# stevengj/nlopt

Hardware: AMD Instinct MI355X
Metric: candidate-evals/sec, CRS2_LM n=4096 pop=100000 (trial phase) (higher is better)
Workload: dtype f64; 1 GPU; NLOPT_GN_CRS2_LM griewank n=4096 pop=100000 seed=42, 2000 candidate evals per step, population resident in HBM

## Files before the change

include/nlopt_amd.h:

```cpp
#ifndef NLOPT_AMD_H
#define NLOPT_AMD_H

#include <stddef.h>
#include <stdint.h>
#include "nlopt.h"

#ifdef __cplusplus
extern "C" {
#endif

#define NLOPT_AMD_OBJ_RASTRIGIN  0
#define NLOPT_AMD_OBJ_ACKLEY     1
#define NLOPT_AMD_OBJ_GRIEWANK   2
#define NLOPT_AMD_OBJ_ROSENBROCK 3
#define NLOPT_AMD_OBJ_LEVY       4
#define NLOPT_AMD_OBJ_SPHERE     5
#define NLOPT_AMD_OBJ_COUNT      6

nlopt_func nlopt_amd_objective(int id);
int nlopt_amd_objective_id(nlopt_func f);
const char *nlopt_amd_objective_name(int id);
void nlopt_amd_objective_box(int id, double *lo, double *hi);

nlopt_func nlopt_amd_constraint_blocksum(void);
int nlopt_amd_constraint_id(nlopt_func f);

int nlopt_amd_device_count(void);

nlopt_result nlopt_amd_set_min_device_objective(nlopt_opt opt, const char *code_object, const char *name, nlopt_func host_twin, void *f_data);
nlopt_result nlopt_amd_set_max_device_objective(nlopt_opt opt, const char *code_object, const char *name, nlopt_func host_twin, void *f_data);
int nlopt_amd_has_device_objective(const nlopt_opt opt);

typedef struct { double f; int64_t row; int32_t kind; int32_t accepted; } nlopt_amd_trace_rec;
nlopt_result nlopt_amd_set_trace(nlopt_opt opt, nlopt_amd_trace_rec *buf, size_t cap);
size_t nlopt_amd_trace_len(const nlopt_opt opt);

typedef struct {
    uint64_t rounds;
    uint64_t slots_launched;
    uint64_t slots_used;
    uint64_t slots_invalid;
    uint64_t slots_newbest;
    uint64_t slots_role;
    uint64_t evals_init, evals_trial, evals_mutation;
    uint64_t accepted;
    uint64_t mt_words;
    double t_init_s, t_trial_s;
    double t_gather_ms;
    uint64_t gather_launches;
    uint64_t gather_bytes;
    uint64_t generations, rank_sweeps;
    double t_eval_s, t_rank_s, t_evolve_s, t_rng_s;
    uint64_t lbfgs_launches, lbfgs_bytes;
    double t_lbfgs_ms;
    double t_stochrank_ms;
    uint64_t stochrank_launches, stochrank_ticks;
    double t_allgather_ms;
    uint64_t allgather_bytes;
    uint64_t evolve_rounds_enqueued, evolve_rounds;
    double t_engine_s, t_walk_s;
    uint64_t list_refreshes, list_refreshes_beside_device;
    double t_list_refresh_s;
    uint64_t isres_gate_timeouts;
    uint64_t mlsl_sampled_ahead;
    uint64_t cobyla_host_searches;
    uint64_t lbfgs_longest_chain_steps;
    uint64_t mlsl_gate_timeouts;
} nlopt_amd_stats;
nlopt_result nlopt_amd_get_stats(const nlopt_opt opt, nlopt_amd_stats *out);
size_t nlopt_amd_get_stats_sized(const nlopt_opt opt, void *out, size_t bytes);

typedef void (*nlopt_amd_progress_fn)(void *data, long generations_done, long numevals);
nlopt_result nlopt_amd_set_progress(nlopt_opt opt, nlopt_amd_progress_fn fn, void *data);

typedef struct nlopt_amd_comm_s nlopt_amd_comm;
typedef int (*nlopt_amd_allgather_fn)(void *ctx, const void *h_send, void *h_recv, size_t bytes);
int nlopt_amd_rccl_unique_id(void *id128);
nlopt_amd_comm *nlopt_amd_comm_create_rccl(int rank, int world, const void *id128);
nlopt_amd_comm *nlopt_amd_comm_create_host(int rank, int world, nlopt_amd_allgather_fn fn, void *ctx);
nlopt_amd_comm *nlopt_amd_comm_create_shm(int rank, int world, const char *name, size_t slot_bytes);
void nlopt_amd_comm_set_timeout(nlopt_amd_comm *c, double seconds);
void nlopt_amd_comm_destroy(nlopt_amd_comm *c);
int nlopt_amd_comm_rank(const nlopt_amd_comm *c);
int nlopt_amd_comm_world(const nlopt_amd_comm *c);
const char *nlopt_amd_comm_error(const nlopt_amd_comm *c);
void nlopt_amd_comm_counters(const nlopt_amd_comm *c, uint64_t *calls, uint64_t *bytes);
nlopt_result nlopt_amd_set_comm(nlopt_opt opt, nlopt_amd_comm *c);

typedef struct nlopt_amd_crs_session nlopt_amd_crs_session;
nlopt_amd_crs_session *nlopt_amd_crs_open(nlopt_opt opt, double *x, double *minf, nlopt_result *ret);
nlopt_result nlopt_amd_crs_step(nlopt_amd_crs_session *s, long eval_budget);
nlopt_result nlopt_amd_crs_close(nlopt_amd_crs_session *s);

#define NLA_MT_N 624
#define NLA_MT_POLYWORDS 312
#define NLA_MT_SEG_REGENS 1024
#define NLA_MT_SEG_WORDS (624ULL * NLA_MT_SEG_REGENS)

int nla_k_mt_jump(const uint64_t *poly, const uint32_t *src_states, uint32_t *dst_states, int count, void *stream);

int nla_k_mt_generate(const uint32_t *seg_states, uint64_t seg_first, int nseg,
                      uint64_t g_first, uint64_t count, uint32_t *out, void *stream);
int nla_k_mt_generate_seg(const uint32_t *seg_states, uint64_t seg_first, int nseg, uint64_t g_first, uint64_t count, uint32_t *out,
                          int seg_regens, void *stream);
int nla_k_mt_rankbits(const uint32_t *seg_states, uint64_t seg_first, int nseg, uint64_t g_rank0, uint64_t g_first,
                      uint64_t count, int64_t popm1, int64_t rowwords, uint64_t *bits, void *stream);
int nla_k_mt_rankbits_gated(const uint32_t *seg_states, uint64_t seg_first, int nseg, uint64_t g_rank0, uint64_t g_first, uint64_t count,
                            int64_t popm1, int64_t rowwords, uint64_t *bits, int *gate, int *ticket, int waves_per_cu, void *stream);
int nla_rankbits_gate_target(uint64_t g_rank0, int64_t popm1, int64_t nrows, int64_t c);

int nla_k_crs_init_rows(int obj, int n, int ld, const double *lb, const double *ub, const uint32_t *words,
                        int64_t row_first, int64_t nrows, double *X, double *F, void *stream);

int nla_k_eval(int obj, int n, int ld, const double *P, int64_t count, double *F, void *stream);

int nla_k_crs_vitter(int n, int64_t N, const uint32_t *words, int nblocks,
                     int32_t *jn, int32_t *pos, int32_t *last, void *stream);

typedef struct { double fT, fM; int32_t t, pad; } nla_crs_slot_status;

int nla_k_crs_advance(int n, int ld, const double *X, int64_t i0, const int32_t *jn_ring,
                      const int32_t *pos_ring, const int32_t *last_ring, uint32_t ring_blocks,
                      uint64_t first_block, int K, const int64_t *W, int nW,
                      const int32_t *t_in, int32_t *t_out, int slot_mask, const double *lb, const double *ub,
                      double *TX, int variant, void *stream);

size_t nla_crs_chain_ctrl_bytes(int K, int nW);
int nla_crs_chain_chunks(int n, int ld);
int nla_k_crs_chain(int obj, int n, int ld, const double *X, int64_t i0, double f_best, const int32_t *jn_ring,
                    const int32_t *pos_ring, const int32_t *last_ring, const uint32_t *words_ring, uint32_t ring_blocks,
                    uint64_t first_block, int K, const int64_t *W, const double *Wf, int nW, int w_on_host, int slot_mask,
                    const double *lb, const double *ub, double *TX, double *TM, void *ctrl, uint32_t ticket_base,
                    nla_crs_slot_status *status, uint32_t *fwcnt, uint32_t *fwrec, int fwcap, void *stream);
int nla_k_crs_chain_lean(int obj, int n, int ld, const double *X, int64_t i0, double f_best, const int32_t *jn_ring,
                         const int32_t *pos_ring, const int32_t *last_ring, const uint32_t *words_ring, uint32_t ring_blocks,
                         uint64_t first_block, int K, const int64_t *W, const double *Wf, int nW, int w_on_host, int slot_mask,
                         const double *lb, const double *ub, double *TX, double *TM, void *ctrl, uint32_t ticket_base,
                         nla_crs_slot_status *status, uint32_t *fwcnt, uint32_t *fwrec, int fwcap, int ctrl_is_zero, void *stream);
int nla_crs_chain_sh_chunks(int n, int ncols);
size_t nla_crs_chain_sh_table_bytes(void);
size_t nla_crs_chain_sh_stop_bytes(void);
int nla_crs_chain_sh_table(void *host_image, int world, int rank, int c0, int ldf, int chunks_total, int chunk0, void *const *peerTX,
                           void *const *peerflags, void *const *peerstop, const double *xbest, const double *lbf, const double *ubf);
int nla_k_crs_chain_sh(int obj, int n, int ncols, int ld, int ldf, const double *X, int64_t i0, double f_best, const int32_t *jn_ring,
                       const int32_t *pos_ring, const int32_t *last_ring, const uint32_t *words_ring, uint32_t ring_blocks,
                       uint64_t first_block, int K, const int64_t *W, const double *Wf, int nW, int w_on_host, int slot_mask,
                       const double *lb, const double *ub, double *TX, double *TM, void *ctrl, uint32_t ticket_base,
                       nla_crs_slot_status *status, uint32_t *fwcnt, uint32_t *fwrec, int fwcap, int ctrl_is_zero,
                       const void *table, uint32_t seq, uint32_t stopbits, int grid_cap, void *stream);
uint32_t nla_crs_chain_sh_tickets(int n, int ncols, int K, int grid_cap);
int nla_k_crs_commit_sh(int nc, int ld, int ldf, int c0, double *X, const double *TX, const double *TM, int ncommit,
                        const int32_t *h_slot, const int32_t *h_kind, const int64_t *h_row, void *zero, size_t zero_bytes,
                        int n, int best_slot, int best_kind, double *xbest, void *stream);
uint32_t nla_crs_chain_tickets(int n, int ld, int K);

int nla_k_crs_finish(int obj, int n, int ld, const double *X, int64_t i0, const double *TX, double *TM,
                     const uint32_t *words_ring, uint32_t ring_blocks, uint64_t first_block, int K,
                     const int32_t *t_in, const int32_t *t_out, int slot_mask,
                     const double *lb, const double *ub, double *fT_ring, double *fM_ring,
                     nla_crs_slot_status *status, void *stream);

int nla_k_crs_advance_args(int n, int ld, const double *X, int64_t i0, const int32_t *jn_ring,
                           const int32_t *pos_ring, const int32_t *last_ring, uint32_t ring_blocks,
                           uint64_t first_block, int K, const int64_t *h_W, int nW,
                           const int32_t *h_t_in, int32_t *t_out, int slot_mask, const double *lb, const double *ub,
                           double *TX, int variant, void *stream);
int nla_k_crs_finish_args(int obj, int n, int ld, const double *X, int64_t i0, const double *TX, double *TM,
                          const uint32_t *words_ring, uint32_t ring_blocks, uint64_t first_block, int K,
                          const int32_t *h_t_in, const int32_t *t_out, int slot_mask,
                          const double *lb, const double *ub, double *fT_ring, double *fM_ring,
                          nla_crs_slot_status *status, void *stream);
int nla_k_crs_finish_args_bell(int obj, int n, int ld, const double *X, int64_t i0, const double *TX, double *TM,
                          const uint32_t *words_ring, uint32_t ring_blocks, uint64_t first_block, int K,
                          const int32_t *h_t_in, const int32_t *t_out, int slot_mask,
                          const double *lb, const double *ub, double *fT_ring, double *fM_ring,
                          nla_crs_slot_status *status, uint32_t *bell_count, uint32_t *bell, uint32_t bell_seq, void *stream);
int nla_k_crs_commit_args(int n, int ld, double *X, const double *TX, const double *TM, int ncommit,
                          const int32_t *h_slot, const int32_t *h_kind, const int64_t *h_row, void *stream);
int nla_k_crs_advance_commit_args(int n, int ld, double *X, int64_t i0, const int32_t *jn_ring,
                                  const int32_t *pos_ring, const int32_t *last_ring, uint32_t ring_blocks,
                                  uint64_t first_block, int K, const int64_t *h_W, int nW,
                                  const int32_t *h_t_in, int32_t *t_out, int slot_mask, const double *lb, const double *ub,
                                  double *TX, const double *TM, int ncommit, const int32_t *h_slot, const int32_t *h_kind,
                                  const int64_t *h_row, int variant, void *stream);

int nla_k_crs_advance_cols(int n, int ncol, int ld, const double *X, int64_t i0, const int32_t *jn_ring,
                           const int32_t *pos_ring, const int32_t *last_ring, uint32_t ring_blocks,
                           uint64_t first_block, int K, const int64_t *W, int nW,
                           const int32_t *t_in, int32_t *t_out, int slot_mask, const double *lb, const double *ub,
                           double *TX, int variant, void *stream);
int nla_k_crs_sh_init_rows(int n, int c0, int nc, int ld, const double *lb, const double *ub, const uint32_t *words,
                           int64_t row_first, int64_t nrows, double *X, void *stream);
int nla_k_crs_sh_mutate_pack(int n, int c0, int nc, int ld, int colper, const double *X, int64_t i0, const double *TX, double *TM,
                             const uint32_t *words_ring, uint32_t ring_blocks, uint64_t first_block, int K, const int32_t *t_in,
                             const int32_t *t_out, int slot_mask, const double *lb, const double *ub, double *SEND,
                             int flag_forced, int flag_timed, void *stream);
int nla_k_crs_sh_eval(int obj, int n, int colper, uint64_t first_block, int K, const int32_t *t_in, const int32_t *t_out, int slot_mask,
                      const double *RECV, int world, double *fT_ring, double *fM_ring, nla_crs_slot_status *status, void *stream);

int nla_k_crs_commit(int n, int ld, double *X, const double *TX, const double *TM, int ncommit,
                     const int32_t *slot, const int32_t *kind, const int64_t *row, void *stream);

int nla_k_crs_commit_zero(int n, int ld, double *X, const double *TX, const double *TM, int ncommit, const int32_t *slot,
                          const int32_t *kind, const int64_t *row, int lists_on_host, void *zero, size_t zero_bytes, void *stream);

int nla_k_crs_mutate(int n, const double *best, double *p, const uint32_t *words,
                     const double *lb, const double *ub, void *stream);


typedef struct { int32_t type; uint32_t q, Q; int32_t pad; double tol; } nla_dev_constraint;

int nla_k_isres_init(int n, int ld, const double *lb, const double *ub, const uint32_t *words, int64_t k_first,
                     int64_t count, const double *x0, double *X, double *S, void *stream);

int nla_k_isres_eval(int obj, int n, int ld, const double *X, int64_t pop, int m, int p, const nla_dev_constraint *con,
                     double *F, double *PEN, double *GPEN, int32_t *FEAS, void *stream);

int nla_k_isres_rank_count(int64_t pop, const double *F, const double *PEN, uint64_t *elems, int32_t *sorted, void *stream);

int nla_k_isres_bits(const uint32_t *words, int64_t row_first, int nrows, int64_t pop, uint64_t *bits, void *stream);

int nla_isres_stochrank_handoff(void);
int nla_k_isres_stochrank(int64_t pop, int64_t nsweeps, uint64_t *streams, int *progress, const uint64_t *bits,
                          int *ticket, uint8_t *swapped, int32_t *irank, void *stream);
int nla_k_isres_stochrank_gated(int64_t pop, int64_t nsweeps, uint64_t *streams, int *progress, const uint64_t *bits, int *ticket,
                                uint8_t *swapped, int32_t *irank, const int *gate, uint64_t gate_g_rank0, int64_t gate_nrows, void *stream);

int nla_k_isres_nrand(const uint32_t *words, int64_t nattempts, int64_t attempt_base, int32_t *counts, int64_t *ztotal,
                      int64_t zbase, double *z, int64_t *zatt, void *stream);

int nla_k_isres_evolve(int n, int ld, int phase, int64_t pop, int64_t survivors, int64_t zcount, double taup, double tau,
                       const double *lb, const double *ub, const double *z, const int32_t *irank, double *X, double *S,
                       double *scratch, int64_t *state, void *stream);

size_t nla_isres_evolve2_ws_bytes(int n);
int nla_isres_evolve2_supported(int n);
int nla_k_isres_inverse(int64_t pop, const int32_t *irank, int32_t *inv, void *stream);
int nla_k_isres_evolve_rounds(int n, int ld, int phase, int64_t pop, int64_t survivors, int64_t zcount, double taup, double tau,
                              const double *lb, const double *ub, const double *z, const int32_t *irank, const int32_t *inv,
                              double *X, double *S, const double *x0c, int64_t *state, double *rho, void *ws, const double *mu_rp,
                              int rounds, void *stream);
int nla_k_isres_evolve_parent_mu(int n, int ld, int64_t survivors, const double *lb, const double *ub, const int32_t *irank,
                                 const double *X, const double *S, double *mu_rp, void *stream);

#define NLA_OBJ_EXTERNAL (-1)
#define NLA_OBJ_NEGATE 0x100
typedef struct { int32_t state, want_grad; } nla_local_req;
typedef struct {
    nla_local_req *req;
    double *EX, *EG, *EF;
    void *save;
    int32_t resume;
    int32_t forced, timeout;
    int32_t pad;
} nla_local_ext;

typedef struct { double minf_max, ftol_rel, ftol_abs, xtol_rel, tolg; int32_t maxeval, exact; double sign;
                 const double *xtol_abs, *x_weights; const int32_t *abort;
                 double *ftrace; int64_t ftrace_cap;
                 int32_t *done;
               } nla_lbfgs_params;
typedef struct { double f; int32_t ret, nevals, iterm, cols; } nla_lbfgs_result;
size_t nla_lbfgs_work_doubles(int ld, int mf, int count);
size_t nla_lbfgs_hist_doubles(int ld, int mf, int count);
size_t nla_lbfgs_save_bytes(void);

int nla_k_lbfgs_batch(int obj, int n, int ld, int mf, int count, const double *lb, const double *ub, double *X,
                      double *work, int *iwork, double *hist, const nla_lbfgs_params *params, nla_lbfgs_result *out,
                      const nla_local_ext *ext, void *stream);

typedef struct { double minf_max, ftol_rel, ftol_abs, xtol_rel, rho_init, sigma_min;
                 int32_t maxeval, inner_maxeval, inner_gradients, always_improve; int32_t exact, pad; double sign;
                 const double *xtol_abs, *x_weights; const int32_t *abort;
                 double *ftrace; int64_t ftrace_cap;
                 int32_t *done;
               } nla_mma_params;
size_t nla_mma_work_doubles(int ld, int count);
size_t nla_mma_save_bytes(void);

typedef struct { double minf_max, ftol_rel, ftol_abs, xtol_rel; int32_t maxeval, exact; double sign;
                 const double *xtol_abs; const int32_t *abort; int32_t *done; } nla_cobyla_params;
size_t nla_cobyla_work_doubles(int n, int ld, int count);
size_t nla_cobyla_work_ints(int n, int count);
size_t nla_cobyla_lds_bytes(int n);
int nla_cobyla_fits(int n);
int nla_k_cobyla_batch(int obj, int n, int ld, int count, const double *lb, const double *ub, const double *dx, double *X,
                       double *work, int *iwork, const nla_cobyla_params *params, nla_lbfgs_result *out, void *stream);

int nla_k_mma_batch(int obj, int n, int ld, int count, const double *lb, const double *ub, const double *sigma_init, double *X,
                    double *work, const nla_mma_params *params, nla_lbfgs_result *out, const nla_local_ext *ext, void *stream);

int nla_k_mlsl_sobol_rows(int n, int ld, const double *lb, const double *ub, const uint32_t *V, uint32_t index_first,
                          int count, double *P, void *stream);
int nla_k_mlsl_dist2(int n, int ld, const double *A, int na, const double *B, int nb, double *D, void *stream);
int nla_k_mlsl_rowmin(const double *D, int ldd, int na, int nb, const double *FA, const double *FB, const double *init, double *out, void *stream);
int nla_k_mlsl_colmin(const double *D, int ldd, int na, int nb, const double *FA, const double *FB, const int32_t *skip, double *inout, void *stream);
int nla_k_mlsl_gather_rows(int n, int ld, const double *src, const int64_t *idx, int count, double *dst, void *stream);
int nla_k_mlsl_gather_pairs(const double *D, int ldd, const int64_t *rows, int nr, const int64_t *cols, int nc, double *out, void *stream);
int nla_k_mlsl_gather_pairs_t(const double *D, int ldd, const int64_t *rows, int nr, const int64_t *cols, int nc, double *out, void *stream);
int nla_k_mlsl_near_bound(int n, int ld, const double *P, const int64_t *idx, int count, const double *lb, const double *ub,
                          double thr, int32_t *flags, void *stream);

int nla_k_mlsl_negate(double *F, int count, void *stream);

int nla_k_esch_cauchy(const uint32_t *words, int64_t nattempts, int64_t attempt_base, int32_t *counts, int64_t *vtotal,
                      int64_t vbase, int64_t vcap, double *v, int64_t *vatt, void *stream);
int nla_k_esch_fill_rows(int n, int ld, const double *lb, const double *ub, const double *v, int64_t e0, int64_t count, double *R, void *stream);
int nla_k_esch_crossover(int n, int ld, int64_t np, int64_t no, const uint32_t *words, const int32_t *slot, double *R, void *stream);
size_t nla_esch_mut_scratch_bytes(int64_t M);
int nla_k_esch_mutate(const uint32_t *W, int64_t M, int64_t total, int n, int ld, int64_t np, int64_t no, const double *lb,
                      const double *ub, const int32_t *slot, double *R, int32_t *last, void *scratch, int64_t *out, void *stream);
int nla_k_esch_gather_rows(int n, int ld, const int32_t *slot, int64_t i0, int64_t count, const double *R, double *G, void *stream);
size_t nla_esch_sort_scratch_bytes(int64_t count);
int nla_k_esch_select(int64_t count, const int32_t *slot_in, const double *fit_in, int32_t *slot_out, double *fit_out,
                      void *scratch, size_t scratch_bytes, void *stream);

int nla_dev_count(void);
int nla_dev_set(int dev);
void *nla_dev_malloc(size_t bytes);
void nla_dev_free(void *p);
void *nla_dev_malloc_uncached(size_t bytes);
void nla_debug_uncached_stats(long out[4]);
void nla_dev_free_uncached(void *p);
size_t nlopt_amd_release_device_memory(void);
void *nla_host_malloc(size_t bytes);
void nla_host_free(void *p);
int nla_host_register(void *p, size_t bytes);
void nla_host_unregister(void *p);
int nla_memcpy_h2d(void *dst, const void *h_src, size_t bytes, void *stream);
int nla_memcpy_d2h(void *h_dst, const void *src, size_t bytes, void *stream);
int nla_memcpy_d2d(void *dst, const void *src, size_t bytes, void *stream);
int nla_memset(void *dst, int value, size_t bytes, void *stream);
void *nla_stream_create(void);
void *nla_stream_create_cu_share(int part, int parts);
#define NLA_IPC_BYTES 96
int nla_ipc_export(const void *p, void *blob96);
void *nla_ipc_open(const void *blob96);
void nla_ipc_close(void *p);
void *nla_stream_create_background(void);
void nla_stream_destroy(void *stream);
int nla_stream_sync(void *stream);
int nla_stream_query(void *stream);
void *nla_event_create(void);
void nla_event_destroy(void *ev);
int nla_event_record(void *ev, void *stream);
int nla_event_sync(void *ev);
float nla_event_elapsed_ms(void *ev0, void *ev1);
int nla_stream_wait_event(void *stream, void *ev);
int nla_k_gate(const int32_t *counter, int32_t from, int32_t need, double timeout_ms, int32_t *gave_up , void *stream);
const char *nla_dev_error_string(int err);
void *nla_module_load_file(const char *path);
void *nla_module_load_data(const void *image);
void nla_module_unload(void *module);
void *nla_module_function(void *module, const char *name);
int nla_module_launch(void *function, unsigned grid_x, unsigned block_x, void **params, void *stream);

#ifdef __cplusplus
}
#endif
#endif
```

nlopt_amd/__init__.py:

```python
import ctypes as C
import os

import numpy as np

_HERE = os.path.dirname(os.path.abspath(__file__))
LIB_PATH = os.environ.get("NLOPT_AMD_LIB") or os.path.join(_HERE, "lib", "libnlopt_amd.so")

GN_CRS2_LM, GN_MLSL, GD_MLSL, GN_MLSL_LDS, GD_MLSL_LDS = 19, 20, 21, 22, 23
LD_LBFGS, LD_MMA, GN_ISRES, G_MLSL, G_MLSL_LDS, GN_ESCH = 11, 24, 35, 38, 39, 42
LN_COBYLA = 25
FAILURE, INVALID_ARGS, OUT_OF_MEMORY, ROUNDOFF_LIMITED, FORCED_STOP = -1, -2, -3, -4, -5
SUCCESS, STOPVAL_REACHED, FTOL_REACHED, XTOL_REACHED, MAXEVAL_REACHED, MAXTIME_REACHED = 1, 2, 3, 4, 5, 6

OBJECTIVES = {"rastrigin": 0, "ackley": 1, "griewank": 2, "rosenbrock": 3, "levy": 4, "sphere": 5}

NLOPT_FUNC = C.CFUNCTYPE(C.c_double, C.c_uint, C.POINTER(C.c_double), C.POINTER(C.c_double), C.c_void_p)

TRACE_DTYPE = np.dtype([("f", "f8"), ("row", "i8"), ("kind", "i4"), ("accepted", "i4")])


class Stats(C.Structure):
    _fields_ = [(k, C.c_uint64) for k in ("rounds", "slots_launched", "slots_used", "slots_invalid", "slots_newbest",
                                           "slots_role", "evals_init", "evals_trial", "evals_mutation", "accepted",
                                           "mt_words")] + \
               [("t_init_s", C.c_double), ("t_trial_s", C.c_double), ("t_gather_ms", C.c_double),
                ("gather_launches", C.c_uint64), ("gather_bytes", C.c_uint64), ("generations", C.c_uint64),
                ("rank_sweeps", C.c_uint64), ("t_eval_s", C.c_double), ("t_rank_s", C.c_double), ("t_evolve_s", C.c_double),
                ("t_rng_s", C.c_double), ("lbfgs_launches", C.c_uint64), ("lbfgs_bytes", C.c_uint64), ("t_lbfgs_ms", C.c_double),
                ("t_stochrank_ms", C.c_double), ("stochrank_launches", C.c_uint64), ("stochrank_ticks", C.c_uint64),
                ("t_allgather_ms", C.c_double), ("allgather_bytes", C.c_uint64),
                ("evolve_rounds_enqueued", C.c_uint64), ("evolve_rounds", C.c_uint64),
                ("t_engine_s", C.c_double), ("t_walk_s", C.c_double),
                ("list_refreshes", C.c_uint64), ("list_refreshes_beside_device", C.c_uint64), ("t_list_refresh_s", C.c_double),
                ("isres_gate_timeouts", C.c_uint64), ("mlsl_sampled_ahead", C.c_uint64), ("cobyla_host_searches", C.c_uint64), ("lbfgs_longest_chain_steps", C.c_uint64), ("mlsl_gate_timeouts", C.c_uint64)]

    def asdict(self):
        return {k: getattr(self, k) for k, _ in self._fields_}


_lib = None


def build(force=False, verbose=False):
    from . import _build as _b
    return _b.build(force=force, verbose=verbose)


def _dp(a):
    return a.ctypes.data_as(C.POINTER(C.c_double))


def lib():
    global _lib
    if _lib is not None:
        return _lib
    if not os.path.exists(LIB_PATH):
        raise RuntimeError("libnlopt_amd.so is not built: run `python -c 'import __graft_entry__ as g; g.build()'`")
    L = C.CDLL(LIB_PATH)
    vp, dbl, dpp = C.c_void_p, C.c_double, C.POINTER(C.c_double)
    L.nlopt_create.restype = vp
    L.nlopt_create.argtypes = [C.c_int, C.c_uint]
    L.nlopt_copy.restype = vp
    L.nlopt_copy.argtypes = [vp]
    L.nlopt_destroy.argtypes = [vp]
    L.nlopt_destroy.restype = None
    L.nlopt_optimize.argtypes = [vp, dpp, dpp]
    for nm in ("nlopt_set_min_objective", "nlopt_set_max_objective"):
        getattr(L, nm).argtypes = [vp, vp, vp]
    for nm in ("nlopt_set_lower_bounds", "nlopt_set_upper_bounds", "nlopt_get_lower_bounds", "nlopt_get_upper_bounds",
               "nlopt_set_xtol_abs", "nlopt_get_xtol_abs", "nlopt_set_x_weights", "nlopt_get_x_weights",
               "nlopt_set_initial_step"):
        getattr(L, nm).argtypes = [vp, dpp]
    for nm in ("nlopt_set_lower_bounds1", "nlopt_set_upper_bounds1", "nlopt_set_stopval", "nlopt_set_ftol_rel",
               "nlopt_set_ftol_abs", "nlopt_set_xtol_rel", "nlopt_set_xtol_abs1", "nlopt_set_x_weights1",
               "nlopt_set_maxtime", "nlopt_set_initial_step1"):
        getattr(L, nm).argtypes = [vp, dbl]
    for nm in ("nlopt_get_stopval", "nlopt_get_ftol_rel", "nlopt_get_ftol_abs", "nlopt_get_xtol_rel", "nlopt_get_maxtime"):
        getattr(L, nm).argtypes = [vp]
        getattr(L, nm).restype = dbl
    L.nlopt_set_lower_bound.argtypes = [vp, C.c_int, dbl]
    L.nlopt_set_upper_bound.argtypes = [vp, C.c_int, dbl]
    L.nlopt_set_maxeval.argtypes = [vp, C.c_int]
    for nm in ("nlopt_get_maxeval", "nlopt_get_numevals", "nlopt_get_force_stop", "nlopt_force_stop", "nlopt_get_algorithm"):
        getattr(L, nm).argtypes = [vp]
    L.nlopt_set_force_stop.argtypes = [vp, C.c_int]
    L.nlopt_get_dimension.argtypes = [vp]
    L.nlopt_get_dimension.restype = C.c_uint
    L.nlopt_set_population.argtypes = [vp, C.c_uint]
    L.nlopt_get_population.argtypes = [vp]
    L.nlopt_get_population.restype = C.c_uint
    L.nlopt_set_vector_storage.argtypes = [vp, C.c_uint]
    L.nlopt_get_vector_storage.argtypes = [vp]
    L.nlopt_get_vector_storage.restype = C.c_uint
    L.nlopt_set_local_optimizer.argtypes = [vp, vp]
    L.nlopt_get_errmsg.argtypes = [vp]
    L.nlopt_get_errmsg.restype = C.c_char_p
    L.nlopt_set_param.argtypes = [vp, C.c_char_p, dbl]
    L.nlopt_get_param.argtypes = [vp, C.c_char_p, dbl]
    L.nlopt_get_param.restype = dbl
    L.nlopt_has_param.argtypes = [vp, C.c_char_p]
    L.nlopt_num_params.argtypes = [vp]
    L.nlopt_num_params.restype = C.c_uint
    L.nlopt_nth_param.argtypes = [vp, C.c_uint]
    L.nlopt_nth_param.restype = C.c_char_p
    for nm in ("nlopt_add_inequality_constraint", "nlopt_add_equality_constraint"):
        getattr(L, nm).argtypes = [vp, vp, vp, dbl]
    for nm in ("nlopt_remove_inequality_constraints", "nlopt_remove_equality_constraints"):
        getattr(L, nm).argtypes = [vp]
    L.nlopt_srand.argtypes = [C.c_ulong]
    L.nlopt_srand.restype = None
    L.nlopt_algorithm_name.argtypes = [C.c_int]
    L.nlopt_algorithm_name.restype = C.c_char_p
    L.nlopt_algorithm_to_string.argtypes = [C.c_int]
    L.nlopt_algorithm_to_string.restype = C.c_char_p
    L.nlopt_algorithm_from_string.argtypes = [C.c_char_p]
    L.nlopt_result_to_string.argtypes = [C.c_int]
    L.nlopt_result_to_string.restype = C.c_char_p
    L.nlopt_result_from_string.argtypes = [C.c_char_p]
    L.nlopt_version.argtypes = [C.POINTER(C.c_int)] * 3
    L.nlopt_urand.argtypes = [dbl, dbl]
    L.nlopt_urand.restype = dbl
    L.nlopt_nrand.argtypes = [dbl, dbl]
    L.nlopt_nrand.restype = dbl
    L.nlopt_iurand.argtypes = [C.c_int]
    L.nla_genrand_int32.restype = C.c_uint32
    L.nlopt_amd_objective.argtypes = [C.c_int]
    L.nlopt_amd_objective.restype = vp
    L.nlopt_amd_objective_id.argtypes = [vp]
    L.nlopt_amd_objective_name.argtypes = [C.c_int]
    L.nlopt_amd_objective_name.restype = C.c_char_p
    L.nlopt_amd_objective_box.argtypes = [C.c_int, dpp, dpp]
    L.nlopt_amd_objective_box.restype = None
    L.nlopt_amd_constraint_blocksum.restype = vp
    L.nlopt_amd_set_trace.argtypes = [vp, vp, C.c_size_t]
    L.nlopt_amd_trace_len.argtypes = [vp]
    L.nlopt_amd_trace_len.restype = C.c_size_t
    L.nlopt_amd_get_stats.argtypes = [vp, C.POINTER(Stats)]
    L.nlopt_amd_crs_open.argtypes = [vp, dpp, dpp, C.POINTER(C.c_int)]
    L.nlopt_amd_crs_open.restype = vp
    L.nlopt_amd_crs_step.argtypes = [vp, C.c_long]
    L.nlopt_amd_crs_close.argtypes = [vp]
    L.nla_dev_malloc.argtypes = [C.c_size_t]
    L.nla_dev_malloc.restype = vp
    L.nla_dev_free.argtypes = [vp]
    L.nla_dev_free.restype = None
    for nm in ("nla_memcpy_h2d", "nla_memcpy_d2h", "nla_memcpy_d2d"):
        getattr(L, nm).argtypes = [vp, vp, C.c_size_t, vp]
    L.nla_memset.argtypes = [vp, C.c_int, C.c_size_t, vp]
    L.nla_stream_create.restype = vp
    L.nla_stream_destroy.argtypes = [vp]
    L.nla_stream_sync.argtypes = [vp]
    L.nla_event_create.restype = vp
    L.nla_event_destroy.argtypes = [vp]
    L.nla_event_record.argtypes = [vp, vp]
    L.nla_event_sync.argtypes = [vp]
    L.nla_event_elapsed_ms.argtypes = [vp, vp]
    L.nla_event_elapsed_ms.restype = C.c_float
    L.nla_dev_error_string.argtypes = [C.c_int]
    L.nla_dev_error_string.restype = C.c_char_p
    L.nla_mtstream_create.argtypes = [vp]
    L.nla_mtstream_create.restype = vp
    L.nla_mtstream_destroy.argtypes = [vp]
    L.nla_mtstream_destroy.restype = None
    L.nla_mtstream_fill.argtypes = [vp, C.c_uint64, C.c_uint64, vp]
    L.nla_mtstream_finish.argtypes = [vp, C.c_uint64]
    L.nla_mtstream_rankbits.argtypes = [vp, C.c_uint64, C.c_uint64, C.c_uint64, C.c_int64, C.c_int64, vp]
    L.nla_k_mt_jump.argtypes = [vp, vp, vp, C.c_int, vp]
    L.nla_k_mt_generate.argtypes = [vp, C.c_uint64, C.c_int, C.c_uint64, C.c_uint64, vp, vp]
    L.nla_k_crs_init_rows.argtypes = [C.c_int, C.c_int, C.c_int, vp, vp, vp, C.c_int64, C.c_int64, vp, vp, vp]
    L.nla_k_eval.argtypes = [C.c_int, C.c_int, C.c_int, vp, C.c_int64, vp, vp]
    L.nla_k_crs_vitter.argtypes = [C.c_int, C.c_int64, vp, C.c_int, vp, vp, vp, vp]
    L.nla_k_crs_advance.argtypes = [C.c_int, C.c_int, vp, C.c_int64, vp, vp, vp, C.c_uint32, C.c_uint64, C.c_int, vp, C.c_int,
                                    vp, vp, C.c_int, vp, vp, vp, C.c_int, vp]
    L.nlopt_amd_has_device_objective.argtypes = [vp]
    L.nla_dev_malloc_uncached.argtypes = [C.c_size_t]
    L.nla_dev_malloc_uncached.restype = vp
    L.nla_dev_free_uncached.argtypes = [vp]
    L.nla_dev_free_uncached.restype = None
    L.nla_k_crs_chain.argtypes = [C.c_int, C.c_int, C.c_int, vp, C.c_int64, C.c_double, vp, vp, vp, vp, C.c_uint32, C.c_uint64, C.c_int, vp, vp,
                                  C.c_int, C.c_int, C.c_int, vp, vp, vp, vp, vp, C.c_uint32, vp, vp, vp, C.c_int, vp]
    L.nla_crs_chain_tickets.argtypes = [C.c_int, C.c_int, C.c_int]
    L.nla_crs_chain_tickets.restype = C.c_uint32
    L.nla_crs_chain_ctrl_bytes.argtypes = [C.c_int, C.c_int]
    L.nla_crs_chain_ctrl_bytes.restype = C.c_size_t
    L.nla_crs_chain_chunks.argtypes = [C.c_int, C.c_int]
    L.nla_k_crs_finish.argtypes = [C.c_int, C.c_int, C.c_int, vp, C.c_int64, vp, vp, vp, C.c_uint32, C.c_uint64, C.c_int,
                                   vp, vp, C.c_int, vp, vp, vp, vp, vp, vp]
    L.nla_k_isres_rank_count.argtypes = [C.c_int64, vp, vp, vp, vp, vp]
    L.nla_k_isres_bits.argtypes = [vp, C.c_int64, C.c_int, C.c_int64, vp, vp]
    L.nla_k_isres_stochrank.argtypes = [C.c_int64, C.c_int64, vp, vp, vp, vp, vp, vp, vp]
    L.nla_k_isres_stochrank_gated.argtypes = [C.c_int64, C.c_int64, vp, vp, vp, vp, vp, vp, vp, C.c_uint64, C.c_int64, vp]
    L.nla_isres_evolve2_ws_bytes.restype = C.c_size_t
    L.nla_isres_evolve2_ws_bytes.argtypes = [C.c_int]
    L.nla_k_isres_inverse.argtypes = [C.c_int64, vp, vp, vp]
    L.nla_k_isres_evolve_rounds.argtypes = ([C.c_int, C.c_int, C.c_int, C.c_int64, C.c_int64, C.c_int64, C.c_double, C.c_double] + [vp] * 12 +
                                            [C.c_int, vp])
    L.nla_k_crs_commit.argtypes = [C.c_int, C.c_int, vp, vp, vp, C.c_int, vp, vp, vp, vp]
    L.nla_k_crs_mutate.argtypes = [C.c_int, vp, vp, vp, vp, vp, vp]
    L.nla_mt_jump_poly_words.argtypes = [C.c_uint64, vp]
    L.nla_mt_jump_poly_words.restype = None
    L.nla_mt_jump_poly_pow2.argtypes = [C.c_int]
    L.nla_mt_jump_poly_pow2.restype = vp
    L.nla_mt_apply_jump_host.argtypes = [vp, vp, vp]
    L.nla_mt_apply_jump_host.restype = None
    L.nla_mt_advance_blocks_host.argtypes = [vp, C.c_uint64, vp]
    L.nla_mt_advance_blocks_host.restype = None
    L.nla_mt_export.argtypes = [vp, C.POINTER(C.c_int)]
    L.nla_mt_export.restype = None
    L.nla_mt_import.argtypes = [vp, C.c_int]
    L.nla_mt_import.restype = None
    L.nla_mt_charpoly_terms.argtypes = [C.POINTER(C.POINTER(C.c_int))]
    L.nlopt_amd_rccl_unique_id.argtypes = [vp]
    L.nlopt_amd_comm_create_rccl.argtypes = [C.c_int, C.c_int, vp]
    L.nlopt_amd_comm_create_rccl.restype = vp
    L.nlopt_amd_comm_create_host.argtypes = [C.c_int, C.c_int, vp, vp]
    L.nlopt_amd_comm_create_host.restype = vp
    L.nlopt_amd_comm_destroy.argtypes = [vp]
    L.nlopt_amd_comm_destroy.restype = None
    L.nlopt_amd_comm_rank.argtypes = [vp]
    L.nlopt_amd_comm_world.argtypes = [vp]
    L.nlopt_amd_comm_error.argtypes = [vp]
    L.nlopt_amd_comm_error.restype = C.c_char_p
    L.nlopt_amd_comm_counters.argtypes = [vp, C.POINTER(C.c_uint64), C.POINTER(C.c_uint64)]
    L.nlopt_amd_comm_counters.restype = None
    L.nlopt_amd_set_comm.argtypes = [vp, vp]
    L.nlopt_amd_set_progress.argtypes = [vp, vp, vp]
    L.nla_comm_allgather_host.argtypes = [vp, vp, vp, C.c_size_t, vp]
    L.nla_comm_allgather_dev.argtypes = [vp, vp, vp, C.c_size_t, vp]
    L.nla_comm_partition.argtypes = [vp, C.c_int64, C.POINTER(C.c_int64), C.POINTER(C.c_int64), C.POINTER(C.c_int64)]
    L.nla_comm_partition.restype = None
    L.nla_dev_set.argtypes = [C.c_int]
    _lib = L
    return L


def device_count():
    return lib().nlopt_amd_device_count()


def srand(seed):
    lib().nlopt_srand(seed)


def objective(name_or_id):
    i = OBJECTIVES[name_or_id] if isinstance(name_or_id, str) else int(name_or_id)
    return lib().nlopt_amd_objective(i)


def objective_box(name_or_id):
    i = OBJECTIVES[name_or_id] if isinstance(name_or_id, str) else int(name_or_id)
    lo, hi = C.c_double(), C.c_double()
    lib().nlopt_amd_objective_box(i, C.byref(lo), C.byref(hi))
    return lo.value, hi.value


class DevBuf:

    def __init__(self, nbytes, uncached=False):
        self.nbytes = int(nbytes)
        self.uncached = bool(uncached)
        self.ptr = (lib().nla_dev_malloc_uncached if uncached else lib().nla_dev_malloc)(self.nbytes)
        if not self.ptr:
            raise MemoryError("nla_dev_malloc(%d) failed" % self.nbytes)

    @classmethod
    def from_array(cls, a, uncached=False):
        a = np.ascontiguousarray(a)
        b = cls(max(a.nbytes, 1), uncached)
        L = lib()
        rc = L.nla_memcpy_h2d(b.ptr, a.ctypes.data, a.nbytes, None) or L.nla_stream_sync(None)
        if rc:
            raise RuntimeError("H2D failed: %s" % L.nla_dev_error_string(rc))
        return b

    def to_array(self, dtype, count):
        out = np.empty(count, dtype=dtype)
        L = lib()
        rc = L.nla_memcpy_d2h(out.ctypes.data, self.ptr, out.nbytes, None) or L.nla_stream_sync(None)
        if rc:
            raise RuntimeError("D2H failed: %s" % L.nla_dev_error_string(rc))
        return out

    def free(self):
        if self.ptr:
            (lib().nla_dev_free_uncached if getattr(self, "uncached", False) else lib().nla_dev_free)(self.ptr)
            self.ptr = None

    def __del__(self):
        try:
            self.free()
        except Exception:
            pass


PROGRESS_FN = C.CFUNCTYPE(None, C.c_void_p, C.c_long, C.c_long)
ALLGATHER_FN = C.CFUNCTYPE(C.c_int, C.c_void_p, C.c_void_p, C.c_void_p, C.c_size_t)


class Comm:

    def __init__(self, handle, keep=None):
        self._L = lib()
        self._h = handle
        self._keep = keep
        if not handle:
            raise RuntimeError("could not create the communicator")

    @classmethod
    def rccl(cls, rank, world, uid):
        buf = C.create_string_buffer(bytes(uid), 128)
        return cls(lib().nlopt_amd_comm_create_rccl(int(rank), int(world), C.cast(buf, C.c_void_p)))

    @classmethod
    def shm(cls, rank, world, name, slot_bytes=0):
        L = lib()
        L.nlopt_amd_comm_create_shm.restype = C.c_void_p
        L.nlopt_amd_comm_create_shm.argtypes = [C.c_int, C.c_int, C.c_char_p, C.c_size_t]
        return cls(L.nlopt_amd_comm_create_shm(int(rank), int(world), name.encode(), int(slot_bytes)))

    @classmethod
    def host(cls, rank, world, allgather):
        def _cb(ctx, send, recv, nbytes):
            try:
                out = allgather(C.string_at(send, nbytes))
                if len(out) != nbytes * world:
                    return 2
                C.memmove(recv, out, len(out))
                return 0
            except Exception:
                import traceback
                traceback.print_exc()
                return 1
        fn = ALLGATHER_FN(_cb)
        return cls(lib().nlopt_amd_comm_create_host(int(rank), int(world), C.cast(fn, C.c_void_p), None), keep=fn)

    @classmethod
    def from_torch_distributed(cls, group=None):
# ... 196 lines not shown
```

nlopt_amd/csrc/api_options.c:

```c
#include "nla_internal.h"
#include <math.h>
#include <stdarg.h>
#include <stdlib.h>
#include <string.h>

static double *dup_doubles(const double *src, unsigned n)
{
    double *d;
    if (!src) return NULL;
    d = (double *) malloc(sizeof(double) * (n ? n : 1));
    if (d && n) memcpy(d, src, sizeof(double) * n);
    return d;
}

const char *nla_set_errmsg(nlopt_opt opt, const char *fmt, ...)
{
    va_list ap;
    va_start(ap, fmt);
    opt->errmsg = nla_vsprintf(opt->errmsg, fmt, ap);
    va_end(ap);
    return opt->errmsg;
}
void nla_unset_errmsg(nlopt_opt opt) { if (opt) { free(opt->errmsg); opt->errmsg = NULL; } }
const char *nlopt_get_errmsg(nlopt_opt opt) { return opt->errmsg; }

static nlopt_result fail_msg(nlopt_opt opt, nlopt_result r, const char *msg) { if (opt) nla_set_errmsg(opt, "%s", msg); return r; }

static void free_constraints(nlopt_opt opt, nla_constraint **c, unsigned *m, unsigned *m_alloc, int munge)
{
    unsigned i;
    if (munge && opt->munge_on_destroy) for (i = 0; i < *m; ++i) opt->munge_on_destroy((*c)[i].f_data);
    for (i = 0; i < *m; ++i) free((*c)[i].tol);
    free(*c);
    *c = NULL; *m = *m_alloc = 0;
}

void nlopt_destroy(nlopt_opt opt)
{
    unsigned i;
    if (!opt) return;
    if (opt->munge_on_destroy) opt->munge_on_destroy(opt->f_data);
    free_constraints(opt, &opt->fc, &opt->m, &opt->m_alloc, 1);
    free_constraints(opt, &opt->h, &opt->p, &opt->p_alloc, 1);
    for (i = 0; i < opt->nparams; ++i) free(opt->params[i].name);
    free(opt->params);
    free(opt->lb); free(opt->ub); free(opt->xtol_abs); free(opt->x_weights); free(opt->dx);
    nlopt_destroy(opt->local_opt);
    nla_userobj_release(opt->userobj);
    free(opt->errmsg);
    free(opt);
}

nlopt_opt nlopt_create(nlopt_algorithm algorithm, unsigned n)
{
    nlopt_opt opt;
    unsigned i;
    if ((int) algorithm < 0 || algorithm >= NLOPT_NUM_ALGORITHMS) return NULL;
    opt = (nlopt_opt) calloc(1, sizeof *opt);
    if (!opt) return NULL;
    opt->algorithm = algorithm;
    opt->n = n;
    opt->stopval = -HUGE_VAL;
    if (n > 0) {
        opt->lb = (double *) malloc(sizeof(double) * n);
        opt->ub = (double *) malloc(sizeof(double) * n);
        if (!opt->lb || !opt->ub) { nlopt_destroy(opt); return NULL; }
        for (i = 0; i < n; ++i) { opt->lb[i] = -HUGE_VAL; opt->ub[i] = +HUGE_VAL; }
    }
    return opt;
}

static int copy_constraints(nlopt_opt dst, nla_constraint **dc, unsigned *dm, unsigned *dalloc,
                            const nla_constraint *sc, unsigned sm)
{
    unsigned i;
    *dc = NULL; *dm = *dalloc = 0;
    if (!sm) return 0;
    *dc = (nla_constraint *) malloc(sizeof(nla_constraint) * sm);
    if (!*dc) return -1;
    memcpy(*dc, sc, sizeof(nla_constraint) * sm);
    for (i = 0; i < sm; ++i) (*dc)[i].tol = NULL;
    *dm = *dalloc = sm;
    for (i = 0; i < sm; ++i) {
        if (dst->munge_on_copy && (*dc)[i].f_data && !((*dc)[i].f_data = dst->munge_on_copy((*dc)[i].f_data))) return -1;
        if (sc[i].tol && !((*dc)[i].tol = dup_doubles(sc[i].tol, sc[i].m))) return -1;
    }
    return 0;
}

nlopt_opt nlopt_copy(const nlopt_opt opt)
{
    nlopt_opt c;
    unsigned i;
    if (!opt) return NULL;
    c = (nlopt_opt) malloc(sizeof *c);
    if (!c) return NULL;
    *c = *opt;
    c->lb = c->ub = c->xtol_abs = c->x_weights = c->dx = NULL;
    c->fc = c->h = NULL; c->m = c->m_alloc = c->p = c->p_alloc = 0;
    c->params = NULL; c->nparams = 0;
    c->local_opt = NULL; c->errmsg = NULL; c->force_stop_child = NULL;
    c->trace = NULL; c->trace_cap = c->trace_len = 0;
    nla_userobj_retain(c->userobj);
    if (c->munge_on_copy && c->f_data && !(c->f_data = c->munge_on_copy(c->f_data))) goto oom;
    if (opt->n > 0) {
        if (!(c->lb = dup_doubles(opt->lb, opt->n)) || !(c->ub = dup_doubles(opt->ub, opt->n))) goto oom;
        if (opt->xtol_abs && !(c->xtol_abs = dup_doubles(opt->xtol_abs, opt->n))) goto oom;
        if (opt->x_weights && !(c->x_weights = dup_doubles(opt->x_weights, opt->n))) goto oom;
        if (opt->dx && !(c->dx = dup_doubles(opt->dx, opt->n))) goto oom;
    }
    if (copy_constraints(c, &c->fc, &c->m, &c->m_alloc, opt->fc, opt->m)) goto oom;
    if (copy_constraints(c, &c->h, &c->p, &c->p_alloc, opt->h, opt->p)) goto oom;
    if (opt->nparams) {
        c->params = (nla_param *) calloc(opt->nparams, sizeof(nla_param));
        if (!c->params) goto oom;
        c->nparams = opt->nparams;
        for (i = 0; i < opt->nparams; ++i) {
            size_t len = strlen(opt->params[i].name) + 1;
            if (!(c->params[i].name = (char *) malloc(len))) goto oom;
            memcpy(c->params[i].name, opt->params[i].name, len);
            c->params[i].val = opt->params[i].val;
        }
    }
    if (opt->local_opt && !(c->local_opt = nlopt_copy(opt->local_opt))) goto oom;
    return c;
oom:
    c->munge_on_destroy = NULL;
    nlopt_destroy(c);
    return NULL;
}

nlopt_result nlopt_set_param(nlopt_opt opt, const char *name, double val)
{
    size_t len;
    unsigned i;
    if (!opt) return NLOPT_INVALID_ARGS;
    if (!name) return fail_msg(opt, NLOPT_INVALID_ARGS, "invalid NULL parameter name");
    len = strnlen(name, 1024) + 1;
    if (len > 1024) return fail_msg(opt, NLOPT_INVALID_ARGS, "parameter name must be < 1024 bytes");
    if (!strncmp(name, "amd_", 4)) {
        static const char *const known[] = { "amd_forward", "amd_shard", "amd_shard_windows", "amd_cu_share", "amd_max_spec", "amd_window_factor", "amd_host_eval",
                                             "amd_exact_dot", "amd_isres_evolve_serial", "amd_isres_overlap", "amd_lbfgs_streaming", "amd_mlsl_seg_regens", "amd_cobyla_host", "amd_cobyla_min_batch", NULL };
        int k;
        for (k = 0; known[k] && strcmp(name, known[k]); ++k) { }
        if (!known[k]) return fail_msg(opt, NLOPT_INVALID_ARGS, "nlopt_amd: no such switch (the amd_* names this build reads: include/nlopt_amd.h, INTEGRATION.md E)");
    }
    for (i = 0; i < opt->nparams; ++i) if (!strcmp(name, opt->params[i].name)) break;
    if (i == opt->nparams) {
        nla_param *np = (nla_param *) realloc(opt->params, sizeof(nla_param) * (opt->nparams + 1));
        if (!np) return NLOPT_OUT_OF_MEMORY;
        opt->params = np;
        if (!(np[i].name = (char *) malloc(len))) return NLOPT_OUT_OF_MEMORY;
        memcpy(np[i].name, name, len);
        opt->nparams++;
    }
    opt->params[i].val = val;
    return NLOPT_SUCCESS;
}

static int find_param(const nlopt_opt opt, const char *name)
{
    unsigned i;
    if (!opt || !name || strnlen(name, 1024) == 1024) return -1;
    for (i = 0; i < opt->nparams; ++i) if (!strcmp(name, opt->params[i].name)) return (int) i;
    return -1;
}
double nlopt_get_param(const nlopt_opt opt, const char *name, double defaultval)
{
    int i = find_param(opt, name);
    return i < 0 ? defaultval : opt->params[i].val;
}
int nlopt_has_param(const nlopt_opt opt, const char *name) { return find_param(opt, name) >= 0; }
unsigned nlopt_num_params(const nlopt_opt opt) { return opt ? opt->nparams : 0; }
const char *nlopt_nth_param(const nlopt_opt opt, unsigned n) { return opt && n < opt->nparams ? opt->params[n].name : NULL; }

static nlopt_result set_objective(nlopt_opt opt, nlopt_func f, nlopt_precond pre, void *f_data, int maximize)
{
    if (!opt) return NLOPT_INVALID_ARGS;
    nla_unset_errmsg(opt);
    if (opt->munge_on_destroy) opt->munge_on_destroy(opt->f_data);
    nla_userobj_release(opt->userobj);
    opt->userobj = NULL;
    opt->f = f; opt->f_data = f_data; opt->pre = pre; opt->maximize = maximize;
    if (nla_isinf(opt->stopval) && (maximize ? opt->stopval < 0 : opt->stopval > 0))
        opt->stopval = maximize ? +HUGE_VAL : -HUGE_VAL;
    return NLOPT_SUCCESS;
}
nlopt_result nlopt_set_precond_min_objective(nlopt_opt o, nlopt_func f, nlopt_precond pre, void *d) { return set_objective(o, f, pre, d, 0); }
nlopt_result nlopt_set_precond_max_objective(nlopt_opt o, nlopt_func f, nlopt_precond pre, void *d) { return set_objective(o, f, pre, d, 1); }
nlopt_result nlopt_set_min_objective(nlopt_opt o, nlopt_func f, void *d) { return set_objective(o, f, NULL, d, 0); }
nlopt_result nlopt_set_max_objective(nlopt_opt o, nlopt_func f, void *d) { return set_objective(o, f, NULL, d, 1); }

static void snap_lower(nlopt_opt opt, unsigned i) { if (opt->lb[i] < opt->ub[i] && nla_istiny(opt->ub[i] - opt->lb[i])) opt->lb[i] = opt->ub[i]; }
static void snap_upper(nlopt_opt opt, unsigned i) { if (opt->lb[i] < opt->ub[i] && nla_istiny(opt->ub[i] - opt->lb[i])) opt->ub[i] = opt->lb[i]; }

nlopt_result nlopt_set_lower_bounds(nlopt_opt opt, const double *lb)
{
    unsigned i;
    nla_unset_errmsg(opt);
    if (!opt || (opt->n && !lb)) return NLOPT_INVALID_ARGS;
    for (i = 0; i < opt->n; ++i) opt->lb[i] = lb[i];
    for (i = 0; i < opt->n; ++i) snap_lower(opt, i);
    return NLOPT_SUCCESS;
}
nlopt_result nlopt_set_lower_bounds1(nlopt_opt opt, double lb)
{
    unsigned i;
    nla_unset_errmsg(opt);
    if (!opt) return NLOPT_INVALID_ARGS;
    for (i = 0; i < opt->n; ++i) { opt->lb[i] = lb; snap_lower(opt, i); }
    return NLOPT_SUCCESS;
}
nlopt_result nlopt_set_lower_bound(nlopt_opt opt, int i, double lb)
{
    nla_unset_errmsg(opt);
    if (!opt) return NLOPT_INVALID_ARGS;
    if (i < 0 || i >= (int) opt->n) return fail_msg(opt, NLOPT_INVALID_ARGS, "invalid bound index");
    opt->lb[i] = lb; snap_lower(opt, (unsigned) i);
    return NLOPT_SUCCESS;
}
nlopt_result nlopt_get_lower_bounds(const nlopt_opt opt, double *lb)
{
    nla_unset_errmsg(opt);
    if (!opt || (opt->n && !lb)) return NLOPT_INVALID_ARGS;
    if (opt->n) memcpy(lb, opt->lb, sizeof(double) * opt->n);
    return NLOPT_SUCCESS;
}
nlopt_result nlopt_set_upper_bounds(nlopt_opt opt, const double *ub)
{
    unsigned i;
    nla_unset_errmsg(opt);
    if (!opt || (opt->n && !ub)) return NLOPT_INVALID_ARGS;
    for (i = 0; i < opt->n; ++i) opt->ub[i] = ub[i];
    for (i = 0; i < opt->n; ++i) snap_upper(opt, i);
    return NLOPT_SUCCESS;
}
nlopt_result nlopt_set_upper_bounds1(nlopt_opt opt, double ub)
{
    unsigned i;
    nla_unset_errmsg(opt);
    if (!opt) return NLOPT_INVALID_ARGS;
    for (i = 0; i < opt->n; ++i) { opt->ub[i] = ub; snap_upper(opt, i); }
    return NLOPT_SUCCESS;
}
nlopt_result nlopt_set_upper_bound(nlopt_opt opt, int i, double ub)
{
    nla_unset_errmsg(opt);
    if (!opt) return NLOPT_INVALID_ARGS;
    if (i < 0 || i >= (int) opt->n) return fail_msg(opt, NLOPT_INVALID_ARGS, "invalid bound index");
    opt->ub[i] = ub; snap_upper(opt, (unsigned) i);
    return NLOPT_SUCCESS;
}
nlopt_result nlopt_get_upper_bounds(const nlopt_opt opt, double *ub)
{
    nla_unset_errmsg(opt);
    if (!opt || (opt->n && !ub)) return NLOPT_INVALID_ARGS;
    if (opt->n) memcpy(ub, opt->ub, sizeof(double) * opt->n);
    return NLOPT_SUCCESS;
}

static int is_auglag(nlopt_algorithm a)
{
    return a == NLOPT_AUGLAG || a == NLOPT_AUGLAG_EQ || a == NLOPT_LN_AUGLAG || a == NLOPT_LN_AUGLAG_EQ ||
           a == NLOPT_LD_AUGLAG || a == NLOPT_LD_AUGLAG_EQ;
}
static int accepts_inequality(nlopt_algorithm a)
{
    return a == NLOPT_LD_MMA || a == NLOPT_LD_CCSAQ || a == NLOPT_LD_SLSQP || a == NLOPT_LN_COBYLA || is_auglag(a) ||
           a == NLOPT_GN_ISRES || a == NLOPT_GN_ORIG_DIRECT || a == NLOPT_GN_ORIG_DIRECT_L || a == NLOPT_GN_AGS;
}
static int accepts_equality(nlopt_algorithm a)
{
    return is_auglag(a) || a == NLOPT_LD_SLSQP || a == NLOPT_GN_ISRES || a == NLOPT_LN_COBYLA;
}

static nlopt_result push_constraint(nlopt_opt opt, unsigned *m, unsigned *m_alloc, nla_constraint **c, unsigned fm,
                                    nlopt_func fc, nlopt_mfunc mfc, nlopt_precond pre, void *data, const double *tol)
{
    double *tolcopy;
    unsigned i;
    if ((fc && mfc) || (fc && fm != 1) || (!fc && !mfc)) return NLOPT_INVALID_ARGS;
    if (tol) for (i = 0; i < fm; ++i) if (tol[i] < 0) return fail_msg(opt, NLOPT_INVALID_ARGS, "negative constraint tolerance");
    tolcopy = (double *) calloc(fm ? fm : 1, sizeof(double));
    if (!tolcopy) return NLOPT_OUT_OF_MEMORY;
    if (tol) memcpy(tolcopy, tol, sizeof(double) * fm);
    if (*m + 1 > *m_alloc) {
        unsigned na = 2 * (*m + 1);
        nla_constraint *nc = (nla_constraint *) realloc(*c, sizeof(nla_constraint) * na);
        if (!nc) { free(tolcopy); return NLOPT_OUT_OF_MEMORY; }
        *c = nc; *m_alloc = na;
    }
    (*c)[*m].m = fm; (*c)[*m].f = fc; (*c)[*m].mf = mfc; (*c)[*m].pre = pre; (*c)[*m].f_data = data; (*c)[*m].tol = tolcopy;
    ++*m;
    return NLOPT_SUCCESS;
}

static nlopt_result add_any(nlopt_opt opt, int equality, unsigned fm, nlopt_func fc, nlopt_mfunc mfc, nlopt_precond pre,
                            void *data, const double *tol)
{
    nlopt_result ret;
    nla_unset_errmsg(opt);
    if (mfc && !fm) {
        if (opt && opt->munge_on_destroy) opt->munge_on_destroy(data);
        return NLOPT_SUCCESS;
    }
    if (!opt) ret = NLOPT_INVALID_ARGS;
    else if (!(equality ? accepts_equality(opt->algorithm) : accepts_inequality(opt->algorithm)))
        ret = fail_msg(opt, NLOPT_INVALID_ARGS, "invalid algorithm for constraints");
    else if (equality) ret = push_constraint(opt, &opt->p, &opt->p_alloc, &opt->h, fm, fc, mfc, pre, data, tol);
    else ret = push_constraint(opt, &opt->m, &opt->m_alloc, &opt->fc, fm, fc, mfc, pre, data, tol);
    if (ret < 0 && opt && opt->munge_on_destroy) opt->munge_on_destroy(data);
    return ret;
}

nlopt_result nlopt_remove_inequality_constraints(nlopt_opt opt)
{
    nla_unset_errmsg(opt);
    if (!opt) return NLOPT_INVALID_ARGS;
    free_constraints(opt, &opt->fc, &opt->m, &opt->m_alloc, 1);
    return NLOPT_SUCCESS;
}
nlopt_result nlopt_remove_equality_constraints(nlopt_opt opt)
{
    nla_unset_errmsg(opt);
    if (!opt) return NLOPT_INVALID_ARGS;
    free_constraints(opt, &opt->h, &opt->p, &opt->p_alloc, 1);
    return NLOPT_SUCCESS;
}
nlopt_result nlopt_add_inequality_mconstraint(nlopt_opt o, unsigned m, nlopt_mfunc fc, void *d, const double *tol) { return add_any(o, 0, m, NULL, fc, NULL, d, tol); }
nlopt_result nlopt_add_precond_inequality_constraint(nlopt_opt o, nlopt_func fc, nlopt_precond pre, void *d, double tol) { return add_any(o, 0, 1, fc, NULL, pre, d, &tol); }
nlopt_result nlopt_add_inequality_constraint(nlopt_opt o, nlopt_func fc, void *d, double tol) { return add_any(o, 0, 1, fc, NULL, NULL, d, &tol); }
nlopt_result nlopt_add_equality_mconstraint(nlopt_opt o, unsigned m, nlopt_mfunc fc, void *d, const double *tol) { return add_any(o, 1, m, NULL, fc, NULL, d, tol); }
nlopt_result nlopt_add_precond_equality_constraint(nlopt_opt o, nlopt_func fc, nlopt_precond pre, void *d, double tol) { return add_any(o, 1, 1, fc, NULL, pre, d, &tol); }
nlopt_result nlopt_add_equality_constraint(nlopt_opt o, nlopt_func fc, void *d, double tol) { return add_any(o, 1, 1, fc, NULL, NULL, d, &tol); }

#define NLA_SCALAR(name, T, field)                                                             \
    nlopt_result nlopt_set_##name(nlopt_opt opt, T v)                                          \
    { if (!opt) return NLOPT_INVALID_ARGS; nla_unset_errmsg(opt); opt->field = v; return NLOPT_SUCCESS; } \
    T nlopt_get_##name(const nlopt_opt opt) { return opt->field; }
NLA_SCALAR(stopval, double, stopval)
NLA_SCALAR(ftol_rel, double, ftol_rel)
NLA_SCALAR(ftol_abs, double, ftol_abs)
NLA_SCALAR(xtol_rel, double, xtol_rel)
NLA_SCALAR(maxeval, int, maxeval)
NLA_SCALAR(maxtime, double, maxtime)
NLA_SCALAR(population, unsigned, stochastic_population)
NLA_SCALAR(vector_storage, unsigned, vector_storage)
int nlopt_get_numevals(const nlopt_opt opt) { return opt->numevals; }
nlopt_algorithm nlopt_get_algorithm(const nlopt_opt opt) { return opt->algorithm; }
unsigned nlopt_get_dimension(const nlopt_opt opt) { return opt->n; }

static nlopt_result ensure_vec(nlopt_opt opt, double **v)
{
    if (!*v && opt->n > 0) { *v = (double *) calloc(opt->n, sizeof(double)); if (!*v) return NLOPT_OUT_OF_MEMORY; }
    return NLOPT_SUCCESS;
}

nlopt_result nlopt_set_xtol_abs(nlopt_opt opt, const double *tol)
{
    if (!opt) return NLOPT_INVALID_ARGS;
    nla_unset_errmsg(opt);
    if (!tol) { free(opt->xtol_abs); opt->xtol_abs = NULL; return NLOPT_SUCCESS; }
    if (ensure_vec(opt, &opt->xtol_abs) != NLOPT_SUCCESS) return NLOPT_OUT_OF_MEMORY;
    if (opt->n) memcpy(opt->xtol_abs, tol, sizeof(double) * opt->n);
    return NLOPT_SUCCESS;
}
nlopt_result nlopt_set_xtol_abs1(nlopt_opt opt, double tol)
{
    unsigned i;
    if (!opt) return NLOPT_INVALID_ARGS;
    nla_unset_errmsg(opt);
    if (ensure_vec(opt, &opt->xtol_abs) != NLOPT_SUCCESS) return NLOPT_OUT_OF_MEMORY;
    for (i = 0; i < opt->n; ++i) opt->xtol_abs[i] = tol;
    return NLOPT_SUCCESS;
}
nlopt_result nlopt_get_xtol_abs(const nlopt_opt opt, double *tol)
{
    unsigned i;
    nla_unset_errmsg(opt);
    if (!opt || (opt->n && !tol)) return NLOPT_INVALID_ARGS;
    for (i = 0; i < opt->n; ++i) tol[i] = opt->xtol_abs ? opt->xtol_abs[i] : 0;
    return NLOPT_SUCCESS;
}
nlopt_result nlopt_set_x_weights(nlopt_opt opt, const double *w)
{
    unsigned i;
    if (!opt) return NLOPT_INVALID_ARGS;
    nla_unset_errmsg(opt);
    if (!w) { free(opt->x_weights); opt->x_weights = NULL; return NLOPT_SUCCESS; }
    for (i = 0; i < opt->n; ++i) if (w[i] < 0) return fail_msg(opt, NLOPT_INVALID_ARGS, "invalid negative weight");
    if (ensure_vec(opt, &opt->x_weights) != NLOPT_SUCCESS) return NLOPT_OUT_OF_MEMORY;
    if (opt->n) memcpy(opt->x_weights, w, sizeof(double) * opt->n);
    return NLOPT_SUCCESS;
}
nlopt_result nlopt_set_x_weights1(nlopt_opt opt, double w)
{
    unsigned i;
    if (!opt) return NLOPT_INVALID_ARGS;
    if (w < 0) return fail_msg(opt, NLOPT_INVALID_ARGS, "invalid negative weight");
    nla_unset_errmsg(opt);
    if (ensure_vec(opt, &opt->x_weights) != NLOPT_SUCCESS) return NLOPT_OUT_OF_MEMORY;
    for (i = 0; i < opt->n; ++i) opt->x_weights[i] = w;
    return NLOPT_SUCCESS;
}
nlopt_result nlopt_get_x_weights(const nlopt_opt opt, double *w)
{
    unsigned i;
    if (!opt) return NLOPT_INVALID_ARGS;
    if (opt->n && !w) return fail_msg(opt, NLOPT_INVALID_ARGS, "invalid NULL weights");
    nla_unset_errmsg(opt);
    for (i = 0; i < opt->n; ++i) w[i] = opt->x_weights ? opt->x_weights[i] : 1;
    return NLOPT_SUCCESS;
}

nlopt_result nlopt_set_force_stop(nlopt_opt opt, int val)
{
    if (!opt) return NLOPT_INVALID_ARGS;
    nla_unset_errmsg(opt);
    opt->force_stop = val;
    if (opt->force_stop_child) return nlopt_set_force_stop(opt->force_stop_child, val);
    return NLOPT_SUCCESS;
}
int nlopt_get_force_stop(const nlopt_opt opt) { return opt->force_stop; }
nlopt_result nlopt_force_stop(nlopt_opt opt) { return nlopt_set_force_stop(opt, 1); }

nlopt_result nlopt_set_local_optimizer(nlopt_opt opt, const nlopt_opt local_opt)
{
    if (!opt) return NLOPT_INVALID_ARGS;
    nla_unset_errmsg(opt);
    if (local_opt && local_opt->n != opt->n) return fail_msg(opt, NLOPT_INVALID_ARGS, "dimension mismatch in local optimizer");
    nlopt_destroy(opt->local_opt);
    opt->local_opt = nlopt_copy(local_opt);
    if (local_opt) {
        if (!opt->local_opt) return NLOPT_OUT_OF_MEMORY;
        nlopt_set_lower_bounds(opt->local_opt, opt->lb);
        nlopt_set_upper_bounds(opt->local_opt, opt->ub);
        nlopt_remove_inequality_constraints(opt->local_opt);
        nlopt_remove_equality_constraints(opt->local_opt);
        nlopt_set_min_objective(opt->local_opt, NULL, NULL);
        nlopt_set_munge(opt->local_opt, NULL, NULL);
        opt->local_opt->force_stop = 0;
    }
    return NLOPT_SUCCESS;
}
// ... 92 lines not shown
```

nlopt_amd/csrc/crs_driver.c:

```c
#include "nla_internal.h"
#include <limits.h>
#include <math.h>
#include <stdlib.h>
#include <string.h>

typedef struct { double f; int64_t row; } osnode;
typedef struct {
    const double *F;
    osnode *node;
    void *mem;
    int64_t nheap, best;
    void *cand;
    int64_t *gpos;
} ordset;
#define OSN(s, i) ((s)->node[(i) + 3])

static inline int key_less(const double *F, int64_t a, int64_t b)
{
    if (F[a] < F[b]) return 1;
    if (F[a] > F[b]) return 0;
    return a < b;
}
static inline int node_less(const osnode a, const osnode b)
{
// ... 172 lines not shown
    tl_refresh(t, s, ahead > need ? ahead : need);
}

static inline int64_t tl_worst(const toplist *t) { return t->T[t->head].row; }

static void tl_idle(toplist *t, ordset *s)
{
    const int k = t->inflight;
    if (k <= 0 || t->whole || t->tail - t->head - k >= k) return;
    { const uint64_t r0 = t->refreshes; tl_refresh(t, s, 3 * k + 16); t->refreshes_idle += t->refreshes - r0; }
}

static void tl_accepted(toplist *t, ordset *s)
{
    topent e = t->T[t->head++];
    const double f = s->F[e.row];
    if (!e.recorded) {
        t->chg[t->nchg++] = e.pos;
        e.recorded = 1;
    }
    if (t->whole || t->thr_f < f || (!(t->thr_f > f) && t->thr_row < e.row)) {
        int lo = t->head, hi = t->tail;
        osnode k; k.f = f; k.row = e.row;
        while (lo < hi) {
            const int mid = (lo + hi) >> 1;
            osnode m; m.f = t->T[mid].f; m.row = t->T[mid].row;
            if (node_less(m, k)) hi = mid; else lo = mid + 1;
        }
        if (t->tail == 2 * t->cap) {
            memmove(t->T, t->T + t->head, sizeof(topent) * (size_t) (t->tail - t->head));
            lo -= t->head; t->tail -= t->head; t->head = 0;
        }
        memmove(t->T + lo + 1, t->T + lo, sizeof(topent) * (size_t) (t->tail - lo));
        e.f = f;
        t->T[lo] = e;
        ++t->tail;
    }
}

typedef struct {
    const nla_crs_engine_ops *ops; void *e;
    const nla_crs_problem *pb;
    ordset os;
    double *F;
    double *x;
    double *minf;
    double *xtmp;
    int need_x;
    const nla_stopping *sp;
    int64_t xrow;
    nlopt_result ret;
} run_state;

static void trace_add(const nla_crs_problem *pb, double f, int64_t row, int kind, int accepted)
{
    if (!pb->trace || !pb->trace_len) return;
    if (*pb->trace_len < pb->trace_cap) {
        nlopt_amd_trace_rec *r = pb->trace + *pb->trace_len;
        r->f = f; r->row = row; r->kind = kind; r->accepted = accepted;
    }
    ++*pb->trace_len;
}

static int after_accept(run_state *rs, uint64_t block, int kind)
{
    const nla_crs_problem *pb = rs->pb;
    nla_stopping *stop = pb->stop;
    const int64_t b = rs->os.best;
    nlopt_result ret = NLOPT_SUCCESS;
    int have_x = 0;
    if (rs->F[b] < *rs->minf) {
        if (rs->F[b] < stop->minf_max) ret = NLOPT_MINF_MAX_REACHED;
        else if (nla_stop_f(stop, rs->F[b], *rs->minf)) ret = NLOPT_FTOL_REACHED;
        else if (rs->need_x) {
            if (rs->ops->read_slot(rs->e, block, kind, rs->xtmp)) return -1;
            if (nla_stop_x(stop, rs->xtmp, rs->x)) ret = NLOPT_XTOL_REACHED;
            memcpy(rs->x, rs->xtmp, sizeof(double) * (size_t) pb->n);
            have_x = 1;
        }
        rs->xrow = have_x ? -1 : b;
        *rs->minf = rs->F[b];
    }
    if (ret != NLOPT_SUCCESS) {
        if (nla_stop_evals(stop)) ret = NLOPT_MAXEVAL_REACHED;
        else if (nla_stop_time(rs->sp)) ret = NLOPT_MAXTIME_REACHED;
    }
    rs->ret = ret;
    return 0;
}

#define TRING 2048
#define FWCAP 48

struct nla_crs_session {
    run_state rs;
    nla_crs_problem pb;
    nlopt_result ret;
    uint64_t block;
    uint64_t fresh_from;
    uint64_t init_words;
    int Kmax, host_eval;
    double kmult;
    double runlen;
    nla_crs_slot_status *status;
    int32_t *tprev;
    uint64_t *cblock;
    int32_t *ckind;
    int64_t *W, *crow;
    toplist tl;
    int forward;
    double *Wf;
    uint32_t *fwcnt, *fwrec;
    uint64_t *lastw;
    nla_stopping view; int agreed_force;
};

static void session_free(nla_crs_session *S)
{
    if (!S) return;
    free(S->rs.F); os_free(&S->rs.os); free(S->rs.xtmp);
    free(S->status); free(S->tprev); free(S->W); tl_free(&S->tl); free(S->cblock); free(S->ckind); free(S->crow);
    free(S->Wf); free(S->fwcnt); free(S->fwrec); free(S->lastw);
    free(S);
}

static void crs_idle(void *arg)
{
    nla_crs_session *S = (nla_crs_session *) arg;
    tl_idle(&S->tl, &S->rs.os);
}

static void engine_failed(nla_crs_session *S)
{
    nla_stopping *stop = S->pb.stop;
    if (stop->stop_msg && S->rs.ops->last_error) nla_stop_msg(stop, "device engine: %s", S->rs.ops->last_error(S->rs.e));
    S->ret = NLOPT_FAILURE;
}

nla_crs_session *nla_crs_begin(const nla_crs_engine_ops *ops, void *e, const nla_crs_problem *pb,
                               double *x, double *minf, nlopt_result *ret_out)
{
    const int n = pb->n;
    const int64_t N = pb->N;
    nla_stopping *stop = pb->stop;
    nlopt_amd_stats *st = pb->stats;
    nla_crs_session *S = (nla_crs_session *) calloc(1, sizeof *S);
    run_state *rs;
    nlopt_result ret = NLOPT_SUCCESS;
    int64_t rows_done = 0, i;
    double t0 = nla_seconds();
    if (!S) { *ret_out = NLOPT_OUT_OF_MEMORY; return NULL; }
    rs = &S->rs;
    S->pb = *pb;
    S->host_eval = pb->obj == -1;
    S->Kmax = pb->max_spec > 0 ? pb->max_spec : 256;
    S->kmult = pb->window_factor > 0 ? pb->window_factor : 1.5;
    if (S->Kmax > 1024) S->Kmax = 1024;
    if (S->host_eval) S->Kmax = 1;
    S->forward = pb->forward && ops->chain && pb->obj >= 0 && S->Kmax > 1;
    if (S->forward && S->Kmax > 256) S->Kmax = 256;
    if (S->forward && pb->max_spec <= 0 && S->Kmax > (n >= 2048 ? 128 : 256)) S->Kmax = n >= 2048 ? 128 : 256;
    if (S->forward && pb->max_spec <= 0 && (int64_t) S->Kmax > N / 16) S->Kmax = N / 16 > 8 ? (int) (N / 16) : 8;
    S->runlen = 4.0;
    rs->ops = ops; rs->e = e; rs->pb = &S->pb; rs->x = x; rs->minf = minf;
    rs->need_x = (stop->xtol_rel > 0 || stop->xtol_abs != NULL);

    rs->F = (double *) malloc(sizeof(double) * (size_t) N);
    const int os_bad = os_alloc(&rs->os, N, 3 * S->Kmax + 64);
    rs->xtmp = (double *) malloc(sizeof(double) * (size_t) (n > 0 ? n : 1));
    S->status = (nla_crs_slot_status *) malloc(sizeof(nla_crs_slot_status) * (size_t) S->Kmax);
    S->tprev = (int32_t *) calloc(TRING, sizeof(int32_t));
    S->W = (int64_t *) malloc(sizeof(int64_t) * (size_t) S->Kmax);
    const int tl_bad = tl_alloc(&S->tl, S->Kmax);
    S->cblock = (uint64_t *) malloc(sizeof(uint64_t) * (size_t) S->Kmax);
    S->ckind = (int32_t *) malloc(sizeof(int32_t) * (size_t) S->Kmax);
    S->crow = (int64_t *) malloc(sizeof(int64_t) * (size_t) S->Kmax);
    S->Wf = (double *) malloc(sizeof(double) * (size_t) S->Kmax);
    if (S->forward) {
        S->fwcnt = (uint32_t *) calloc((size_t) S->Kmax, sizeof(uint32_t));
        S->fwrec = (uint32_t *) calloc((size_t) S->Kmax * FWCAP, sizeof(uint32_t));
        S->lastw = (uint64_t *) calloc((size_t) N, sizeof(uint64_t));
    }
    if (!rs->F || os_bad || !rs->xtmp || !S->status || !S->tprev || !S->W || tl_bad || !S->Wf || !S->cblock ||
        !S->ckind || !S->crow || (S->forward && (!S->fwcnt || !S->fwrec || !S->lastw))) {
        session_free(S);
        *ret_out = NLOPT_OUT_OF_MEMORY;
        return NULL;
    }
    rs->os.F = rs->F;
    S->tl.st = st;
    if (ops->set_idle) ops->set_idle(e, crs_idle, S);

    rs->sp = stop;
    if (ops->init_population(e, x, rs->F)) { engine_failed(S); *ret_out = S->ret; return S; }
    if (pb->comm) {
        rs->sp = nla_comm_agree_stop(pb->comm, stop, &S->view, &S->agreed_force);
        if (!rs->sp) { nla_stop_msg(stop, "stop agreement failed: %s", nlopt_amd_comm_error(pb->comm)); S->ret = NLOPT_FAILURE; *ret_out = S->ret; return S; }
    }
    for (i = 0; i < N && ret == NLOPT_SUCCESS; ++i) {
        if (S->host_eval) {
            if (i == 0) rs->F[0] = pb->f((unsigned) n, x, NULL, pb->f_data);
            else {
                if (ops->read_row(e, i, rs->xtmp)) { engine_failed(S); *ret_out = S->ret; return S; }
                rs->F[i] = pb->f((unsigned) n, rs->xtmp, NULL, pb->f_data);
            }
        }
        ++*stop->nevals_p;
        if (st) ++st->evals_init;
        os_push(&rs->os, i);
        trace_add(pb, rs->F[i], i, 0, 1);
        rows_done = i + 1;
        if (rs->F[i] < stop->minf_max) ret = NLOPT_MINF_MAX_REACHED;
        else if (nla_stop_evals(stop)) ret = NLOPT_MAXEVAL_REACHED;
        else if (nla_stop_time(rs->sp)) ret = NLOPT_MAXTIME_REACHED;
    }
    S->init_words = 2ULL * (uint64_t) n * (uint64_t) (rows_done - 1);
    *minf = rs->F[rs->os.best];
    if (ops->read_row(e, rs->os.best, x)) { engine_failed(S); *ret_out = S->ret; return S; }
    rs->xrow = -1;
    if (st) st->t_init_s = nla_seconds() - t0;
    S->ret = ret;
    *ret_out = ret;
    return S;
}

nlopt_result nla_crs_advance(nla_crs_session *S, int64_t eval_budget)
{
    run_state *rs = &S->rs;
    const nla_crs_engine_ops *ops = rs->ops;
    void *e = rs->e;
    const nla_crs_problem *pb = &S->pb;
    nla_stopping *stop = pb->stop;
    nlopt_amd_stats *st = pb->stats;
    const int n = pb->n, host_eval = S->host_eval;
    const int64_t N = pb->N;
    nla_crs_slot_status *status = S->status;
    uint64_t *cblock = S->cblock;
    int32_t *ckind = S->ckind;
    int64_t *W = S->W, *crow = S->crow;
    nlopt_result ret = S->ret;
    const int evals_at_entry = *stop->nevals_p;
    double t0 = nla_seconds();

    while (ret == NLOPT_SUCCESS) {
        int K, nW, j = 0, ncommit = 0, best_changed = 0, cap, a, timed_pass = 1;
        uint64_t wend;
        if (eval_budget > 0 && (int64_t) (*stop->nevals_p - evals_at_entry) >= eval_budget) break;
        if (pb->comm) {
            if (ops->stop_flags_in && ops->stop_flags_out) ops->stop_flags_in(e, nla_stop_forced(stop), nla_stop_time(stop));
            else {
                rs->sp = nla_comm_agree_stop(pb->comm, stop, &S->view, &S->agreed_force);
                if (!rs->sp) { nla_stop_msg(stop, "stop agreement failed: %s", nlopt_amd_comm_error(pb->comm)); S->ret = NLOPT_FAILURE; return S->ret; }
            }
        }
        cap = ops->max_slots(e, S->block);
        if (cap <= 0) { engine_failed(S); return S->ret; }
        K = (int) ceil(S->kmult * S->runlen) + 4;
        if (K > S->Kmax) K = S->Kmax;
        if (K > cap) K = cap;
        if (K < 1) K = 1;
        if (!S->forward && S->fresh_from > S->block && (uint64_t) K < S->fresh_from - S->block && S->fresh_from - S->block <= (uint64_t) cap &&
            S->fresh_from - S->block <= (uint64_t) S->Kmax)
            K = (int) (S->fresh_from - S->block);
        nW = K < N ? K : (int) N;
        tl_need(&S->tl, &rs->os, nW, 3 * K + 16);
        for (a = 0; a < nW; ++a) { W[a] = S->tl.T[S->tl.head + a].row; S->Wf[a] = S->tl.T[S->tl.head + a].f; }
        if (S->forward) for (a = 0; a < nW; ++a) __builtin_prefetch(&S->lastw[W[a]], 1);
        const double t_eng0 = st ? nla_seconds() : 0.;
        const uint64_t gl0 = st ? st->gather_launches : 0;
        S->tl.inflight = nW;
        if (S->forward) {
            if (st && S->fresh_from > S->block) st->slots_invalid += S->fresh_from - S->block;
            S->fresh_from = S->block;
            if (ops->chain(e, S->block, K, rs->os.best, rs->F[rs->os.best], W, S->Wf, nW, status, S->fwcnt, S->fwrec, FWCAP)) { engine_failed(S); return S->ret; }
            if (pb->comm && ops->stop_flags_in && ops->stop_flags_out) {
                int forced = 0, timed = 0;
                ops->stop_flags_out(e, &forced, &timed);
                nla_stop_view(stop, forced, timed, &S->view, &S->agreed_force);
                rs->sp = &S->view;
            }
        } else
        {
            if (!S->forward && ops->advance(e, S->block, K, S->fresh_from, rs->os.best, W, nW, status)) { engine_failed(S); return S->ret; }
            if (pb->comm && ops->stop_flags_in && ops->stop_flags_out) {
                int forced = 0, timed = 0;
                ops->stop_flags_out(e, &forced, &timed);
                nla_stop_view(stop, forced, timed, &S->view, &S->agreed_force);
                rs->sp = &S->view;
            }
        }
        S->tl.inflight = 0;
        timed_pass = !st || st->gather_launches != gl0;
        wend = S->block + (uint64_t) K;
        const double t_walk0 = st ? nla_seconds() : 0.;
        if (st) {
            st->t_engine_s += t_walk0 - t_eng0;
            ++st->rounds;
            for (a = 0; a < K; ++a) {
                const uint64_t b = S->block + (uint64_t) a;
                const int32_t told = b >= S->fresh_from ? 0 : S->tprev[b % TRING];
                const int32_t tnew = status[a].t;
                if (b >= S->fresh_from) ++st->slots_launched;
                if (tnew > told && timed_pass) st->gather_bytes += 8ULL * (uint64_t) n * (uint64_t) (tnew - told + (told == 0 ? 1 : 0));
                S->tprev[b % TRING] = tnew;
            }
        }
        if (wend > S->fresh_from) S->fresh_from = wend;

        while (j < K && ret == NLOPT_SUCCESS) {
            int64_t worst;
            int kind = 1, accepted = 0;
            double fcand;
            const uint64_t blk = S->block + (uint64_t) j;
            if (best_changed) break;
            if (status[j].t < n) break;
            if (S->forward) {
                const uint32_t cnt = S->fwcnt[j];
                int ok = cnt <= FWCAP;
                uint32_t c;
                for (c = 0; ok && c < cnt; ++c) {
                    const uint32_t rec = S->fwrec[(size_t) j * FWCAP + c];
                    const int64_t r = W[rec & 0xffu];
                    const uint64_t pbk = S->block + (uint64_t) ((rec >> 8) & 0xffu);
                    const unsigned kind = (rec >> 16) & 3u;
                    if (kind == 0) ok = (S->lastw[r] >> 1) <= S->block;
                    else ok = S->lastw[r] == (((pbk + 1) << 1) | (kind == 1 ? 1u : 0u));
                }
                if (!ok) {
                    if (st) ++st->slots_invalid;
                    break;
                }
            }
            if (st) ++st->slots_used;
            if (S->tl.head == S->tl.tail) tl_need(&S->tl, &rs->os, 1, 3 * K + 16);
            worst = tl_worst(&S->tl);
            if (host_eval) {
                if (ops->read_slot(e, blk, 1, rs->xtmp)) { engine_failed(S); return S->ret; }
                status[j].fT = pb->f((unsigned) n, rs->xtmp, NULL, pb->f_data);
            }
            fcand = status[j].fT;
            ++*stop->nevals_p;
            if (st) ++st->evals_trial;
            if (nla_stop_forced(rs->sp)) { trace_add(pb, fcand, -1, 1, 0); ret = NLOPT_FORCED_STOP; ++j; break; }
            if (fcand < rs->F[worst]) accepted = 1;
            else {
                trace_add(pb, fcand, -1, 1, 0);
                if (nla_stop_evals(stop)) { ret = NLOPT_MAXEVAL_REACHED; ++j; break; }
                if (nla_stop_time(rs->sp)) { ret = NLOPT_MAXTIME_REACHED; ++j; break; }
                kind = 2;
                if (host_eval) {
                    if (ops->mutate_slot(e, blk, rs->os.best) || ops->read_slot(e, blk, 1, rs->xtmp)) { engine_failed(S); return S->ret; }
                    status[j].fM = pb->f((unsigned) n, rs->xtmp, NULL, pb->f_data);
                }
                fcand = status[j].fM;
                ++*stop->nevals_p;
                if (st) { ++st->evals_mutation; if (blk + 1 < S->fresh_from) ++st->slots_role; }
                if (nla_stop_forced(rs->sp)) { trace_add(pb, fcand, -1, 2, 0); ret = NLOPT_FORCED_STOP; j += 2; break; }
                if (fcand < rs->F[worst]) accepted = 1;
                else {
                    trace_add(pb, fcand, -1, 2, 0);
                    if (nla_stop_evals(stop)) { ret = NLOPT_MAXEVAL_REACHED; j += 2; break; }
                    if (nla_stop_time(rs->sp)) { ret = NLOPT_MAXTIME_REACHED; j += 2; break; }
                }
            }
            if (accepted) {
                if (worst == rs->xrow) {
                    if (ops->read_row(e, rs->xrow, rs->x)) { engine_failed(S); return S->ret; }
                    rs->xrow = -1;
                }
                rs->F[worst] = fcand;
                tl_accepted(&S->tl, &rs->os);
                trace_add(pb, fcand, worst, kind, 1);
                if (st) ++st->accepted;
                cblock[ncommit] = blk; ckind[ncommit] = host_eval ? 1 : kind; crow[ncommit] = worst; ++ncommit;
                if (S->forward) S->lastw[worst] = ((blk + 1) << 1) | (kind == 1 ? 1u : 0u);
                if (key_less(rs->F, worst, rs->os.best)) { rs->os.best = worst; best_changed = 1; }
                if (after_accept(rs, blk, host_eval ? 1 : kind)) { engine_failed(S); return S->ret; }
                ret = rs->ret;
            }
            j += (kind == 2) ? 2 : 1;
        }
        S->block += (uint64_t) j;
        if (best_changed) {
            if (st && S->fresh_from > S->block) st->slots_newbest += S->fresh_from - S->block;
            S->fresh_from = S->block;
        }
        if (S->fresh_from < S->block) S->fresh_from = S->block;
        {
            double obs = (j >= K) ? 2.0 * K : (double) j;
            S->runlen = 0.7 * S->runlen + 0.3 * obs;
            if (S->runlen < 1.0) S->runlen = 1.0;
        }
        if (ncommit > 0) {
            int k, m = 0;
            for (k = 0; k < ncommit; ++k) {
                int later = 0, q;
                for (q = k + 1; q < ncommit; ++q) if (crow[q] == crow[k]) { later = 1; break; }
                if (!later) { cblock[m] = cblock[k]; ckind[m] = ckind[k]; crow[m] = crow[k]; ++m; }
            }
            if (ops->commit(e, m, cblock, ckind, crow)) { engine_failed(S); return S->ret; }
        }
        if (st) st->t_walk_s += nla_seconds() - t_walk0;
    }
    if (st) st->t_trial_s += nla_seconds() - t0;
    S->ret = ret;
    return ret;
}

nlopt_result nla_crs_end(nla_crs_session *S, uint64_t *words_used)
{
    nlopt_result ret;
    if (!S) return NLOPT_INVALID_ARGS;
    ret = S->ret;
    if (words_used) *words_used = S->init_words + 2ULL * (uint64_t) S->pb.n * S->block;
    if (ret != NLOPT_FAILURE && S->rs.os.nheap > 0 && S->rs.xrow >= 0 && S->rs.ops->read_row(S->rs.e, S->rs.xrow, S->rs.x)) {
        engine_failed(S);
        ret = S->ret;
    }
    if (S->rs.ops->set_idle) S->rs.ops->set_idle(S->rs.e, NULL, NULL);
    session_free(S);
    return ret;
}

nlopt_result nla_crs_run(const nla_crs_engine_ops *ops, void *e, const nla_crs_problem *pb,
                         double *x, double *minf, uint64_t *words_used)
{
    nlopt_result ret;
    nla_crs_session *S = nla_crs_begin(ops, e, pb, x, minf, &ret);
    if (!S) return ret;
    if (ret == NLOPT_SUCCESS) nla_crs_advance(S, 0);
    return nla_crs_end(S, words_used);
}
```

nlopt_amd/csrc/crs_engine.c:

```c
#include "nla_internal.h"
#include "nla_switches.h"
#include <stdio.h>
#include <stdlib.h>
#include <string.h>

#define INIT_CHUNK_WORDS (1ULL << 28)
#define NLA_KC_MAX 16
#define KCAP 1024
#define OBJK(e) (((e)->obj >= 0 && (e)->sign < 0) ? ((e)->obj | NLA_OBJ_NEGATE) : (e)->obj)
#define NLA_KARG_MAX 128
#define TIME_EVERY 8
#define TIME_EVERY_WINDOW 4
#define ROWPAD 64

typedef struct {
    int64_t index;
    void *ev_ready;
    int waited;
} crs_batch;

#define UPLOAD_BYTES (KCAP * (8 + 8 + 4 + 4 + 4 + 4))
#define CHAIN_KMAX 256
#define CHAIN_FWCAP 48

struct nla_crs_hip_engine {
    int n, ld, obj;
    nla_userobj *user; double sign;
    int32_t *d_list, *h_list;
    double *h_fTM;
    int64_t N;
    int B;
    int variant;
    void *main, *rng;
    nla_mtstream *mts;
    double *d_lb, *d_ub, *d_X, *d_F;
    uint32_t *d_initwords; size_t initwords_cap;
    crs_batch bat[2];
    uint32_t *d_words;
    int32_t *d_jn, *d_pos, *d_last;
    double *d_TX, *d_TM, *d_fT, *d_fM;
    char *d_up, *h_up;
    int32_t *d_tout;
    nla_crs_slot_status *d_status, *h_status;
    int32_t h_t[KCAP];
    int npending;
    int fuse_commit;
    int32_t pend_slot[KCAP], pend_kind[KCAP];
    int64_t pend_row[KCAP];
    void *ev0, *ev1;
    unsigned pass_no; int timed;
    int uncached;
    int direct_status;
    int doorbell;
    uint32_t *h_bell, *d_bellcount, bell_seq;
    void (*idle_fn)(void *); void *idle_arg;
    void *d_ctrl;
    uint32_t ticket_base;
    uint32_t *h_fwcnt, *h_fwrec;
    double *d_Wf;
    int force_upload;
    FILE *pass_log;
    nlopt_amd_stats *stats;
    nlopt_amd_comm *comm;
    int sharded, world, rank, c0, nc, colper;
    int ncopy;
    double *d_csend, *d_crecv;
    int stop_in[2], stop_out[2];
    double *d_gsend, *d_grecv, *h_g;
    const double *h_lb_full, *h_ub_full;
    int shchain, ldf, ncolp;
    int sh_chunks, sh_chunk0, sh_chunks_total;
    uint32_t sh_seq;
    int sh_grid_cap;
    void *d_shared;
    uint32_t *d_flags, *d_stopw;
    void *peer_block[8];
    void *d_table;
    double *d_xbest, *d_lbf, *d_ubf;
    int64_t xbest_row;
    char err[256];
};

#define NLA_CRS_FORWARD_MIN_N 1

#define FAIL(e, ...) do { snprintf((e)->err, sizeof (e)->err, __VA_ARGS__); return -1; } while (0)
#define CK(e, call) do { int rc_ = (call); if (rc_) FAIL(e, "%.160s failed: %s", #call, nla_dev_error_string(rc_)); } while (0)

int nla_crs_can_shard(int n, int world)
{
    if (world < 2) return 0;
    return (int64_t) (world - 1) * ((n + world - 1) / world) < n;
}

static int shchain_colper(int n, int world) { return (((n + world - 1) / world) + 15) & ~15; }
int nla_crs_can_shard_windows(int n, int world)
{
    if (world < 2 || world > 8) return 0;
    return (int64_t) (world - 1) * shchain_colper(n, world) < n;
}

static uint64_t trial_word0(const nla_crs_hip_engine *e) { return 2ULL * (uint64_t) e->n * (uint64_t) (e->N - 1); }

static int prepare_batch(nla_crs_hip_engine *e, crs_batch *b, int64_t index)
{
    const size_t half = (size_t) (index & 1) * (size_t) e->B;
    const uint64_t w0 = trial_word0(e) + 2ULL * (uint64_t) e->n * (uint64_t) index * (uint64_t) e->B;
    uint32_t *words = e->d_words + half * 2 * (size_t) e->n;
    b->index = index;
    b->waited = 0;
    if (nla_mtstream_fill(e->mts, w0, 2ULL * (uint64_t) e->n * (uint64_t) e->B, words))
        FAIL(e, "MT stream fill failed for batch %lld", (long long) index);
    CK(e, nla_k_crs_vitter(e->n, e->N, words, e->B, e->d_jn + half, e->d_pos + half * (size_t) e->n, e->d_last + half, e->rng));
    CK(e, nla_event_record(b->ev_ready, e->rng));
    return 0;
}

static int ensure_blocks(nla_crs_hip_engine *e, uint64_t first, uint64_t last)
{
    const int64_t i0 = (int64_t) (first / (uint64_t) e->B), i1 = (int64_t) (last / (uint64_t) e->B);
    crs_batch *cur = &e->bat[i0 & 1], *nxt = &e->bat[(i0 + 1) & 1];
    if (i1 > i0 + 1) FAIL(e, "window reaches past the prepared batches");
    if (cur->index != i0 && prepare_batch(e, cur, i0)) return -1;
    if (nxt->index != i0 + 1 && prepare_batch(e, nxt, i0 + 1)) return -1;
    if (!cur->waited) { CK(e, nla_stream_wait_event(e->main, cur->ev_ready)); cur->waited = 1; }
    if (i1 > i0 && !nxt->waited) { CK(e, nla_stream_wait_event(e->main, nxt->ev_ready)); nxt->waited = 1; }
    return 0;
}

void nla_crs_hip_engine_destroy(nla_crs_hip_engine *e, uint64_t words_used)
{
    if (!e) return;
    if (e->main) nla_stream_sync(e->main);
    if (e->rng) nla_stream_sync(e->rng);
    if (e->mts) { nla_mtstream_finish(e->mts, words_used); nla_mtstream_destroy(e->mts); }
    if (e->pass_log) fclose(e->pass_log);
    for (int i = 0; i < 2; ++i) nla_event_destroy(e->bat[i].ev_ready);
    nla_dev_free(e->d_words); nla_dev_free(e->d_jn); nla_dev_free(e->d_pos); nla_dev_free(e->d_last);
    nla_dev_free(e->d_lb); nla_dev_free(e->d_ub); nla_dev_free(e->d_X); nla_dev_free(e->d_F);
    nla_dev_free(e->d_initwords);
    if (e->shchain) {
        for (int r = 0; r < 8; ++r) nla_ipc_close(e->peer_block[r]);
        nla_dev_free_uncached(e->d_shared); nla_dev_free_uncached(e->d_TM); nla_dev_free_uncached(e->d_ctrl);
        nla_dev_free(e->d_table); nla_dev_free(e->d_xbest); nla_dev_free(e->d_lbf); nla_dev_free(e->d_ubf);
    } else
    if (e->uncached) { nla_dev_free_uncached(e->d_TX); nla_dev_free_uncached(e->d_TM); nla_dev_free_uncached(e->d_ctrl); }
    else { nla_dev_free(e->d_TX); nla_dev_free(e->d_TM); nla_dev_free(e->d_ctrl); }
    nla_dev_free(e->d_fT);
    nla_dev_free(e->d_up); nla_dev_free(e->d_tout); nla_dev_free(e->d_status);
    nla_dev_free(e->d_list); nla_host_free(e->h_list); nla_host_free(e->h_fTM);
    nla_dev_free(e->d_Wf); nla_host_free(e->h_fwcnt); nla_host_free(e->h_fwrec);
    nla_host_free(e->h_up); nla_host_free(e->h_status); nla_host_free(e->h_bell); nla_dev_free(e->d_bellcount);
    nla_dev_free(e->d_csend); nla_dev_free(e->d_crecv); nla_dev_free(e->d_gsend); nla_dev_free(e->d_grecv); nla_host_free(e->h_g);
    nla_event_destroy(e->ev0); nla_event_destroy(e->ev1);
    if (e->rng != e->main) nla_stream_destroy(e->rng);
    nla_stream_destroy(e->main);
    free(e);
}

static int shchain_setup(nla_crs_hip_engine *e);

nla_crs_hip_engine *nla_crs_hip_engine_create(int n, int64_t N, const double *lb, const double *ub, int obj, int forward,
                                              nlopt_amd_comm *comm, int shard, int cu_parts, nlopt_amd_stats *stats, char **errmsg)
{
    nla_crs_hip_engine *e;
    size_t B;
    (void) errmsg;
    if (nla_dev_count() <= 0) return NULL;
    e = (nla_crs_hip_engine *) calloc(1, sizeof *e);
    if (!e) return NULL;
    e->n = n; e->N = N; e->obj = obj; e->stats = stats; e->comm = comm; e->h_lb_full = lb; e->h_ub_full = ub;
    e->world = nlopt_amd_comm_world(comm); e->rank = nlopt_amd_comm_rank(comm);
    e->sharded = shard && nla_crs_can_shard(n, e->world) && obj >= 0;
    e->shchain = e->sharded && shard == 2 && nla_crs_can_shard_windows(n, e->world);
    e->c0 = 0; e->nc = e->ncopy = n; e->colper = n;
    e->xbest_row = -1;
    e->sh_grid_cap = cu_parts >= 2 ? (224 / cu_parts >= 4 ? 224 / cu_parts : 4) : 0;
    if (e->sharded) {
        e->colper = e->shchain ? shchain_colper(n, e->world) : (n + e->world - 1) / e->world;
        e->c0 = e->rank * e->colper;
        e->nc = n - e->c0 < e->colper ? n - e->c0 : e->colper;
        e->ncopy = e->nc;
        forward = e->shchain;
    }
    e->ld = (e->nc + 15) & ~15;
    e->ldf = e->shchain ? ((n + 15) & ~15) : e->ld;
    e->ncolp = (n >= 128 && (e->nc & 1)) ? e->nc + 1 : e->nc;
    e->bat[0].index = e->bat[1].index = -1;
    {
        const char *lg = NLA_DBG_ENV("NLA_CRS_BATCH_LOG2");
        const int lg2 = lg ? atoi(lg) : 28;
        B = (size_t) ((1ULL << (lg2 >= 20 && lg2 <= 31 ? lg2 : 28)) / (2ULL * (uint64_t) n));
    }
    if (B > 65536) B = 65536;
    if (B < 2 * KCAP) B = 2 * KCAP;
    e->B = (int) B;
    if (NLA_DBG_ENV("NLA_CRS_PASS_LOG")) e->pass_log = fopen(NLA_DBG_ENV("NLA_CRS_PASS_LOG"), "a");
    e->main = cu_parts >= 2 ? nla_stream_create_cu_share(e->rank % cu_parts, cu_parts) : nla_stream_create();
    if (!e->main && cu_parts >= 2) e->main = nla_stream_create();
    e->rng = NLA_DBG_ENV("NLA_ONE_STREAM") ? e->main : nla_stream_create();
    if (!e->main || !e->rng) goto fail;
    e->mts = nla_mtstream_create(e->rng);
    if (!e->mts) goto fail;
    e->d_lb = (double *) nla_dev_malloc(sizeof(double) * (size_t) e->ld);
    e->d_ub = (double *) nla_dev_malloc(sizeof(double) * (size_t) e->ld);
    e->d_X = (double *) nla_dev_malloc(sizeof(double) * (size_t) e->ld * (size_t) (N + ROWPAD));
    e->d_F = (double *) nla_dev_malloc(sizeof(double) * (size_t) (N + ROWPAD));
    e->d_words = (uint32_t *) nla_dev_malloc(sizeof(uint32_t) * 2 * (size_t) n * 2 * B);
    e->d_jn = (int32_t *) nla_dev_malloc(sizeof(int32_t) * 2 * B);
    e->d_last = (int32_t *) nla_dev_malloc(sizeof(int32_t) * 2 * B);
    e->d_pos = (int32_t *) nla_dev_malloc(sizeof(int32_t) * 2 * B * (size_t) n);
    for (int i = 0; i < 2; ++i) {
        e->bat[i].ev_ready = nla_event_create();
        if (!e->bat[i].ev_ready) goto fail;
    }
    e->uncached = (forward && obj >= 0) || NLA_DBG_ENV("NLA_UC_ALWAYS") != NULL;
    if (e->shchain) {
        const size_t txb = sizeof(double) * (size_t) e->ldf * KCAP;
        e->sh_chunks = nla_crs_chain_sh_chunks(n, e->ncolp);
        e->sh_chunks_total = 0;
        for (int r = 0; r < e->world; ++r) {
            const int c0r = r * e->colper, ncr = n - c0r < e->colper ? n - c0r : e->colper;
            if (r == e->rank) e->sh_chunk0 = e->sh_chunks_total;
            e->sh_chunks_total += nla_crs_chain_sh_chunks(n, (n >= 128 && (ncr & 1)) ? ncr + 1 : ncr);
        }
        {
            const size_t flb = (sizeof(uint32_t) * (size_t) CHAIN_KMAX * (size_t) e->sh_chunks_total + 127) & ~(size_t) 127;
            e->d_shared = nla_dev_malloc_uncached(txb + flb + nla_crs_chain_sh_stop_bytes());
            e->d_TX = (double *) e->d_shared;
            e->d_flags = e->d_shared ? (uint32_t *) ((char *) e->d_shared + txb) : NULL;
            e->d_stopw = e->d_shared ? (uint32_t *) ((char *) e->d_shared + txb + flb) : NULL;
            if (e->d_shared && nla_memset(e->d_flags, 0, flb + nla_crs_chain_sh_stop_bytes(), e->main)) goto fail;
        }
        e->d_TM = (double *) nla_dev_malloc_uncached(txb);
        e->d_table = nla_dev_malloc(nla_crs_chain_sh_table_bytes());
        e->d_xbest = (double *) nla_dev_malloc(sizeof(double) * (size_t) e->ldf);
        e->d_lbf = (double *) nla_dev_malloc(sizeof(double) * (size_t) e->ldf);
        e->d_ubf = (double *) nla_dev_malloc(sizeof(double) * (size_t) e->ldf);
    } else {
    e->d_TX = (double *) (e->uncached ? nla_dev_malloc_uncached : nla_dev_malloc)(sizeof(double) * (size_t) e->ld * KCAP);
    e->d_TM = (double *) (e->uncached ? nla_dev_malloc_uncached : nla_dev_malloc)(sizeof(double) * (size_t) e->ld * KCAP);
    }
    e->d_fT = (double *) nla_dev_malloc(sizeof(double) * 2 * KCAP);
    e->d_fM = e->d_fT ? e->d_fT + KCAP : NULL;
    e->d_up = (char *) nla_dev_malloc(UPLOAD_BYTES);
    e->d_tout = (int32_t *) nla_dev_malloc(sizeof(int32_t) * KCAP);
    e->d_status = (nla_crs_slot_status *) nla_dev_malloc(sizeof(nla_crs_slot_status) * (KCAP + 1));
    e->h_up = (char *) nla_host_malloc(UPLOAD_BYTES);
    e->h_status = (nla_crs_slot_status *) nla_host_malloc(sizeof(nla_crs_slot_status) * (KCAP + 1));
    e->ev0 = nla_event_create();
    e->ev1 = nla_event_create();
    if (obj == -2) {
        e->d_list = (int32_t *) nla_dev_malloc(sizeof(int32_t) * KCAP);
        e->h_list = (int32_t *) nla_host_malloc(sizeof(int32_t) * KCAP);
        e->h_fTM = (double *) nla_host_malloc(sizeof(double) * 2 * KCAP);
        if (!e->d_list || !e->h_list || !e->h_fTM) goto fail;
    }
    if (e->uncached && obj >= 0) {
        e->d_ctrl = nla_dev_malloc_uncached(nla_crs_chain_ctrl_bytes(CHAIN_KMAX, CHAIN_KMAX));
        e->d_Wf = (double *) nla_dev_malloc(sizeof(double) * CHAIN_KMAX);
        e->h_fwcnt = (uint32_t *) nla_host_malloc(sizeof(uint32_t) * CHAIN_KMAX);
        e->h_fwrec = (uint32_t *) nla_host_malloc(sizeof(uint32_t) * CHAIN_KMAX * CHAIN_FWCAP);
    }
    e->direct_status = !NLA_DBG_ENV("NLA_CRS_COPY_STATUS");
    e->h_bell = (uint32_t *) nla_host_malloc(64);
    e->d_bellcount = (uint32_t *) nla_dev_malloc(64);
    e->doorbell = 1;
    e->force_upload = NLA_DBG_ENV("NLA_CRS_UPLOAD") != NULL;
    if (!e->d_lb || !e->d_ub || !e->d_X || !e->d_F || !e->d_words || !e->d_jn || !e->d_last || !e->d_pos || !e->d_TX ||
        !e->d_TM || !e->d_fT || !e->d_up || !e->d_tout || !e->d_status || !e->h_up || !e->h_status || !e->h_bell || !e->d_bellcount || !e->ev0 || !e->ev1 ||
        (e->uncached && obj >= 0 && (!e->d_ctrl || !e->d_Wf || !e->h_fwcnt || !e->h_fwrec))) {
        if (e->shchain) shchain_setup(e);
        goto fail;
    }
    if (e->sharded) {
        const size_t cslots = e->shchain ? 1 : 2 * KCAP;
        e->d_csend = (double *) nla_dev_malloc(sizeof(double) * (cslots * (size_t) e->colper + 2));
        e->d_crecv = (double *) nla_dev_malloc(sizeof(double) * (cslots * (size_t) e->colper + 2) * (size_t) e->world);
        e->d_gsend = (double *) nla_dev_malloc(sizeof(double) * (size_t) e->colper);
        e->d_grecv = (double *) nla_dev_malloc(sizeof(double) * (size_t) e->colper * (size_t) e->world);
        e->h_g = (double *) nla_host_malloc(sizeof(double) * (size_t) e->colper * (size_t) e->world);
        if (!e->d_csend || !e->d_crecv || !e->d_gsend || !e->d_grecv || !e->h_g) goto fail;
        {
            size_t big = sizeof(double) * (cslots * (size_t) e->colper + 2), ini = sizeof(double) * (size_t) ((e->N - 1 + e->world - 1) / e->world);
            if (nla_comm_reserve(comm, big > ini ? big : ini)) goto fail;
        }
        if (nla_memset(e->d_gsend, 0, sizeof(double) * (size_t) e->colper, e->main) ||
            nla_memset(e->d_csend, 0, sizeof(double) * (cslots * (size_t) e->colper + 2), e->main)) goto fail;
    }
    *e->h_bell = 0;
    if (nla_memset(e->d_bellcount, 0, 64, e->main)) goto fail;
    if ((e->d_ctrl && nla_memset(e->d_ctrl, 0, nla_crs_chain_ctrl_bytes(CHAIN_KMAX, CHAIN_KMAX), e->main)) ||
        nla_memset(e->d_lb, 0, sizeof(double) * (size_t) e->ld, e->main) || nla_memset(e->d_ub, 0, sizeof(double) * (size_t) e->ld, e->main) ||
        nla_memcpy_h2d(e->d_lb, lb + e->c0, sizeof(double) * (size_t) e->nc, e->main) ||
        nla_memcpy_h2d(e->d_ub, ub + e->c0, sizeof(double) * (size_t) e->nc, e->main) || nla_stream_sync(e->main)) goto fail;
    if (e->shchain && shchain_setup(e)) goto fail;
    return e;
fail:
    nla_crs_hip_engine_destroy(e, 0);
    return NULL;
}

static int shchain_setup(nla_crs_hip_engine *e)
{
    unsigned char mine[NLA_IPC_BYTES], all[8 * NLA_IPC_BYTES];
    void *ptx[8], *pfl[8], *pst[8];
    char *img;
    const size_t txb = sizeof(double) * (size_t) e->ldf * KCAP;
    const size_t flb = (sizeof(uint32_t) * (size_t) CHAIN_KMAX * (size_t) e->sh_chunks_total + 127) & ~(size_t) 127;
    int ok = e->d_shared && e->d_TM && e->d_table && e->d_xbest && e->d_lbf && e->d_ubf && e->d_ctrl && e->main, bad = 0;
    memset(mine, 0, sizeof mine);
    if (ok && (nla_stream_sync(e->main) || nla_ipc_export(e->d_shared, mine))) { ok = 0; memset(mine, 0, sizeof mine); }
    if (nla_comm_allgather_host(e->comm, mine, all, NLA_IPC_BYTES, e->main)) FAIL(e, "exchange of the window buffers' handles failed: %s", nlopt_amd_comm_error(e->comm));
    for (int r = 0; r < e->world; ++r) {
        int zero = 1;
        for (int i = 0; i < NLA_IPC_BYTES; ++i) if (all[r * NLA_IPC_BYTES + i]) { zero = 0; break; }
        if (zero) bad = 1;
    }
    if (!ok || bad) FAIL(e, "%s", ok ? "another rank could not set up its window buffers" : "window buffers: allocation or export failed");
    for (int r = 0; r < e->world; ++r) {
        char *base;
        if (r == e->rank) base = (char *) e->d_shared;
        else {
            e->peer_block[r] = nla_ipc_open(all + r * NLA_IPC_BYTES);
            if (!e->peer_block[r]) { bad = 1; base = (char *) e->d_shared; }
            else base = (char *) e->peer_block[r];
        }
        ptx[r] = base; pfl[r] = base + txb; pst[r] = base + txb + flb;
    }
    if (!nla_comm_agree_ready(e->comm, !bad) || bad) FAIL(e, "%s", bad ? "mapping a peer's window buffers failed (hipIpcOpenMemHandle)" : "another rank could not map the window buffers");
    img = (char *) malloc(nla_crs_chain_sh_table_bytes());
    if (!img) FAIL(e, "out of memory");
    if (nla_crs_chain_sh_table(img, e->world, e->rank, e->c0, e->ldf, e->sh_chunks_total, e->sh_chunk0, ptx, pfl, pst, e->d_xbest, e->d_lbf, e->d_ubf) ||
        nla_memcpy_h2d(e->d_table, img, nla_crs_chain_sh_table_bytes(), e->main) ||
        nla_memset(e->d_lbf, 0, sizeof(double) * (size_t) e->ldf, e->main) || nla_memset(e->d_ubf, 0, sizeof(double) * (size_t) e->ldf, e->main) ||
        nla_memset(e->d_xbest, 0, sizeof(double) * (size_t) e->ldf, e->main) ||
        nla_memcpy_h2d(e->d_lbf, e->h_lb_full, sizeof(double) * (size_t) e->n, e->main) ||
        nla_memcpy_h2d(e->d_ubf, e->h_ub_full, sizeof(double) * (size_t) e->n, e->main) || nla_stream_sync(e->main)) { free(img); FAIL(e, "window table upload failed"); }
    free(img);
    return 0;
}

static void dump_init(nla_crs_hip_engine *e, size_t nwords)
{
    char path[512];
    FILE *fp;
    const size_t nx = (size_t) e->N * (size_t) e->ld;
    int64_t hdr[5] = { e->n, e->ld, e->N, (int64_t) nwords, (int64_t) nla_mtstream_origin(e->mts) };
    uint32_t *w = (uint32_t *) malloc(sizeof(uint32_t) * (nwords ? nwords : 1));
    double *x = (double *) malloc(sizeof(double) * (nx + (size_t) e->N));
    if (w && x && !nla_memcpy_d2h(w, e->d_initwords, sizeof(uint32_t) * nwords, e->main) &&
        !nla_memcpy_d2h(x, e->d_X, sizeof(double) * nx, e->main) && !nla_memcpy_d2h(x + nx, e->d_F, sizeof(double) * (size_t) e->N, e->main) &&
        !nla_stream_sync(e->main)) {
        snprintf(path, sizeof path, "%s/init_last.bin", NLA_DBG_ENV("NLA_CRS_DEBUG_DIR"));
        if ((fp = fopen(path, "wb"))) {
            fwrite(hdr, sizeof hdr, 1, fp); fwrite(w, sizeof(uint32_t), nwords, fp); fwrite(x, sizeof(double), nx + (size_t) e->N, fp);
            fclose(fp);
        }
    }
    free(w); free(x);
}

static int gather_point(nla_crs_hip_engine *e, const double *src, double *x)
{
#define GP(call, what) do { int rc_ = (call); if (rc_) { snprintf(e->err, sizeof e->err, "%s failed: %s", what, nla_dev_error_string(rc_)); nla_comm_abort(e->comm); return -1; } } while (0)
    GP(nla_memcpy_d2d(e->d_gsend, src, sizeof(double) * (size_t) e->nc, e->main), "gather_point: D2D");
    if (nla_comm_allgather_dev(e->comm, e->d_gsend, e->d_grecv, sizeof(double) * (size_t) e->colper, e->main)) {
        nla_comm_abort(e->comm);
        FAIL(e, "all-gather of a point's slices failed: %s", nlopt_amd_comm_error(e->comm));
    }
    GP(nla_memcpy_d2h(e->h_g, e->d_grecv, sizeof(double) * (size_t) e->colper * (size_t) e->world, e->main), "gather_point: D2H");
    GP(nla_stream_sync(e->main), "gather_point: synchronisation");
#undef GP
    for (int r = 0; r < e->world; ++r) {
        const int c0 = r * e->colper, cnt = e->n - c0 < e->colper ? e->n - c0 : e->colper;
        memcpy(x + c0, e->h_g + (size_t) r * (size_t) e->colper, sizeof(double) * (size_t) cnt);
// ... 228 lines not shown
    const int n = e->n;
    const uint32_t ring = 2u * (uint32_t) e->B;
    int32_t t_in[KCAP];
    const int64_t *d_W = NULL;
    const int32_t *d_tin = NULL;
    if (K < 1 || K > KCAP || nW > KCAP || nW < 0) FAIL(e, "bad window K=%d nW=%d", K, nW);
    if (e->shchain) FAIL(e, "this engine was set up for device-resolved windows on a column-sharded population: no conservative passes");
    if (K > op_max_slots(ve, first_block)) FAIL(e, "window reaches past the prepared batches");
    if (ensure_blocks(e, first_block, first_block + (uint64_t) K)) { if (!e->err[0]) snprintf(e->err, sizeof e->err, "batch preparation failed"); return -1; }
    e->timed = (e->n >= 2048 || e->pass_log || (e->pass_no++ % TIME_EVERY) == 0) && e->stats;
#define EVREC(ev) do { if (e->timed) CK(e, nla_event_record((ev), e->main)); } while (0)
    for (int a = 0; a < K; ++a) {
        const uint64_t b = first_block + (uint64_t) a;
        t_in[a] = b >= fresh_from ? 0 : e->h_t[b & (KCAP - 1)];
    }
    if (e->sharded) {
        const int ncol = (e->ld % 2 == 0 && e->nc % 2 != 0) ? e->nc + 1 : e->nc;
        int lerr = 0;
#define SOFT(call) do { if (!lerr) { int rc_ = (call); if (rc_) { lerr = 1; snprintf(e->err, sizeof e->err, "%.160s failed: %s", #call, nla_dev_error_string(rc_)); } } } while (0)
#define HARD(call) do { int rc_ = (call); if (rc_) { if (!lerr) snprintf(e->err, sizeof e->err, "%.160s failed: %s", #call, nla_dev_error_string(rc_)); nla_comm_abort(e->comm); return -1; } } while (0)
        if (upload_and_commit(e, W, nW, t_in, K, &d_W, &d_tin, NULL, NULL)) { lerr = 1; d_tin = e->d_tout; }
        if (nla_dbg_int("NLA_CRS_FAIL_RANK", -1) == e->rank && (int64_t) e->pass_no == (int64_t) nla_dbg_int("NLA_CRS_FAIL_PASS", -1)) {
            lerr = 1; snprintf(e->err, sizeof e->err, "injected failure (NLA_CRS_FAIL_RANK / NLA_CRS_FAIL_PASS)");
        }
        EVREC(e->ev0);
        SOFT(nla_k_crs_advance_cols(n, ncol, e->ld, e->d_X, i0, e->d_jn, e->d_pos, e->d_last, ring, first_block, K, d_W, nW,
                                    d_tin, e->d_tout, KCAP - 1, e->d_lb, e->d_ub, e->d_TX, e->variant, e->main));
        EVREC(e->ev1);
        HARD(nla_k_crs_sh_mutate_pack(n, e->c0, e->nc, e->ld, e->colper, e->d_X, i0, e->d_TX, e->d_TM, e->d_words, ring, first_block, K,
                                      d_tin, e->d_tout, KCAP - 1, e->d_lb, e->d_ub, e->d_csend, lerr ? 2 : e->stop_in[0], e->stop_in[1], e->main));
        if (nla_comm_allgather_dev(e->comm, e->d_csend, e->d_crecv, sizeof(double) * (2 * (size_t) K * (size_t) e->colper + 2), e->main)) {
            nla_comm_abort(e->comm);
            if (!lerr) snprintf(e->err, sizeof e->err, "all-gather of the candidates failed: %s", nlopt_amd_comm_error(e->comm));
            return -1;
        }
        HARD(nla_k_crs_sh_eval(OBJK(e), n, e->colper, first_block, K, d_tin, e->d_tout, KCAP - 1, e->d_crecv, e->world, e->d_fT, e->d_fM, e->d_status, e->main));
        if (e->stats) e->stats->allgather_bytes += (uint64_t) e->world * (2 * (uint64_t) K * (uint64_t) e->colper + 2) * sizeof(double);
        HARD(nla_memcpy_d2h(e->h_status, e->d_status, sizeof(nla_crs_slot_status) * ((size_t) K + 1), e->main));
        if (e->idle_fn) e->idle_fn(e->idle_arg);
        HARD(nla_stream_sync(e->main));
#undef SOFT
#undef HARD
        if (e->h_status[K].t != 0) {
            if (!lerr) snprintf(e->err, sizeof e->err, "another rank failed in the middle of a sharded pass");
            return -1;
        }
        e->stop_out[0] = e->h_status[K].fT != 0.; e->stop_out[1] = e->h_status[K].fM != 0.;
        goto have_status;
    }
    if (K <= NLA_KARG_MAX && nW <= NLA_KARG_MAX && e->npending <= NLA_KARG_MAX && !e->force_upload && e->obj != -2) {
        int fuse = e->fuse_commit && e->npending > 0 && e->npending <= NLA_KC_MAX;
        for (int c = 0; fuse && c < e->npending; ++c)
            for (int a = 0; a < K; ++a)
                if ((int32_t) ((first_block + (uint64_t) a) & (KCAP - 1)) == e->pend_slot[c]) { fuse = 0; break; }
        if (e->npending && !fuse) {
            CK(e, nla_k_crs_commit_args(n, e->ld, e->d_X, e->d_TX, e->d_TM, e->npending, e->pend_slot, e->pend_kind, e->pend_row, e->main));
            e->npending = 0;
        }
        EVREC(e->ev0);
        if (fuse) {
            CK(e, nla_k_crs_advance_commit_args(n, e->ld, e->d_X, i0, e->d_jn, e->d_pos, e->d_last, ring, first_block, K, W, nW,
                                                t_in, e->d_tout, KCAP - 1, e->d_lb, e->d_ub, e->d_TX, e->d_TM, e->npending, e->pend_slot,
                                                e->pend_kind, e->pend_row, e->variant, e->main));
            e->npending = 0;
        } else
        CK(e, nla_k_crs_advance_args(n, e->ld, e->d_X, i0, e->d_jn, e->d_pos, e->d_last, ring, first_block, K, W, nW,
                                     t_in, e->d_tout, KCAP - 1, e->d_lb, e->d_ub, e->d_TX, e->variant, e->main));
        EVREC(e->ev1);
        if (e->direct_status && e->doorbell) {
            const uint32_t seq = ++e->bell_seq ? e->bell_seq : ++e->bell_seq;
            CK(e, nla_k_crs_finish_args_bell(OBJK(e), n, e->ld, e->d_X, i0, e->d_TX, e->d_TM, e->d_words, ring, first_block, K,
                                             t_in, e->d_tout, KCAP - 1, e->d_lb, e->d_ub, e->d_fT, e->d_fM, e->h_status, e->d_bellcount,
                                             e->h_bell, seq, e->main));
            if (e->idle_fn) e->idle_fn(e->idle_arg);
            if (bell_wait(e, seq)) CK(e, nla_stream_sync(e->main));
            goto have_status;
        }
        CK(e, nla_k_crs_finish_args(OBJK(e), n, e->ld, e->d_X, i0, e->d_TX, e->d_TM, e->d_words, ring, first_block, K,
                                    t_in, e->d_tout, KCAP - 1, e->d_lb, e->d_ub, e->d_fT, e->d_fM,
                                    e->direct_status ? e->h_status : e->d_status, e->main));
        if (e->direct_status) {
            if (e->idle_fn) e->idle_fn(e->idle_arg);
            CK(e, nla_stream_sync(e->main));
            goto have_status;
        }
        goto launched;
    }
    if (upload_and_commit(e, W, nW, t_in, K, &d_W, &d_tin, NULL, NULL)) return -1;
    EVREC(e->ev0);
    CK(e, nla_k_crs_advance(n, e->ld, e->d_X, i0, e->d_jn, e->d_pos, e->d_last, ring, first_block, K, d_W, nW,
                            d_tin, e->d_tout, KCAP - 1, e->d_lb, e->d_ub, e->d_TX, e->variant, e->main));
    EVREC(e->ev1);
    CK(e, nla_k_crs_finish(OBJK(e), n, e->ld, e->d_X, i0, e->d_TX, e->d_TM, e->d_words, ring, first_block, K,
                           d_tin, e->d_tout, KCAP - 1, e->d_lb, e->d_ub, e->d_fT, e->d_fM, e->d_status, e->main));
launched:
    if (e->obj == -2) {
        for (int a = 0; a < K; ++a) e->h_list[a] = -(int32_t) (((first_block + (uint64_t) a) & (KCAP - 1)) + 1);
        CK(e, nla_memcpy_h2d(e->d_list, e->h_list, sizeof(int32_t) * (size_t) K, e->main));
        CK(e, nla_userobj_evalgrad_list(e->user, n, e->ld, K, e->d_list, e->d_TX, e->d_fT, NULL, e->sign, e->main));
        CK(e, nla_userobj_evalgrad_list(e->user, n, e->ld, K, e->d_list, e->d_TM, e->d_fM, NULL, e->sign, e->main));
        CK(e, nla_memcpy_d2h(e->h_fTM, e->d_fT, sizeof(double) * 2 * KCAP, e->main));
    }
    CK(e, nla_memcpy_d2h(e->h_status, e->d_status, sizeof(nla_crs_slot_status) * (size_t) K, e->main));
    if (e->idle_fn) e->idle_fn(e->idle_arg);
    CK(e, nla_stream_sync(e->main));
    if (e->obj == -2)
        for (int a = 0; a < K; ++a) {
            const size_t q = (size_t) ((first_block + (uint64_t) a) & (KCAP - 1));
            e->h_status[a].fT = e->h_fTM[q]; e->h_status[a].fM = e->h_fTM[KCAP + q];
        }
have_status:
    memcpy(status, e->h_status, sizeof(nla_crs_slot_status) * (size_t) K);

    for (int a = 0; a < K; ++a) e->h_t[(first_block + (uint64_t) a) & (KCAP - 1)] = status[a].t;
    if (e->timed) {
        float ms = nla_event_elapsed_ms(e->ev0, e->ev1);
        if (ms >= 0) e->stats->t_gather_ms += ms;
        e->stats->gather_launches += 1;
    }
#undef EVREC
    if (e->pass_log) {
        long rows = 0;
        int done_in = 0, fresh = 0, stopped = 0;
        for (int a = 0; a < K; ++a) {
            rows += status[a].t - t_in[a];
            done_in += t_in[a] == n;
            fresh += t_in[a] == 0;
            stopped += status[a].t < n;
        }
        fprintf(e->pass_log, "%d,%d,%d,%d,%d,%d,%ld,%.4f\n", n, K, nW, done_in, fresh, stopped, rows, (double) nla_event_elapsed_ms(e->ev0, e->ev1));
    }
    return 0;
}

static int op_commit(void *ve, int ncommit, const uint64_t *block, const int32_t *kind, const int64_t *row)
{
    nla_crs_hip_engine *e = (nla_crs_hip_engine *) ve;
    if (ncommit <= 0) return 0;
    if (e->npending && flush_commits(e)) return -1;
    if (ncommit > KCAP) FAIL(e, "too many commits");
    for (int c = 0; c < ncommit; ++c) {
        e->pend_slot[c] = (int32_t) (block[c] & (KCAP - 1));
        e->pend_kind[c] = kind[c];
        e->pend_row[c] = row[c];
    }
    e->npending = ncommit;
    return 0;
}

static int op_read_slot(void *ve, uint64_t block, int kind, double *x)
{
    nla_crs_hip_engine *e = (nla_crs_hip_engine *) ve;
    const double *src = (kind == 1 ? e->d_TX : e->d_TM) + (size_t) (block & (KCAP - 1)) * (size_t) e->ld;
    if (e->shchain) {
        const double *whole = (kind == 1 ? e->d_TX : e->d_TM) + (size_t) (block & (KCAP - 1)) * (size_t) e->ldf;
        CK(e, nla_memcpy_d2h(x, whole, sizeof(double) * (size_t) e->n, e->main));
        CK(e, nla_stream_sync(e->main));
        return 0;
    }
    if (flush_commits(e)) return -1;
    if (e->sharded) return gather_point(e, src, x);
    CK(e, nla_memcpy_d2h(x, src, sizeof(double) * (size_t) e->n, e->main));
    CK(e, nla_stream_sync(e->main));
    return 0;
}

static int op_read_row(void *ve, int64_t row, double *x)
{
    nla_crs_hip_engine *e = (nla_crs_hip_engine *) ve;
    if (flush_commits(e)) return -1;
    if (e->sharded) return gather_point(e, e->d_X + (size_t) row * (size_t) e->ld, x);
    CK(e, nla_memcpy_d2h(x, e->d_X + (size_t) row * (size_t) e->ld, sizeof(double) * (size_t) e->n, e->main));
    CK(e, nla_stream_sync(e->main));
    return 0;
}

static int op_mutate_slot(void *ve, uint64_t block, int64_t i0)
{
    nla_crs_hip_engine *e = (nla_crs_hip_engine *) ve;
    const uint32_t ring = 2u * (uint32_t) e->B;
    if (ensure_blocks(e, block, block + 1) || flush_commits(e)) return -1;
    CK(e, nla_k_crs_mutate(e->n, e->d_X + (size_t) i0 * (size_t) e->ld, e->d_TX + (size_t) (block & (KCAP - 1)) * (size_t) e->ld,
                           e->d_words + (size_t) ((block + 1) % ring) * 2 * (size_t) e->n, e->d_lb, e->d_ub, e->main));
    return 0;
}

static int commit_sh(nla_crs_hip_engine *e, void *zero, size_t zero_bytes, int best_slot, int best_kind)
{
    int done = 0, first = 1;
    while (first || done < e->npending) {
        const int cnt = e->npending - done < NLA_KARG_MAX ? e->npending - done : NLA_KARG_MAX;
        CK(e, nla_k_crs_commit_sh(e->nc, e->ld, e->ldf, e->c0, e->d_X, e->d_TX, e->d_TM, cnt, e->pend_slot + done, e->pend_kind + done, e->pend_row + done,
                                  first ? zero : NULL, first ? zero_bytes : 0, e->n, first ? best_slot : -1, best_kind, e->d_xbest, e->main));
        done += cnt; first = 0;
    }
    e->npending = 0;
    return 0;
}

static int op_chain_sh(nla_crs_hip_engine *e, uint64_t first_block, int K, int64_t i0, double f_best, const int64_t *W, const double *Wf, int nW,
                       nla_crs_slot_status *status, uint32_t *fwcnt, uint32_t *fwrec, int fwcap)
{
    const int n = e->n;
    const uint32_t ring = 2u * (uint32_t) e->B;
    const int on_host = nW <= NLA_KARG_MAX;
    const int64_t *d_W = W;
    const double *d_Wf = Wf;
    const size_t zero_bytes = nla_crs_chain_ctrl_bytes(K, nW) - sizeof(uint32_t);
    void *zero = (char *) e->d_ctrl + sizeof(uint32_t);
    int best_slot = -1, best_kind = 0;
    if (i0 != e->xbest_row) {
        for (int c = e->npending - 1; c >= 0; --c)
            if (e->pend_row[c] == i0) { best_slot = e->pend_slot[c]; best_kind = e->pend_kind[c]; break; }
        if (best_slot < 0) {
            if (flush_commits(e)) return -1;
            CK(e, nla_memcpy_d2d(e->d_gsend, e->d_X + (size_t) i0 * (size_t) e->ld, sizeof(double) * (size_t) e->nc, e->main));
            if (nla_comm_allgather_dev(e->comm, e->d_gsend, e->d_grecv, sizeof(double) * (size_t) e->colper, e->main)) {
                nla_comm_abort(e->comm);
                FAIL(e, "all-gather of the best row's slices failed: %s", nlopt_amd_comm_error(e->comm));
            }
            CK(e, nla_memcpy_d2d(e->d_xbest, e->d_grecv, sizeof(double) * (size_t) n, e->main));
        }
        e->xbest_row = i0;
    }
    if (!on_host) {
        memcpy(e->h_up, W, 8 * (size_t) nW); memcpy(e->h_up + 8 * (size_t) nW, Wf, 8 * (size_t) nW);
        CK(e, nla_memcpy_h2d(e->d_up, e->h_up, 16 * (size_t) nW, e->main));
        d_W = (const int64_t *) e->d_up; d_Wf = (const double *) (e->d_up + 8 * (size_t) nW);
    }
    if (commit_sh(e, zero, zero_bytes, best_slot, best_kind)) return -1;
    e->timed = e->stats != NULL;
    if (e->timed) CK(e, nla_event_record(e->ev0, e->main));
    ++e->sh_seq;
    {
        const int rc = nla_k_crs_chain_sh(OBJK(e), n, e->ncolp, e->ld, e->ldf, e->d_X, i0, f_best, e->d_jn, e->d_pos, e->d_last, e->d_words, ring, first_block, K,
                                          d_W, d_Wf, nW, on_host, KCAP - 1, e->d_lb, e->d_ub, e->d_TX, e->d_TM, e->d_ctrl, e->ticket_base, e->h_status,
                                          e->h_fwcnt, e->h_fwrec, fwcap, 1, e->d_table, e->sh_seq, (uint32_t) ((e->stop_in[0] ? 1 : 0) | (e->stop_in[1] ? 2 : 0)), e->sh_grid_cap, e->main);
        if (rc) FAIL(e, "nla_k_crs_chain_sh failed: %s", nla_dev_error_string(rc));
    }
    e->ticket_base += nla_crs_chain_sh_tickets(n, e->ncolp, K, e->sh_grid_cap);
    if (e->timed) CK(e, nla_event_record(e->ev1, e->main));
    if (e->idle_fn) e->idle_fn(e->idle_arg);
    CK(e, nla_stream_sync(e->main));
    if (e->h_status[K].t != 0) FAIL(e, "a rank's share of a trial point did not arrive within 1.5 s (column-sharded window %u)", e->sh_seq);
    e->stop_out[0] = e->h_status[K].fT != 0.; e->stop_out[1] = e->h_status[K].fM != 0.;
    memcpy(status, e->h_status, sizeof(nla_crs_slot_status) * (size_t) K);
    memcpy(fwcnt, e->h_fwcnt, sizeof(uint32_t) * (size_t) K);
    for (int a = 0; a < K; ++a) {
        const uint32_t c = e->h_fwcnt[a] < (uint32_t) fwcap ? e->h_fwcnt[a] : (uint32_t) fwcap;
        if (c) memcpy(fwrec + (size_t) a * (size_t) fwcap, e->h_fwrec + (size_t) a * (size_t) fwcap, sizeof(uint32_t) * (size_t) c);
    }
    for (int a = 0; a < K; ++a) e->h_t[(first_block + (uint64_t) a) & (KCAP - 1)] = n;
    if (e->timed) {
        float ms = nla_event_elapsed_ms(e->ev0, e->ev1);
        if (ms >= 0) e->stats->t_gather_ms += ms;
        e->stats->gather_launches += 1;
        e->stats->allgather_bytes += (uint64_t) K * (uint64_t) (e->world - 1) * (uint64_t) e->ncolp * sizeof(double);
    }
    return 0;
}

static int op_chain(void *ve, uint64_t first_block, int K, int64_t i0, double f_best, const int64_t *W, const double *Wf, int nW,
                    nla_crs_slot_status *status, uint32_t *fwcnt, uint32_t *fwrec, int fwcap)
{
    nla_crs_hip_engine *e = (nla_crs_hip_engine *) ve;
    const int n = e->n;
    const uint32_t ring = 2u * (uint32_t) e->B;
    const int on_host = nW <= NLA_KARG_MAX && !e->force_upload;
    const int64_t *d_W = W;
    const double *d_Wf = Wf;
    if (e->obj < 0 || !e->d_ctrl) FAIL(e, "no device-resolved windows for a host objective");
    if (K < 1 || K > CHAIN_KMAX || nW < 0 || nW > CHAIN_KMAX || fwcap != CHAIN_FWCAP) FAIL(e, "bad window K=%d nW=%d", K, nW);
    if (K > op_max_slots(ve, first_block)) FAIL(e, "window reaches past the prepared batches");
    if (ensure_blocks(e, first_block, first_block + (uint64_t) K)) { if (!e->err[0]) snprintf(e->err, sizeof e->err, "batch preparation failed"); return -1; }
    if (e->shchain) return op_chain_sh(e, first_block, K, i0, f_best, W, Wf, nW, status, fwcnt, fwrec, fwcap);
    {
        const size_t zero_bytes = nla_crs_chain_ctrl_bytes(K, nW) - sizeof(uint32_t);
        void *zero = (char *) e->d_ctrl + sizeof(uint32_t);
        int zeroed = 0;
        if (e->npending && e->npending <= NLA_KARG_MAX && !e->force_upload) {
            CK(e, nla_k_crs_commit_zero(n, e->ld, e->d_X, e->d_TX, e->d_TM, e->npending, e->pend_slot, e->pend_kind, e->pend_row, 1, zero, zero_bytes, e->main));
            e->npending = 0; zeroed = 1;
        }
        if (e->npending || !on_host) {
            const int nc = e->npending, nWu = on_host ? 0 : nW;
            const size_t oW = 0, oF = oW + 8 * (size_t) nWu, oR = oF + 8 * (size_t) nWu, oS = oR + 8 * (size_t) nc, oK = oS + 4 * (size_t) nc;
            const size_t total = oK + 4 * (size_t) nc;
            if (nWu) { memcpy(e->h_up + oW, W, 8 * (size_t) nWu); memcpy(e->h_up + oF, Wf, 8 * (size_t) nWu); }
            if (nc) {
                memcpy(e->h_up + oR, e->pend_row, 8 * (size_t) nc);
                memcpy(e->h_up + oS, e->pend_slot, 4 * (size_t) nc);
                memcpy(e->h_up + oK, e->pend_kind, 4 * (size_t) nc);
            }
            CK(e, nla_memcpy_h2d(e->d_up, e->h_up, total, e->main));
            if (nc) {
                CK(e, nla_k_crs_commit_zero(e->ncopy, e->ld, e->d_X, e->d_TX, e->d_TM, nc, (const int32_t *) (e->d_up + oS), (const int32_t *) (e->d_up + oK),
                                            (const int64_t *) (e->d_up + oR), 0, zero, zero_bytes, e->main));
                e->npending = 0; zeroed = 1;
            }
            if (nWu) { d_W = (const int64_t *) (e->d_up + oW); d_Wf = (const double *) (e->d_up + oF); }
        }
        e->timed = (n >= 2048 || e->pass_log || (e->pass_no++ % TIME_EVERY_WINDOW) == 0) && e->stats;
        if (e->timed) CK(e, nla_event_record(e->ev0, e->main));
        {
            const int rc = nla_k_crs_chain_lean(OBJK(e), n, e->ld, e->d_X, i0, f_best, e->d_jn, e->d_pos, e->d_last, e->d_words, ring, first_block, K, d_W,
                                                d_Wf, nW, on_host, KCAP - 1, e->d_lb, e->d_ub, e->d_TX, e->d_TM, e->d_ctrl, e->ticket_base, e->h_status,
                                                e->h_fwcnt, e->h_fwrec, fwcap, zeroed, e->main);
            if (rc) FAIL(e, "nla_k_crs_chain failed: %s", nla_dev_error_string(rc));
        }
    }
    e->ticket_base += nla_crs_chain_tickets(n, e->ld, K);
    if (e->timed) CK(e, nla_event_record(e->ev1, e->main));
    if (e->idle_fn) e->idle_fn(e->idle_arg);
    CK(e, nla_stream_sync(e->main));
    memcpy(status, e->h_status, sizeof(nla_crs_slot_status) * (size_t) K);
    memcpy(fwcnt, e->h_fwcnt, sizeof(uint32_t) * (size_t) K);
    for (int a = 0; a < K; ++a) {
        const uint32_t c = e->h_fwcnt[a] < (uint32_t) fwcap ? e->h_fwcnt[a] : (uint32_t) fwcap;
        if (c) memcpy(fwrec + (size_t) a * (size_t) fwcap, e->h_fwrec + (size_t) a * (size_t) fwcap, sizeof(uint32_t) * (size_t) c);
    }
    for (int a = 0; a < K; ++a) e->h_t[(first_block + (uint64_t) a) & (KCAP - 1)] = n;
    if (e->timed) {
        float ms = nla_event_elapsed_ms(e->ev0, e->ev1);
        if (ms >= 0) e->stats->t_gather_ms += ms;
        e->stats->gather_launches += 1;
        if (e->pass_log) fprintf(e->pass_log, "%d,%d,%d,%d,%d,%d,%ld,%.4f\n", n, K, nW, 0, K, 0, (long) K * n, (double) ms);
    }
    return 0;
}

static const char *op_last_error(void *ve) { return ((nla_crs_hip_engine *) ve)->err; }
static void op_stop_flags_in(void *ve, int forced, int timed) { nla_crs_hip_engine *e = (nla_crs_hip_engine *) ve; e->stop_in[0] = forced != 0; e->stop_in[1] = timed != 0; }
static void op_stop_flags_out(void *ve, int *forced, int *timed) { nla_crs_hip_engine *e = (nla_crs_hip_engine *) ve; *forced = e->stop_out[0]; *timed = e->stop_out[1]; }

static void op_set_idle(void *ve, void (*fn)(void *), void *arg) { nla_crs_hip_engine *e = (nla_crs_hip_engine *) ve; e->idle_fn = fn; e->idle_arg = arg; }

static int op_reset_slot(void *ve, uint64_t block)
{
    ((nla_crs_hip_engine *) ve)->h_t[block & (KCAP - 1)] = 0;
    return 0;
}

const nla_crs_engine_ops nla_crs_hip_ops = {
    op_init_population, op_max_slots, op_advance, op_chain, op_reset_slot, op_commit, op_read_slot, op_read_row, op_mutate_slot, op_last_error,
    op_stop_flags_in, op_stop_flags_out, op_set_idle
};

static nlopt_result crs_open_common(nlopt_opt opt, int n, nlopt_func f, void *f_data, const double *lb, const double *ub, const double *x,
                                    nla_stopping *stop, int population, nla_crs_problem *pb, nla_crs_hip_engine **eout)
{
    int64_t N = population ? (int64_t) population : 10 * ((int64_t) n + 1);
    nla_userobj *user = NULL;
    double sign = 1.;
    *eout = NULL;
    if (N < n + 1) {
        nla_stop_msg(stop, "population %d should be >= dimension + 1 = %d", (int) N, n + 1);
        return NLOPT_INVALID_ARGS;
    }
    memset(pb, 0, sizeof *pb);
    pb->forward = n >= NLA_CRS_FORWARD_MIN_N;
    pb->n = n; pb->N = N; pb->lb = lb; pb->ub = ub; pb->f = f; pb->f_data = f_data; pb->stop = stop;
    {
        nla_evaluator ev;
        nla_evaluator_resolve(&ev, opt, f, f_data);
        pb->obj = ev.kind == NLA_EVAL_DEVICE ? ev.obj : (ev.kind == NLA_EVAL_USER ? -2 : -1);
        user = ev.user; sign = ev.sign;
    }
    if (opt) {
        pb->trace = opt->trace; pb->trace_cap = opt->trace_cap; pb->trace_len = &opt->trace_len;
        pb->stats = &opt->stats;
        pb->max_spec = (int) nlopt_get_param(opt, "amd_max_spec", 0);
        pb->window_factor = nlopt_get_param(opt, "amd_window_factor", 0);
        pb->forward = nlopt_get_param(opt, "amd_forward", n >= NLA_CRS_FORWARD_MIN_N ? 1 : 0) != 0;
        pb->forward = nla_dbg_int("NLA_CRS_FORWARD", pb->forward);
        if (nlopt_get_param(opt, "amd_host_eval", 0) != 0) pb->obj = -1;
    }
    if (nla_dev_count() <= 0) {
        nla_stop_msg(stop, "nlopt_amd: no HIP device visible (this library has no CPU fallback)");
        nla_comm_agree_ready(opt ? opt->comm : NULL, 0);
        return NLOPT_FAILURE;
    }
    {
        nlopt_amd_comm *comm = opt ? opt->comm : NULL;
        const int shard = comm && nla_crs_can_shard(n, nlopt_amd_comm_world(comm)) && pb->obj >= 0 &&
                          (!opt || nlopt_get_param(opt, "amd_shard", 1) != 0);
        const int windows = shard && pb->forward && pb->max_spec != 1  &&
                            nla_crs_can_shard_windows(n, nlopt_amd_comm_world(comm)) &&
                            (!opt || nlopt_get_param(opt, "amd_shard_windows", 1) != 0);
        const int cu_parts = opt ? (int) nlopt_get_param(opt, "amd_cu_share", 0) : 0;
        if (shard) { pb->comm = comm; if (!windows) pb->forward = 0; }
        *eout = nla_crs_hip_engine_create(n, N, lb, ub, pb->obj, pb->forward, comm, windows ? 2 : shard, windows || !comm ? cu_parts : 0, pb->stats, NULL);
        if (windows) {
            const int all = nla_comm_agree_ready(comm, *eout != NULL);
            if (!all) {
                if (*eout) nla_crs_hip_engine_destroy(*eout, 0);
                pb->forward = 0;
                *eout = nla_crs_hip_engine_create(n, N, lb, ub, pb->obj, 0, comm, 1, 0, pb->stats, NULL);
            }
        }
        if (*eout) { (*eout)->fuse_commit = 1; (*eout)->doorbell = 1; }
    }
    if (opt && nlopt_amd_comm_world(opt->comm) > 1) {
        const int all = nla_comm_agree_same(opt->comm, *eout != NULL, nla_problem_fingerprint(NLOPT_GN_CRS2_LM, n, (int) N, pb->obj, lb, ub, x, stop) + nla_params_fingerprint(opt));
        if (all <= 0 && *eout) {
            nla_crs_hip_engine_destroy(*eout, 0); *eout = NULL;
            if (all < 0) { nla_stop_msg(stop, NLA_MSG_RANKS_DIFFER); return NLOPT_INVALID_ARGS; }
            nla_stop_msg(stop, "nlopt_amd: another rank could not set up its device engine");
            return NLOPT_FAILURE;
        }
    }
    if (!*eout) {
        nla_stop_msg(stop, "nlopt_amd: could not create the device engine (out of device memory?)");
        return NLOPT_OUT_OF_MEMORY;
    }
    (*eout)->user = user; (*eout)->sign = sign;
    (*eout)->variant = 0;
    return NLOPT_SUCCESS;
}

nlopt_result nla_crs_minimize(nlopt_opt opt, int n, nlopt_func f, void *f_data, const double *lb, const double *ub,
                              double *x, double *minf, nla_stopping *stop, int population)
{
    nla_crs_problem pb;
    nla_crs_hip_engine *e;
    nlopt_result ret;
    uint64_t words = 0;
    ret = crs_open_common(opt, n, f, f_data, lb, ub, x, stop, population, &pb, &e);
    if (ret != NLOPT_SUCCESS) return ret;
    ret = nla_crs_run(&nla_crs_hip_ops, e, &pb, x, minf, &words);
    if (pb.stats) pb.stats->mt_words = words;
    nla_crs_hip_engine_destroy(e, words);
    return ret;
}

struct nlopt_amd_crs_session {
    nlopt_opt opt;
    nla_stopping stop;
    nla_crs_problem pb;
    nla_crs_hip_engine *e;
    nla_crs_session *S;
    nlopt_result ret;
};

nlopt_result nla_setup_run(nlopt_opt opt, double *x, double *minf, nla_stopping *stop);

nlopt_amd_crs_session *nlopt_amd_crs_open(nlopt_opt opt, double *x, double *minf, nlopt_result *ret_out)
{
    nlopt_amd_crs_session *h;
    nlopt_result ret;
    int pop;
    nla_unset_errmsg(opt);
    if (!opt || opt->algorithm != NLOPT_GN_CRS2_LM || opt->maximize) { if (ret_out) *ret_out = NLOPT_INVALID_ARGS; return NULL; }
    h = (nlopt_amd_crs_session *) calloc(1, sizeof *h);
    if (!h) { if (ret_out) *ret_out = NLOPT_OUT_OF_MEMORY; return NULL; }
    h->opt = opt;
    nlopt_set_force_stop(opt, 0);
    ret = nla_setup_run(opt, x, minf, &h->stop);
    if (ret == NLOPT_SUCCESS) {
        pop = opt->stochastic_population > 0 ? (int) opt->stochastic_population
                                             : (nla_stochastic_population > 0 ? nla_stochastic_population : 0);
        ret = crs_open_common(opt, (int) opt->n, opt->f, opt->f_data, opt->lb, opt->ub, x, &h->stop, pop, &h->pb, &h->e);
    }
    if (ret != NLOPT_SUCCESS) { if (ret_out) *ret_out = ret; free(h); return NULL; }
    h->S = nla_crs_begin(&nla_crs_hip_ops, h->e, &h->pb, x, minf, &ret);
    h->ret = ret;
    if (ret_out) *ret_out = ret;
    if (!h->S) { nla_crs_hip_engine_destroy(h->e, 0); free(h); return NULL; }
    return h;
}

nlopt_result nlopt_amd_crs_step(nlopt_amd_crs_session *h, long eval_budget)
{
    if (!h || !h->S) return NLOPT_INVALID_ARGS;
    if (h->ret == NLOPT_SUCCESS) h->ret = nla_crs_advance(h->S, (int64_t) eval_budget);
    return h->ret;
}

nlopt_result nlopt_amd_crs_close(nlopt_amd_crs_session *h)
{
    nlopt_result ret;
    uint64_t words = 0;
    if (!h) return NLOPT_INVALID_ARGS;
    ret = nla_crs_end(h->S, &words);
    if (h->pb.stats) h->pb.stats->mt_words = words;
    nla_crs_hip_engine_destroy(h->e, words);
    free(h);
    return ret;
}
```

nlopt_amd/csrc/hip/crs_chain.hip:

```cpp
#include "crs_common.h"
#include "../nla_switches.h"
#include <stdlib.h>
#include "../../../include/nlopt_amd.h"

#define NLA_CHAIN_LIGHT_BELOW 2048
#define CH_EXTRA 32
#define CH_FWAVES 8
#include <stddef.h>
#include <string.h>

struct chain_ctrl {
    uint32_t ticket, lock, next, halt, naccept, wp, nextra, pk;
    double xf[CH_EXTRA]; int64_t xrow[CH_EXTRA];
};

#include "crs_chain_resolver.h"
static_assert(offsetof(chain_ctrl, next) == 4 * CH_CTRL_NEXT && offsetof(chain_ctrl, halt) == 4 * CH_CTRL_HALT && offsetof(chain_ctrl, naccept) == 4 * CH_CTRL_NACCEPT &&
              offsetof(chain_ctrl, wp) == 4 * CH_CTRL_WP && offsetof(chain_ctrl, nextra) == 4 * CH_CTRL_NEXTRA && offsetof(chain_ctrl, pk) == 4 * CH_CTRL_PK &&
              sizeof(chain_ctrl) % 16 == 0, "crs_chain_resolver.h addresses the control block by word");

#define NLA_KA_MAX 128
struct chain_lists { int inl; int64_t W[NLA_KA_MAX]; double Wf[NLA_KA_MAX]; };

__device__ __forceinline__ uint32_t ld_agent(const uint32_t *p) { return __hip_atomic_load(p, __ATOMIC_RELAXED, __HIP_MEMORY_SCOPE_AGENT); }
__device__ __forceinline__ void st_agent(uint32_t *p, uint32_t v) { __hip_atomic_store(p, v, __ATOMIC_RELAXED, __HIP_MEMORY_SCOPE_AGENT); }
__device__ __forceinline__ uint32_t ld_sys(const uint32_t *p) { return __hip_atomic_load(p, __ATOMIC_RELAXED, __HIP_MEMORY_SCOPE_SYSTEM); }
__device__ __forceinline__ void st_sys(uint32_t *p, uint32_t v) { __hip_atomic_store(p, v, __ATOMIC_RELAXED, __HIP_MEMORY_SCOPE_SYSTEM); }
__device__ __forceinline__ void st_sys_f64(double *p, double v)
{
    __hip_atomic_store(reinterpret_cast<uint64_t *>(p), (uint64_t) __double_as_longlong(v), __ATOMIC_RELAXED, __HIP_MEMORY_SCOPE_SYSTEM);
}

#define NLA_SH_MAXW 8
struct chain_shard {
    int world, rank, c0, ldf, chunks_total, chunk0, pad0, pad1;
    double *peerTX[NLA_SH_MAXW];
    uint32_t *peerflags[NLA_SH_MAXW];
    uint32_t *peerstop[NLA_SH_MAXW];
    const double *xbest, *lbf, *ubf;
};
#define NLA_SH_WAIT_TICKS 150000000ull

template <int VEC, int U, int WAVES, int OBJ, bool SH = false>
__global__ __launch_bounds__(WAVES * 64) void crs_chain_kernel(
    const chain_lists L_first_kernel_argument,
    int n, int ld, const double *__restrict__ X, int64_t i0, double f_best, const int32_t *__restrict__ jn_ring,
    const int32_t *__restrict__ pos_ring, const int32_t *__restrict__ last_ring, const uint32_t *__restrict__ words_ring,
    uint32_t ring_blocks, uint64_t first_block, int K, const int64_t *__restrict__ Wd, const double *__restrict__ Wfd, int nW,
    int slot_mask, int chunks, const double *__restrict__ lb, const double *__restrict__ ub, double *__restrict__ TX,
    double *__restrict__ TM, chain_ctrl *__restrict__ ctrl, uint32_t ticket_base, nla_crs_slot_status *__restrict__ status,
    uint32_t *__restrict__ fwcnt, uint32_t *__restrict__ fwrec, int fwcap, double sign, uint64_t resolver_timeout,
    int ncols, const chain_shard *__restrict__ S, uint32_t seq, uint32_t stopbits)
{
    typedef const __attribute__((address_space(4))) chain_lists *kernarg_lists;
    const kernarg_lists Lk = (kernarg_lists) __builtin_amdgcn_kernarg_segment_ptr();
    (void) L_first_kernel_argument;
    typedef typename VecT<VEC>::T V;
    static_assert(U <= 64, "one lane per row of a batch");
    __shared__ V sacc[64];
    __shared__ int32_t srow[NLA_ADV_RCAP];
    __shared__ int s_turn, s_ticket, s_last, s_state;
    __shared__ uint32_t s_nrec, s_halt;
    __shared__ double scratch[2 * CH_FWAVES];
    volatile __attribute__((address_space(3))) int *turn = (volatile __attribute__((address_space(3))) int *) &s_turn;
    const int lane = threadIdx.x & 63;
    const int wave = __builtin_amdgcn_readfirstlane((int) (threadIdx.x >> 6));
    double *fv = reinterpret_cast<double *>(ctrl + 1);
    uint32_t *done = reinterpret_cast<uint32_t *>(fv + 2 * (size_t) K), *rowstate = done + 2 * (size_t) K;
    const int64_t *W = Lk->inl ? (const int64_t *) Lk->W : Wd;
    const double *Wf = Lk->inl ? (const double *) Lk->Wf : Wfd;
#define CH_NEXT do { if constexpr (SH) continue; else return; } while (0)
    for (;;) {
    if constexpr (SH) __syncthreads();
    if (threadIdx.x == 0) { s_ticket = (int) (atomicAdd(&ctrl->ticket, 1u) - ticket_base); s_nrec = 0; s_halt = ld_agent(&ctrl->halt); }
    __syncthreads();
    if constexpr (SH) { if (s_ticket > K * chunks) return; }
    if (s_ticket == 0) {
        if (wave == 0) {
            if constexpr (SH) {
                if (lane < S->world) st_sys(S->peerstop[lane] + (seq & 1u) * NLA_SH_MAXW + (uint32_t) S->rank, (seq << 2) | (stopbits & 3u));
            }
            chain_resolver_wave(reinterpret_cast<uint32_t *>(ctrl), reinterpret_cast<const uint64_t *>(fv), rowstate, K, nW, W, Wf, f_best, i0,
                                resolver_timeout, !SH && n < NLA_CHAIN_LIGHT_BELOW);
            if constexpr (SH) {
                uint32_t bits = 0, bad = 0;
                if (lane < S->world) {
                    const uint32_t *wp_ = S->peerstop[S->rank] + (seq & 1u) * NLA_SH_MAXW + (uint32_t) lane;
                    const uint64_t t0 = wall_clock64();
                    uint32_t v;
                    while (((v = ld_sys(wp_)) >> 2) != seq) {
                        if (wall_clock64() - t0 > NLA_SH_WAIT_TICKS) { bad = 1; break; }
                        __builtin_amdgcn_s_sleep(8);
                    }
                    bits = v & 3u;
                }
                const uint32_t forced = __ballot((bits & 1u) != 0) != 0, timed = __ballot((bits & 2u) != 0) != 0;
                const uint32_t failed = (__ballot(bad != 0) != 0 || ld_agent(&ctrl->lock) != 0) ? 1u : 0u;
                if (lane == 0) { status[K].fT = forced ? 1. : 0.; status[K].fM = timed ? 1. : 0.; status[K].t = (int32_t) failed; status[K].pad = 0; }
            }
        }
        return;
    }
    const int wg = s_ticket - 1;
    const int a = wg / chunks, chunk = wg % chunks;
    {
        const uint32_t h = s_halt;
        if ((h & 2u) && (uint32_t) a >= (h >> 8)) {
            if (threadIdx.x == 0) { status[a].t = 0; if (chunk == 0) fwcnt[a] = 0; }
            CH_NEXT;
        }
    }
    const uint64_t block = first_block + (uint64_t) a;
    const uint32_t rb = (uint32_t) (block % ring_blocks);
    const int q = (int) (block & (uint64_t) slot_mask);
    const int32_t *p = pos_ring + (size_t) rb * (size_t) n;
    const int jn = jn_ring[rb];
    const int64_t rbase = p[n - 1];
    int64_t al = rbase + (rbase >= i0 ? 1 : 0) + (int64_t) last_ring[rb];
    al += (al == i0) ? 1 : 0;
    auto pick_row = [&](int t) -> int32_t {
        int64_t r;
        if (t < n - 1) { r = p[t]; r += (r >= i0 ? 1 : 0); } else r = al;
        return (int32_t) r;
    };
    const int nun = a < nW ? a : nW;
    auto mark_hazards = [&](int cnt) {
        int hit[(256 + 63) / 64];
#pragma unroll
        for (int it = 0; it < (256 + 63) / 64; ++it) {
            const int j = it * 64 + lane;
            hit[it] = -1;
            if (j < nun) {
                const int64_t r = W[j];
                int lo = 0, hi = cnt - 1;
                while (r != i0 && lo <= hi) {
                    const int mid = (lo + hi) >> 1;
                    const int32_t pv = srow[mid];
                    if (pv == (int32_t) r) { hit[it] = mid; break; }
                    if (pv < (int32_t) r) lo = mid + 1; else hi = mid - 1;
                }
            }
        }
        asm volatile("s_waitcnt lgkmcnt(0)" ::: "memory");
#pragma unroll
        for (int it = 0; it < (256 + 63) / 64; ++it)
            if (hit[it] >= 0) srow[hit[it]] = -(it * 64 + lane + 1);
    };
    const int col = (chunk * 64 + lane) * VEC;
    const bool active = col < (SH ? ncols : n);
    const size_t colc = active ? (size_t) col : 0;
    const double *Xc = X + colc;
    const size_t tld = SH ? (size_t) S->ldf : (size_t) ld;
    const size_t tc0 = SH ? (size_t) S->c0 : 0;
    double *accrow = TX + (size_t) q * tld + tc0 + colc;
    if (wave == 0) sacc[lane] = ldv<VEC>(Xc + (size_t) i0 * (size_t) ld);
    const double hneg = -(0.5 * n);
    const uint32_t lane_off = (uint32_t) (colc * sizeof(double));
    V v[U];
    for (int seg0 = 0; seg0 < n; seg0 += NLA_ADV_RCAP) {
        const int cnt = (n - seg0 < NLA_ADV_RCAP) ? n - seg0 : NLA_ADV_RCAP;
        nla_lds_barrier();
        for (int i = threadIdx.x; i < cnt; i += WAVES * 64) srow[i] = pick_row(seg0 + i);
        nla_lds_barrier();
        if (wave == 0 && nun > 0) mark_hazards(cnt);
        if (threadIdx.x == 0) *turn = 0;
        nla_lds_barrier();
        const int nb = (cnt + U - 1) / U;
        auto issue = [&](int b) {
            const int base = b * U;
            const int mine = base + lane < cnt ? base + lane : cnt - 1;
            const int32_t myrow = srow[mine];
#pragma unroll
            for (int u = 0; u < U; ++u) {
                const int64_t r = (int64_t) __builtin_amdgcn_readlane(myrow, u);
                const char *rowp = reinterpret_cast<const char *>(X + (size_t) r * (size_t) ld);
                if (r < 0) {
                    const int j = (int) (-r - 1);
                    uint32_t rs;
                    for (;;) {
                        rs = ld_agent(&rowstate[j]);
                        if (rs) break;
                        const uint32_t pk = ld_agent(&ctrl->pk);
                        if ((int32_t) (((pk & 0xffffu) - (uint32_t) a) & ((pk >> 16) - (uint32_t) (a - j))) >= 0) { rs = ld_agent(&rowstate[j]); break; }
                        __builtin_amdgcn_s_sleep(4);
                    }
                    __builtin_amdgcn_fence(__ATOMIC_ACQUIRE, "wavefront");
                    int pj = 0, kind = 0;
                    if (rs && (int) (rs >> 3) < a) {
                        pj = (int) (rs >> 3); kind = (int) ((rs >> 1) & 3u);
                        const int qk = (int) ((first_block + (uint64_t) pj) & (uint64_t) slot_mask);
                        rowp = reinterpret_cast<const char *>((kind == 1 ? TX : TM) + (size_t) qk * tld + tc0);
                    } else rowp = reinterpret_cast<const char *>(X + (size_t) W[j] * (size_t) ld);
                    if (chunk == 0 && lane == 0 && base + u < cnt) {
                        const uint32_t k = atomicAdd(&s_nrec, 1u);
                        if ((int) k < fwcap) fwrec[(size_t) a * (size_t) fwcap + k] = (uint32_t) j | ((uint32_t) pj << 8) | ((uint32_t) kind << 16);
                    }
                }
                v[u] = *reinterpret_cast<const V *>(rowp + lane_off);
            }
        };
        if (wave < nb) issue(wave);
        for (int ph = wave; ph < nb; ph += WAVES) {
            while (*turn != ph) __builtin_amdgcn_s_sleep(1);
            asm volatile("" ::: "memory");
            V acc = sacc[lane];
            const int base = ph * U, tb = seg0 + base;
            if (base + U <= cnt && !(jn >= tb && jn < tb + U)) {
#pragma unroll
                for (int u = 0; u < U; ++u) add_row(acc, v[u]);
            } else {
#pragma unroll
                for (int u = 0; u < U; ++u)
                    if (base + u < cnt) acc_row(acc, v[u], (tb + u == jn) ? hneg : 1.0);
            }
            sacc[lane] = acc;
            asm volatile("s_waitcnt lgkmcnt(0)" ::: "memory");
            if (lane == 0) *turn = ph + 1;
            if (ph + WAVES < nb) issue(ph + WAVES);
        }
        if (wave == 0) {
            while (*turn != nb) __builtin_amdgcn_s_sleep(1);
            asm volatile("" ::: "memory");
        }
    }
    if (wave == 0 && active) {
        V acc = sacc[lane];
        const double s = 2.0 / n;
        double rx, ry = 0.;
        if constexpr (VEC == 1) {
            double a0 = *reinterpret_cast<double *>(&acc);
            rx = nla_clamp_box(a0 * s, lb[col], ub[col]);
            *accrow = rx;
        } else {
            double2 a2 = *reinterpret_cast<double2 *>(&acc), r2;
            r2.x = rx = nla_clamp_box(a2.x * s, lb[col], ub[col]);
            r2.y = ry = nla_clamp_box(a2.y * s, lb[col + 1], ub[col + 1]);
            *reinterpret_cast<double2 *>(accrow) = r2;
        }
        if constexpr (SH) {
            const int me = S->rank, Wn = S->world;
            for (int r = 0; r < Wn; ++r) {
                if (r == me) continue;
                double *dst = S->peerTX[r] + (size_t) q * tld + tc0 + colc;
                st_sys_f64(dst, rx);
                if constexpr (VEC == 2) st_sys_f64(dst + 1, ry);
            }
        }
        (void) ry;
        asm volatile("s_waitcnt vmcnt(0)" ::: "memory");
    }
    __syncthreads();
    if constexpr (SH) {
        if (threadIdx.x < (unsigned) S->world)
            st_sys(S->peerflags[threadIdx.x] + (size_t) a * (size_t) S->chunks_total + (size_t) (S->chunk0 + chunk), seq << 2);
    }
    if (threadIdx.x == 0) {
        if (chunk == 0) fwcnt[a] = s_nrec;
        s_last = (atomicAdd(&done[a], 1u) == (uint32_t) (chunks - 1));
    }
    __syncthreads();
    if (!s_last) CH_NEXT;
    if constexpr (SH) {
        if (wave == 0) {
            const uint32_t *fl = S->peerflags[S->rank] + (size_t) a * (size_t) S->chunks_total;
            const int nch = S->chunks_total;
            const uint64_t t0 = wall_clock64();
            int state = 0;
            while (!state) {
                bool all = true;
                for (int c = lane; c < nch; c += 64) all = all && ((int32_t) (ld_sys(fl + c) - (seq << 2)) >= 0);
                if (__ballot(!all) == 0) state = 1;
                else {
                    const uint32_t h = ld_agent(&ctrl->halt);
                    if ((h & 2u) && (uint32_t) a >= (h >> 8)) state = 2;
                    else if (wall_clock64() - t0 > NLA_SH_WAIT_TICKS) state = 3;
                    else __builtin_amdgcn_s_sleep(4);
                }
            }
            if (lane == 0) s_state = state;
        }
        __syncthreads();
        if (s_state != 1) {
            if (threadIdx.x == 0) {
                status[a].t = 0;
                if (s_state == 3) st_agent(&ctrl->lock, 1u);
            }
            CH_NEXT;
        }
        __builtin_amdgcn_fence(__ATOMIC_ACQUIRE, "");
    } else
    {
        if (n < NLA_CHAIN_LIGHT_BELOW) __builtin_amdgcn_fence(__ATOMIC_ACQUIRE, "workgroup");
        else __builtin_amdgcn_fence(__ATOMIC_ACQUIRE, "agent");
    }
    {
        const int tid = threadIdx.x;
        const double *x = TX + (size_t) q * tld;
        const double *xb = SH ? S->xbest : X + (size_t) i0 * (size_t) ld;
        const double *lbm = SH ? S->lbf : lb, *ubm = SH ? S->ubf : ub;
        const uint32_t *w = words_ring + (size_t) ((block + 1) % ring_blocks) * 2 * (size_t) n;
        double *m = TM + (size_t) q * tld;
        auto getx = [&](int i) { return __builtin_nontemporal_load(x + i); };
        const double fT = sign * nla_block_objective_as<OBJ, WAVES, CH_FWAVES>(n, getx, scratch);
        uint64_t *rec = reinterpret_cast<uint64_t *>(fv) + 2 * (size_t) a;
#ifndef NLA_CHAIN_LATE_FT
        if (tid == 0) __hip_atomic_store(rec, ch_bits_of_f(fT), __ATOMIC_RELAXED, __HIP_MEMORY_SCOPE_AGENT);
#endif
        auto mut = [&](int i) {
            const uint2 ww = *reinterpret_cast<const uint2 *>(w + 2 * i);
            const double wv = nla_urand_from(0., 1., ww.x, ww.y);
            return nla_clamp_box(xb[i] * (1 + wv) - wv * getx(i), lbm[i], ubm[i]);
        };
        for (int i = tid; i < n; i += WAVES * 64) m[i] = mut(i);
        const double fM = sign * nla_block_objective_as<OBJ, WAVES, CH_FWAVES>(n, mut, scratch);
        asm volatile("s_waitcnt vmcnt(0)" ::: "memory");
        __syncthreads();
        if (tid == 0) {
            status[a].fT = fT; status[a].fM = fM; status[a].t = n; status[a].pad = 0;
#ifdef NLA_CHAIN_LATE_FT
            __hip_atomic_store(rec, ch_bits_of_f(fT), __ATOMIC_RELAXED, __HIP_MEMORY_SCOPE_AGENT);
#endif
            __hip_atomic_store(rec + 1, ch_bits_of_f(fM), __ATOMIC_RELAXED, __HIP_MEMORY_SCOPE_AGENT);
        }
    }
    if constexpr (!SH) return;
    }
#undef CH_NEXT
}

extern "C" size_t nla_crs_chain_ctrl_bytes(int K, int nW)
{
    return sizeof(chain_ctrl) + sizeof(double) * 2 * (size_t) K + sizeof(uint32_t) * (2 * (size_t) K + (size_t) nW + 8);
}

static bool chain_vec2(int n, int ld)
{
    static int force1 = -1;
    if (force1 < 0) { const char *s = NLA_DBG_ENV("NLA_CHAIN_VEC1"); force1 = (s && atoi(s) > 0) ? 1 : 0; }
    return !force1 && (n % 2 == 0) && (ld % 2 == 0) && n >= 128;
}

extern "C" int nla_crs_chain_chunks(int n, int ld)
{
    const bool vec2 = chain_vec2(n, ld);
    const int cpw = vec2 ? 128 : 64;
    return (n + cpw - 1) / cpw;
}

extern "C" uint32_t nla_crs_chain_tickets(int n, int ld, int K)
{
    return (uint32_t) nla_crs_chain_chunks(n, ld) * (uint32_t) K + 1u;
}

extern "C" int nla_k_crs_chain_lean(int obj, int n, int ld, const double *X, int64_t i0, double f_best, const int32_t *jn_ring,
                                    const int32_t *pos_ring, const int32_t *last_ring, const uint32_t *words_ring, uint32_t ring_blocks,
                                    uint64_t first_block, int K, const int64_t *W, const double *Wf, int nW, int w_on_host, int slot_mask,
                                    const double *lb, const double *ub, double *TX, double *TM, void *ctrl, uint32_t ticket_base,
                                    nla_crs_slot_status *status, uint32_t *fwcnt, uint32_t *fwrec, int fwcap, int ctrl_is_zero, void *stream);
extern "C" int nla_k_crs_chain(int obj, int n, int ld, const double *X, int64_t i0, double f_best, const int32_t *jn_ring,
                               const int32_t *pos_ring, const int32_t *last_ring, const uint32_t *words_ring, uint32_t ring_blocks,
                               uint64_t first_block, int K, const int64_t *W, const double *Wf, int nW, int w_on_host, int slot_mask,
                               const double *lb, const double *ub, double *TX, double *TM, void *ctrl, uint32_t ticket_base,
                               nla_crs_slot_status *status, uint32_t *fwcnt, uint32_t *fwrec, int fwcap, void *stream)
{
    return nla_k_crs_chain_lean(obj, n, ld, X, i0, f_best, jn_ring, pos_ring, last_ring, words_ring, ring_blocks, first_block, K, W, Wf, nW, w_on_host,
                                slot_mask, lb, ub, TX, TM, ctrl, ticket_base, status, fwcnt, fwrec, fwcap, 0, stream);
}

static int chain_launch(int obj, int n, int ld, const double *X, int64_t i0, double f_best, const int32_t *jn_ring,
                        const int32_t *pos_ring, const int32_t *last_ring, const uint32_t *words_ring, uint32_t ring_blocks,
                        uint64_t first_block, int K, const int64_t *W, const double *Wf, int nW, int w_on_host, int slot_mask,
                        const double *lb, const double *ub, double *TX, double *TM, void *ctrl, uint32_t ticket_base,
                        nla_crs_slot_status *status, uint32_t *fwcnt, uint32_t *fwrec, int fwcap, int ctrl_is_zero, void *stream,
                        int ncols, const chain_shard *S, int ldf, uint32_t seq, uint32_t stopbits, int grid_cap);
extern "C" int nla_k_crs_chain_lean(int obj, int n, int ld, const double *X, int64_t i0, double f_best, const int32_t *jn_ring,
                                    const int32_t *pos_ring, const int32_t *last_ring, const uint32_t *words_ring, uint32_t ring_blocks,
                                    uint64_t first_block, int K, const int64_t *W, const double *Wf, int nW, int w_on_host, int slot_mask,
                                    const double *lb, const double *ub, double *TX, double *TM, void *ctrl, uint32_t ticket_base,
                                    nla_crs_slot_status *status, uint32_t *fwcnt, uint32_t *fwrec, int fwcap, int ctrl_is_zero, void *stream)
{
    return chain_launch(obj, n, ld, X, i0, f_best, jn_ring, pos_ring, last_ring, words_ring, ring_blocks, first_block, K, W, Wf, nW, w_on_host, slot_mask,
                        lb, ub, TX, TM, ctrl, ticket_base, status, fwcnt, fwrec, fwcap, ctrl_is_zero, stream, n, nullptr, ld, 0u, 0u, 0);
}

extern "C" int nla_crs_chain_sh_chunks(int n, int ncols)
{
    const int cpw = (n >= 128 && ncols % 2 == 0) ? 128 : 64;
    return (ncols + cpw - 1) / cpw;
}
extern "C" size_t nla_crs_chain_sh_table_bytes(void) { return sizeof(chain_shard); }
extern "C" int nla_crs_chain_sh_table(void *host_image, int world, int rank, int c0, int ldf, int chunks_total, int chunk0, void *const *peerTX,
                                      void *const *peerflags, void *const *peerstop, const double *xbest, const double *lbf, const double *ubf)
{
    if (world < 2 || world > NLA_SH_MAXW || rank < 0 || rank >= world) return (int) hipErrorInvalidValue;
    chain_shard t;
    memset(&t, 0, sizeof t);
    t.world = world; t.rank = rank; t.c0 = c0; t.ldf = ldf; t.chunks_total = chunks_total; t.chunk0 = chunk0;
    for (int r = 0; r < world; ++r) { t.peerTX[r] = (double *) peerTX[r]; t.peerflags[r] = (uint32_t *) peerflags[r]; t.peerstop[r] = (uint32_t *) peerstop[r]; }
    t.xbest = xbest; t.lbf = lbf; t.ubf = ubf;
    memcpy(host_image, &t, sizeof t);
    return 0;
}
extern "C" size_t nla_crs_chain_sh_stop_bytes(void) { return sizeof(uint32_t) * 2 * NLA_SH_MAXW; }
extern "C" int nla_k_crs_chain_sh(int obj, int n, int ncols, int ld, int ldf, const double *X, int64_t i0, double f_best, const int32_t *jn_ring,
                                  const int32_t *pos_ring, const int32_t *last_ring, const uint32_t *words_ring, uint32_t ring_blocks,
                                  uint64_t first_block, int K, const int64_t *W, const double *Wf, int nW, int w_on_host, int slot_mask,
                                  const double *lb, const double *ub, double *TX, double *TM, void *ctrl, uint32_t ticket_base,
                                  nla_crs_slot_status *status, uint32_t *fwcnt, uint32_t *fwrec, int fwcap, int ctrl_is_zero,
                                  const void *table, uint32_t seq, uint32_t stopbits, int grid_cap, void *stream)
{
    if (!table || ncols < 1 || ncols > ld || ldf < n || ldf % 16 != 0) return (int) hipErrorInvalidValue;
    return chain_launch(obj, n, ld, X, i0, f_best, jn_ring, pos_ring, last_ring, words_ring, ring_blocks, first_block, K, W, Wf, nW, w_on_host, slot_mask,
                        lb, ub, TX, TM, ctrl, ticket_base, status, fwcnt, fwrec, fwcap, ctrl_is_zero, stream, ncols, (const chain_shard *) table, ldf, seq, stopbits, grid_cap);
}
static unsigned chain_sh_grid(int n, int ncols, int K, int grid_cap)
{
    const long total = (long) nla_crs_chain_sh_chunks(n, ncols) * K + 1;
    return (unsigned) ((grid_cap >= 2 && grid_cap < total) ? grid_cap : total);
}
extern "C" uint32_t nla_crs_chain_sh_tickets(int n, int ncols, int K, int grid_cap)
{
    return (uint32_t) nla_crs_chain_sh_chunks(n, ncols) * (uint32_t) K + chain_sh_grid(n, ncols, K, grid_cap);
}

static int chain_launch(int obj, int n, int ld, const double *X, int64_t i0, double f_best, const int32_t *jn_ring,
                        const int32_t *pos_ring, const int32_t *last_ring, const uint32_t *words_ring, uint32_t ring_blocks,
                        uint64_t first_block, int K, const int64_t *W, const double *Wf, int nW, int w_on_host, int slot_mask,
                        const double *lb, const double *ub, double *TX, double *TM, void *ctrl, uint32_t ticket_base,
                        nla_crs_slot_status *status, uint32_t *fwcnt, uint32_t *fwrec, int fwcap, int ctrl_is_zero, void *stream,
                        int ncols, const chain_shard *S, int ldf, uint32_t seq, uint32_t stopbits, int grid_cap)
{
    if (K <= 0) return 0;
    if (K > 256 || nW > 256 || nW < 0 || obj < 0) return (int) hipErrorInvalidValue;
    const double sign = nla_obj_sign(&obj);
    if (ld % 16 != 0 || ((uintptr_t) TX | (uintptr_t) TM) % 128 != 0) return (int) hipErrorInvalidValue;
    (void) ldf;
    hipStream_t st = (hipStream_t) stream;
    chain_lists L;
    L.inl = 0;
    if (w_on_host) {
        if (nW > NLA_KA_MAX) return (int) hipErrorInvalidValue;
        L.inl = 1;
        for (int j = 0; j < nW; ++j) { L.W[j] = W[j]; L.Wf[j] = Wf[j]; }
        W = nullptr; Wf = nullptr;
    }
    const bool sh = S != nullptr;
    const bool vec2 = sh ? (n >= 128 && ncols % 2 == 0 && ld % 2 == 0) : chain_vec2(n, ld);
    const int chunks = sh ? nla_crs_chain_sh_chunks(n, ncols) : nla_crs_chain_chunks(n, ld);
    if (sh && (ldf % 16 != 0)) return (int) hipErrorInvalidValue;
    const dim3 grid(sh ? chain_sh_grid(n, ncols, K, grid_cap) : (unsigned) ((long) chunks * K) + 1u);
    const uint64_t res_timeout = 200000000ull;
    chain_ctrl *c = (chain_ctrl *) ctrl;
    if (!ctrl_is_zero) {
        hipError_t e = hipMemsetAsync((char *) ctrl + sizeof(uint32_t), 0, nla_crs_chain_ctrl_bytes(K, nW) - sizeof(uint32_t), st);
        if (e != hipSuccess) return (int) e;
    }
#define CHAIN(VEC, UU, WV, O) hipLaunchKernelGGL((crs_chain_kernel<VEC, UU, WV, O>), grid, dim3(WV * 64), 0, st, L, n, ld, X, i0, f_best, jn_ring, \
        pos_ring, last_ring, words_ring, ring_blocks, first_block, K, W, Wf, nW, slot_mask, chunks, lb, ub, TX, TM, c, ticket_base, status,         \
        fwcnt, fwrec, fwcap, sign, res_timeout, ncols, S, seq, stopbits)
#define CHAIN_SH(VEC, UU, WV, O) hipLaunchKernelGGL((crs_chain_kernel<VEC, UU, WV, O, true>), grid, dim3(WV * 64), 0, st, L, n, ld, X, i0, f_best, jn_ring, \
        pos_ring, last_ring, words_ring, ring_blocks, first_block, K, W, Wf, nW, slot_mask, chunks, lb, ub, TX, TM, c, ticket_base, status,         \
        fwcnt, fwrec, fwcap, sign, res_timeout, ncols, S, seq, stopbits)
#ifndef NLA_CHAIN_MID_W
#define NLA_CHAIN_MID_W 8
#endif
#ifndef NLA_CHAIN_MID_U
#define NLA_CHAIN_MID_U 32
#endif
#ifndef NLA_CHAIN_LOW_W
#define NLA_CHAIN_LOW_W 4
#endif
#ifndef NLA_CHAIN_LOW_U
#define NLA_CHAIN_LOW_U 16
#endif
#ifndef NLA_CHAIN_TINY_W
#define NLA_CHAIN_TINY_W 4
#endif
#define CHAIN_SHAPE(O)                                                                   \
    if (vec2) {                                                                          \
        if (n >= 2048) CHAIN(2, 32, 8, O); else if (n >= 512) CHAIN(2, NLA_CHAIN_MID_U, NLA_CHAIN_MID_W, O); else CHAIN(2, NLA_CHAIN_LOW_U, NLA_CHAIN_LOW_W, O); \
    } else {                                                                             \
        if (n >= 2048) CHAIN(1, 32, 8, O); else if (n >= 512) CHAIN(1, NLA_CHAIN_MID_U, NLA_CHAIN_MID_W, O); else if (n >= 128) CHAIN(1, NLA_CHAIN_LOW_U, NLA_CHAIN_LOW_W, O); else CHAIN(1, 16, NLA_CHAIN_TINY_W, O); \
    }
#define CHAIN_SHAPE_SH(O)                                                                \
    if (vec2) { if (n >= 512) CHAIN_SH(2, 32, 8, O); else CHAIN_SH(2, 16, 4, O); } else CHAIN_SH(1, 16, 4, O);
    if (sh) { NLA_OBJ_DISPATCH(obj, CHAIN_SHAPE_SH) }
    else { NLA_OBJ_DISPATCH(obj, CHAIN_SHAPE) }
#undef CHAIN_SHAPE_SH
#undef CHAIN_SH
#undef CHAIN_SHAPE
#undef CHAIN
    NLA_LAUNCH_CHECK();
    return 0;
}
```

nlopt_amd/csrc/hip/crs_chain_resolver.h:

```cpp
#ifndef NLA_CRS_CHAIN_RESOLVER_H
#define NLA_CRS_CHAIN_RESOLVER_H

#ifndef CH_EXTRA
#define CH_EXTRA 32
#endif

#ifndef CH_PRIMITIVES_DEFINED
#define CH_DEV __device__ __forceinline__
CH_DEV int ch_lane() { return (int) (threadIdx.x & 63u); }
CH_DEV uint64_t ch_ballot(bool p) { return __ballot(p); }
CH_DEV uint64_t ch_readlane_u64(uint64_t v, uint32_t l)
{
    const int ls = __builtin_amdgcn_readfirstlane((int) l);
    const uint32_t lo = (uint32_t) __builtin_amdgcn_readlane((int) (uint32_t) v, ls), hi = (uint32_t) __builtin_amdgcn_readlane((int) (uint32_t) (v >> 32), ls);
    return (uint64_t) lo | ((uint64_t) hi << 32);
}
CH_DEV uint64_t ch_shuffle_u64(uint64_t v, uint32_t src)
{
    const uint32_t lo = (uint32_t) __builtin_amdgcn_ds_bpermute((int) (src << 2), (int) (uint32_t) v);
    const uint32_t hi = (uint32_t) __builtin_amdgcn_ds_bpermute((int) (src << 2), (int) (uint32_t) (v >> 32));
    return (uint64_t) lo | ((uint64_t) hi << 32);
}
CH_DEV uint64_t ch_ld64(const uint64_t *p) { return __hip_atomic_load(p, __ATOMIC_RELAXED, __HIP_MEMORY_SCOPE_AGENT); }
CH_DEV void ch_st32(uint32_t *p, uint32_t v) { __hip_atomic_store(p, v, __ATOMIC_RELAXED, __HIP_MEMORY_SCOPE_AGENT); }
CH_DEV void ch_release() { __builtin_amdgcn_fence(__ATOMIC_RELEASE, "agent"); }
CH_DEV void ch_landed() { asm volatile("s_waitcnt vmcnt(0)" ::: "memory"); }
CH_DEV void ch_sleep() { __builtin_amdgcn_s_sleep(2); }
CH_DEV uint64_t ch_clock() { return (uint64_t) wall_clock64(); }
CH_DEV double ch_f_of_bits(uint64_t b) { return __longlong_as_double((long long) ~b); }
#endif

#ifdef CH_PRIMITIVES_DEFINED
CH_DEV void ch_landed() { ch_release(); }
#endif

CH_DEV uint64_t ch_bits_of_f(double f)
{
    uint64_t b;
    __builtin_memcpy(&b, &f, sizeof b);
    b = ~b;
    return b ? b : 1ull;
}

CH_DEV uint32_t ch_rowstate_word(int kind, uint32_t slot) { return 1u | ((uint32_t) kind << 1) | (slot << 3); }

#define CH_CTRL_NEXT 2
#define CH_CTRL_HALT 3
#define CH_CTRL_NACCEPT 4
#define CH_CTRL_WP 5
#define CH_CTRL_NEXTRA 6
#define CH_CTRL_PK 7

CH_DEV void chain_resolver_wave(uint32_t *ctrl_words, const uint64_t *recs, uint32_t *rowstate, int K, int nW,
                                const int64_t *W, const double *Wf, double f_best, int64_t i0, uint64_t timeout, bool light = false)
{
    const int lane = ch_lane();
    uint32_t next = 0, wp = 0, nextra = 0, naccept = 0, halt = 0, idle = 0;
    uint64_t xfb = 0;
    int64_t xrow = 0;
    uint64_t wfb[4];
    int64_t wrow[4];
    for (int q = 0; q < 4; ++q) {
        const int idx = lane + 64 * q;
        double f = 0.;
        wrow[q] = -1;
        if (idx < nW) { f = Wf[idx]; wrow[q] = W[idx]; }
        __builtin_memcpy(&wfb[q], &f, sizeof f);
    }
    auto list_f = [&](uint32_t idx) {
        const uint32_t q = idx >> 6;
        const uint64_t v = q == 0 ? wfb[0] : q == 1 ? wfb[1] : q == 2 ? wfb[2] : wfb[3];
        return ch_f_of_bits(~ch_readlane_u64(v, idx & 63u));
    };
    auto list_row = [&](uint32_t idx) {
        const uint32_t q = idx >> 6;
        const int64_t v = q == 0 ? wrow[0] : q == 1 ? wrow[1] : q == 2 ? wrow[2] : wrow[3];
        return (int64_t) ch_readlane_u64((uint64_t) v, idx & 63u);
    };
    const double f_last = nW > 0 ? list_f((uint32_t) nW - 1u) : 0.;
    const int64_t r_last = nW > 0 ? list_row((uint32_t) nW - 1u) : -1;
    uint64_t t0 = ch_clock();
    while (next < (uint32_t) K && !halt) {
        const uint32_t s = next + (uint32_t) lane;
        uint64_t rt = 0, rm = 0;
        if (s < (uint32_t) K) { rt = ch_ld64(recs + 2 * (size_t) s); rm = ch_ld64(recs + 2 * (size_t) s + 1); }
        const uint64_t ok = ch_ballot(rt != 0);
        const uint32_t run = (ok == ~0ull) ? 64u : (uint32_t) __builtin_ctzll(~ok);
        if (run == 0) {
            if ((++idle & 255u) == 0 && ch_clock() - t0 > timeout) { halt = 1; break; }
            ch_sleep();
            continue;
        }
        uint32_t i = 0;
        while (i < run && !halt) {
#ifndef NLA_CHAIN_NO_FASTSTEP
            if (nextra == 0 && wp < (uint32_t) nW) {
                const uint32_t rel = (uint32_t) lane - i;
                const bool in = (uint32_t) lane >= i && (uint32_t) lane < run && wp + rel < (uint32_t) nW;
                const uint32_t idx = wp + (in ? rel : 0u);
                const uint32_t q0 = wp >> 6;
                const uint64_t va = q0 == 0 ? wfb[0] : q0 == 1 ? wfb[1] : q0 == 2 ? wfb[2] : wfb[3];
                uint64_t fwb = ch_shuffle_u64(va, idx & 63u);
                if ((wp & 63u) + (run - i) > 64u) {
                    const uint64_t vb = q0 == 0 ? wfb[1] : q0 == 1 ? wfb[2] : wfb[3];
                    const uint64_t fb2 = ch_shuffle_u64(vb, idx & 63u);
                    if ((idx >> 6) != q0) fwb = fb2;
                }
                const double fw_l = ch_f_of_bits(~fwb), fT_l = ch_f_of_bits(rt);
                const bool ok = in && fT_l < fw_l && !(fT_l >= f_last) && !(fT_l <= f_best);
                const uint64_t m = ch_ballot(ok) >> i;
                const uint32_t P = (m == ~0ull) ? 64u : (uint32_t) __builtin_ctzll(~m);
                if (P) {
                    if ((uint32_t) lane >= i && (uint32_t) lane < i + P) ch_st32(&rowstate[wp + rel], ch_rowstate_word(1, next + (uint32_t) lane));
                    wp += P; naccept += P; i += P;
                    if (i >= run) break;
                }
            }
#endif
            const uint32_t j = next + i;
            const double fT = ch_f_of_bits(ch_readlane_u64(rt, i));
            const uint64_t rmi = ch_readlane_u64(rm, i);
            const double fM = ch_f_of_bits(rmi);
            double fw = -__builtin_huge_val();
            int64_t rw = -1;
            int xi = -1;
            if (wp < (uint32_t) nW) { fw = list_f(wp); rw = list_row(wp); }
            for (uint32_t e = 0; e < nextra; ++e) {
                const double xe = ch_f_of_bits(~ch_readlane_u64(xfb, e));
                const int64_t re = (int64_t) ch_readlane_u64((uint64_t) xrow, e);
                if (rw < 0 || xe > fw || (xe == fw && re > rw)) { fw = xe; rw = re; xi = (int) e; }
            }
            if (rw < 0) { halt = 1; break; }
            int kind = 0;
            double fnew = 0;
            if (fT < fw) { kind = 1; fnew = fT; }
            else if (rmi == 0) break;
            else if (fM < fw) { kind = 2; fnew = fM; }
            if (kind) {
                if (xi >= 0) {
                    const uint64_t lf = ch_readlane_u64(xfb, nextra - 1);
                    const int64_t lr = (int64_t) ch_readlane_u64((uint64_t) xrow, nextra - 1);
                    if (lane == xi) { xfb = lf; xrow = lr; }
                    --nextra;
                } else {
                    if (lane == 0) ch_st32(&rowstate[wp], ch_rowstate_word(kind, j));
                    ++wp;
                }
                ++naccept;
                if (nW > 0 && (fnew > f_last || (fnew == f_last && rw > r_last))) {
                    if (nextra == CH_EXTRA) halt = 1;
                    else {
                        uint64_t fb;
                        __builtin_memcpy(&fb, &fnew, sizeof fb);
                        if (lane == (int) nextra) { xfb = fb; xrow = rw; }
                        ++nextra;
                    }
                }
                if (fnew < f_best || (fnew == f_best && rw < i0)) {
                    halt = 2u | ((j + 1u) << 8);
                    if (lane == 0) ch_st32(&ctrl_words[CH_CTRL_HALT], halt);
                }
            }
            i += (kind == 1) ? 1u : 2u;
        }
        if (i == 0 && !halt) {
            if ((++idle & 255u) == 0 && ch_clock() - t0 > timeout) { halt = 1; break; }
            ch_sleep();
            continue;
        }
        next += i;
        idle = 0;
        t0 = ch_clock();
        if (halt) break;
        if (light) ch_landed(); else ch_release();
        if (lane == 0) {
            ch_st32(&ctrl_words[CH_CTRL_NEXT], next);
            ch_st32(&ctrl_words[CH_CTRL_PK], next | ((next - wp) << 16));
        }
    }
    if (light) ch_landed(); else ch_release();
    if (lane == 0) {
        if (halt) { ch_st32(&ctrl_words[CH_CTRL_NEXT], (uint32_t) K + 2u); ch_st32(&ctrl_words[CH_CTRL_PK], 0xffffffffu); }
        ch_st32(&ctrl_words[CH_CTRL_HALT], halt);
        ch_st32(&ctrl_words[CH_CTRL_NACCEPT], naccept);
        ch_st32(&ctrl_words[CH_CTRL_WP], wp);
        ch_st32(&ctrl_words[CH_CTRL_NEXTRA], nextra);
    }
}

#endif
```

Measured before the change: 45240 evals/s.

## Add persistent chain kernel with early abandonment of dead CRS slots

Adds a persistent-grid variant of the CRS chain kernel, where workgroups loop over tickets, plus an optional abandonment path. When the resolver finds a slot's trial rejected or a new best halting later slots, it marks following slots dead, and in-flight chunks poll that flag and leave early to save gather and eval work. Abandonment is off by default, but the persistent grid is chosen whenever the cap allows, and the driver uses the new entry point when it is present. It adds polling overhead and more complex completion accounting through left-counters in the done words.

```diff
diff --git a/include/nlopt_amd.h b/include/nlopt_amd.h
--- a/include/nlopt_amd.h
+++ b/include/nlopt_amd.h
@@ -66,6 +66,7 @@
     uint64_t cobyla_host_searches;
     uint64_t lbfgs_longest_chain_steps;
     uint64_t mlsl_gate_timeouts;
+    uint64_t slots_abandoned, slots_abandoned_recomputed;
 } nlopt_amd_stats;
 nlopt_result nlopt_amd_get_stats(const nlopt_opt opt, nlopt_amd_stats *out);
 size_t nlopt_amd_get_stats_sized(const nlopt_opt opt, void *out, size_t bytes);
@@ -153,6 +154,13 @@
                         const int32_t *h_slot, const int32_t *h_kind, const int64_t *h_row, void *zero, size_t zero_bytes,
                         int n, int best_slot, int best_kind, double *xbest, void *stream);
 uint32_t nla_crs_chain_tickets(int n, int ld, int K);
+int nla_k_crs_chain_wgs(int obj, int n, int ld, const double *X, int64_t i0, double f_best, const int32_t *jn_ring,
+                        const int32_t *pos_ring, const int32_t *last_ring, const uint32_t *words_ring, uint32_t ring_blocks,
+                        uint64_t first_block, int K, const int64_t *W, const double *Wf, int nW, int w_on_host, int slot_mask,
+                        const double *lb, const double *ub, double *TX, double *TM, void *ctrl, uint32_t ticket_base,
+                        nla_crs_slot_status *status, uint32_t *fwcnt, uint32_t *fwrec, int fwcap, int ctrl_is_zero, int wgs, int abandon,
+                        void *stream) __attribute__((weak));
+uint32_t nla_crs_chain_tickets_wgs(int n, int ld, int K, int wgs) __attribute__((weak));
 
 int nla_k_crs_finish(int obj, int n, int ld, const double *X, int64_t i0, const double *TX, double *TM,
                      const uint32_t *words_ring, uint32_t ring_blocks, uint64_t first_block, int K,
diff --git a/nlopt_amd/__init__.py b/nlopt_amd/__init__.py
--- a/nlopt_amd/__init__.py
+++ b/nlopt_amd/__init__.py
@@ -32,7 +32,8 @@
                 ("evolve_rounds_enqueued", C.c_uint64), ("evolve_rounds", C.c_uint64),
                 ("t_engine_s", C.c_double), ("t_walk_s", C.c_double),
                 ("list_refreshes", C.c_uint64), ("list_refreshes_beside_device", C.c_uint64), ("t_list_refresh_s", C.c_double),
-                ("isres_gate_timeouts", C.c_uint64), ("mlsl_sampled_ahead", C.c_uint64), ("cobyla_host_searches", C.c_uint64), ("lbfgs_longest_chain_steps", C.c_uint64), ("mlsl_gate_timeouts", C.c_uint64)]
+                ("isres_gate_timeouts", C.c_uint64), ("mlsl_sampled_ahead", C.c_uint64), ("cobyla_host_searches", C.c_uint64), ("lbfgs_longest_chain_steps", C.c_uint64), ("mlsl_gate_timeouts", C.c_uint64),
+                ("slots_abandoned", C.c_uint64), ("slots_abandoned_recomputed", C.c_uint64)]
 
     def asdict(self):
         return {k: getattr(self, k) for k, _ in self._fields_}
diff --git a/nlopt_amd/csrc/api_options.c b/nlopt_amd/csrc/api_options.c
--- a/nlopt_amd/csrc/api_options.c
+++ b/nlopt_amd/csrc/api_options.c
@@ -139,7 +139,7 @@
     len = strnlen(name, 1024) + 1;
     if (len > 1024) return fail_msg(opt, NLOPT_INVALID_ARGS, "parameter name must be < 1024 bytes");
     if (!strncmp(name, "amd_", 4)) {
-        static const char *const known[] = { "amd_forward", "amd_shard", "amd_shard_windows", "amd_cu_share", "amd_max_spec", "amd_window_factor", "amd_host_eval",
+        static const char *const known[] = { "amd_forward", "amd_shard", "amd_shard_windows", "amd_cu_share", "amd_max_spec", "amd_chain_wgs", "amd_chain_abandon", "amd_window_factor", "amd_host_eval",
                                              "amd_exact_dot", "amd_isres_evolve_serial", "amd_isres_overlap", "amd_lbfgs_streaming", "amd_mlsl_seg_regens", "amd_cobyla_host", "amd_cobyla_min_batch", NULL };
         int k;
         for (k = 0; known[k] && strcmp(name, known[k]); ++k) { }
diff --git a/nlopt_amd/csrc/crs_driver.c b/nlopt_amd/csrc/crs_driver.c
--- a/nlopt_amd/csrc/crs_driver.c
+++ b/nlopt_amd/csrc/crs_driver.c
@@ -498,6 +498,10 @@
                 const int32_t tnew = status[a].t;
                 if (b >= S->fresh_from) ++st->slots_launched;
                 if (tnew > told && timed_pass) st->gather_bytes += 8ULL * (uint64_t) n * (uint64_t) (tnew - told + (told == 0 ? 1 : 0));
+                if (S->forward && tnew == 0 && status[a].pad > 0) {
+                    if ((status[a].pad & 3) == 1) ++st->slots_abandoned;
+                    if (timed_pass) st->gather_bytes += 8ULL * (uint64_t) n * (uint64_t) (status[a].pad >> 2);
+                }
                 S->tprev[b % TRING] = tnew;
             }
         }
@@ -509,7 +513,10 @@
             double fcand;
             const uint64_t blk = S->block + (uint64_t) j;
             if (best_changed) break;
-            if (status[j].t < n) break;
+            if (status[j].t < n) {
+                if (st && S->forward && status[j].pad > 0 && (status[j].pad & 3) == 1) ++st->slots_abandoned_recomputed;
+                break;
+            }
             if (S->forward) {
                 const uint32_t cnt = S->fwcnt[j];
                 int ok = cnt <= FWCAP;
diff --git a/nlopt_amd/csrc/crs_engine.c b/nlopt_amd/csrc/crs_engine.c
--- a/nlopt_amd/csrc/crs_engine.c
+++ b/nlopt_amd/csrc/crs_engine.c
@@ -20,6 +20,9 @@
 } crs_batch;
 
 #define UPLOAD_BYTES (KCAP * (8 + 8 + 4 + 4 + 4 + 4))
+#ifndef NLA_CHAIN_ABANDON_DEFAULT
+#define NLA_CHAIN_ABANDON_DEFAULT 0
+#endif
 #define CHAIN_KMAX 256
 #define CHAIN_FWCAP 48
 
@@ -71,6 +74,7 @@
     int shchain, ldf, ncolp;
     int sh_chunks, sh_chunk0, sh_chunks_total;
     uint32_t sh_seq;
+    int chain_wgs, chain_abandon;
     int sh_grid_cap;
     void *d_shared;
     uint32_t *d_flags, *d_stopw;
@@ -905,14 +909,20 @@
         }
         e->timed = (n >= 2048 || e->pass_log || (e->pass_no++ % TIME_EVERY_WINDOW) == 0) && e->stats;
         if (e->timed) CK(e, nla_event_record(e->ev0, e->main));
-        {
+        if (nla_k_crs_chain_wgs && nla_crs_chain_tickets_wgs) {
+            const int rc = nla_k_crs_chain_wgs(OBJK(e), n, e->ld, e->d_X, i0, f_best, e->d_jn, e->d_pos, e->d_last, e->d_words, ring, first_block, K, d_W,
+                                               d_Wf, nW, on_host, KCAP - 1, e->d_lb, e->d_ub, e->d_TX, e->d_TM, e->d_ctrl, e->ticket_base, e->h_status,
+                                               e->h_fwcnt, e->h_fwrec, fwcap, zeroed, e->chain_wgs, e->chain_abandon, e->main);
+            if (rc) FAIL(e, "nla_k_crs_chain_wgs failed: %s", nla_dev_error_string(rc));
+            e->ticket_base += nla_crs_chain_tickets_wgs(n, e->ld, K, e->chain_wgs);
+        } else {
             const int rc = nla_k_crs_chain_lean(OBJK(e), n, e->ld, e->d_X, i0, f_best, e->d_jn, e->d_pos, e->d_last, e->d_words, ring, first_block, K, d_W,
                                                 d_Wf, nW, on_host, KCAP - 1, e->d_lb, e->d_ub, e->d_TX, e->d_TM, e->d_ctrl, e->ticket_base, e->h_status,
                                                 e->h_fwcnt, e->h_fwrec, fwcap, zeroed, e->main);
             if (rc) FAIL(e, "nla_k_crs_chain failed: %s", nla_dev_error_string(rc));
-        }
-    }
-    e->ticket_base += nla_crs_chain_tickets(n, e->ld, K);
+            e->ticket_base += nla_crs_chain_tickets(n, e->ld, K);
+        }
+    }
     if (e->timed) CK(e, nla_event_record(e->ev1, e->main));
     if (e->idle_fn) e->idle_fn(e->idle_arg);
     CK(e, nla_stream_sync(e->main));
@@ -1001,6 +1011,12 @@
                 *eout = nla_crs_hip_engine_create(n, N, lb, ub, pb->obj, 0, comm, 1, 0, pb->stats, NULL);
             }
         }
+        if (*eout) {
+            int wgs = (int) nlopt_get_param(opt, "amd_chain_wgs", 0);
+            wgs = nla_dbg_int("NLA_CHAIN_WGS", wgs);
+            (*eout)->chain_wgs = (wgs < -1 || wgs == 1) ? 0 : wgs;
+            (*eout)->chain_abandon = nla_dbg_int("NLA_CHAIN_ABANDON", opt ? nlopt_get_param(opt, "amd_chain_abandon", NLA_CHAIN_ABANDON_DEFAULT) != 0 : NLA_CHAIN_ABANDON_DEFAULT);
+        }
         if (*eout) { (*eout)->fuse_commit = 1; (*eout)->doorbell = 1; }
     }
     if (opt && nlopt_amd_comm_world(opt->comm) > 1) {
diff --git a/nlopt_amd/csrc/hip/crs_chain.hip b/nlopt_amd/csrc/hip/crs_chain.hip
--- a/nlopt_amd/csrc/hip/crs_chain.hip
+++ b/nlopt_amd/csrc/hip/crs_chain.hip
@@ -14,6 +14,7 @@
     double xf[CH_EXTRA]; int64_t xrow[CH_EXTRA];
 };
 
+#define CH_LEFT 0x10000u
 #include "crs_chain_resolver.h"
 static_assert(offsetof(chain_ctrl, next) == 4 * CH_CTRL_NEXT && offsetof(chain_ctrl, halt) == 4 * CH_CTRL_HALT && offsetof(chain_ctrl, naccept) == 4 * CH_CTRL_NACCEPT &&
               offsetof(chain_ctrl, wp) == 4 * CH_CTRL_WP && offsetof(chain_ctrl, nextra) == 4 * CH_CTRL_NEXTRA && offsetof(chain_ctrl, pk) == 4 * CH_CTRL_PK &&
@@ -41,7 +42,7 @@
 };
 #define NLA_SH_WAIT_TICKS 150000000ull
 
-template <int VEC, int U, int WAVES, int OBJ, bool SH = false>
+template <int VEC, int U, int WAVES, int OBJ, bool SH = false, bool PERSIST = false>
 __global__ __launch_bounds__(WAVES * 64) void crs_chain_kernel(
     const chain_lists L_first_kernel_argument,
     int n, int ld, const double *__restrict__ X, int64_t i0, double f_best, const int32_t *__restrict__ jn_ring,
@@ -50,7 +51,7 @@
     int slot_mask, int chunks, const double *__restrict__ lb, const double *__restrict__ ub, double *__restrict__ TX,
     double *__restrict__ TM, chain_ctrl *__restrict__ ctrl, uint32_t ticket_base, nla_crs_slot_status *__restrict__ status,
     uint32_t *__restrict__ fwcnt, uint32_t *__restrict__ fwrec, int fwcap, double sign, uint64_t resolver_timeout,
-    int ncols, const chain_shard *__restrict__ S, uint32_t seq, uint32_t stopbits)
+    int ncols, const chain_shard *__restrict__ S, uint32_t seq, uint32_t stopbits, int abandon)
 {
     typedef const __attribute__((address_space(4))) chain_lists *kernarg_lists;
     const kernarg_lists Lk = (kernarg_lists) __builtin_amdgcn_kernarg_segment_ptr();
@@ -59,29 +60,38 @@
     static_assert(U <= 64, "one lane per row of a batch");
     __shared__ V sacc[64];
     __shared__ int32_t srow[NLA_ADV_RCAP];
-    __shared__ int s_turn, s_ticket, s_last, s_state;
-    __shared__ uint32_t s_nrec, s_halt;
+    __shared__ int s_turn, s_ticket, s_last, s_state, s_left, s_leftpicks;
+    __shared__ uint32_t s_nrec, s_halt, s_dead;
     __shared__ double scratch[2 * CH_FWAVES];
     volatile __attribute__((address_space(3))) int *turn = (volatile __attribute__((address_space(3))) int *) &s_turn;
+    volatile __attribute__((address_space(3))) int *left = (volatile __attribute__((address_space(3))) int *) &s_left;
     const int lane = threadIdx.x & 63;
     const int wave = __builtin_amdgcn_readfirstlane((int) (threadIdx.x >> 6));
     double *fv = reinterpret_cast<double *>(ctrl + 1);
-    uint32_t *done = reinterpret_cast<uint32_t *>(fv + 2 * (size_t) K), *rowstate = done + 2 * (size_t) K;
+    uint32_t *done = reinterpret_cast<uint32_t *>(fv + 2 * (size_t) K), *dead = done + (size_t) K, *rowstate = done + 2 * (size_t) K;
+    uint32_t *abpicks = rowstate + (size_t) nW + 8;
+    const bool AB = !SH && abandon != 0;
     const int64_t *W = Lk->inl ? (const int64_t *) Lk->W : Wd;
     const double *Wf = Lk->inl ? (const double *) Lk->Wf : Wfd;
+    constexpr bool LOOP = SH || PERSIST;
 #define CH_NEXT do { if constexpr (SH) continue; else return; } while (0)
+#define CH_LEAVE { if constexpr (LOOP) continue; else return; }
     for (;;) {
-    if constexpr (SH) __syncthreads();
-    if (threadIdx.x == 0) { s_ticket = (int) (atomicAdd(&ctrl->ticket, 1u) - ticket_base); s_nrec = 0; s_halt = ld_agent(&ctrl->halt); }
+    if constexpr (LOOP) __syncthreads();
+    if (threadIdx.x == 0) {
+        const int t = (int) (atomicAdd(&ctrl->ticket, 1u) - ticket_base);
+        s_ticket = t; s_nrec = 0; s_halt = ld_agent(&ctrl->halt); s_left = 0; s_leftpicks = 0;
+        s_dead = (AB && t >= 1 && t <= K * chunks) ? ld_agent(&dead[(t - 1) / chunks]) : 0u;
+    }
     __syncthreads();
-    if constexpr (SH) { if (s_ticket > K * chunks) return; }
+    if constexpr (LOOP) { if (s_ticket > K * chunks) return; }
     if (s_ticket == 0) {
         if (wave == 0) {
             if constexpr (SH) {
                 if (lane < S->world) st_sys(S->peerstop[lane] + (seq & 1u) * NLA_SH_MAXW + (uint32_t) S->rank, (seq << 2) | (stopbits & 3u));
             }
             chain_resolver_wave(reinterpret_cast<uint32_t *>(ctrl), reinterpret_cast<const uint64_t *>(fv), rowstate, K, nW, W, Wf, f_best, i0,
-                                resolver_timeout, !SH && n < NLA_CHAIN_LIGHT_BELOW);
+                                resolver_timeout, !SH && n < NLA_CHAIN_LIGHT_BELOW, AB ? dead : nullptr);
             if constexpr (SH) {
                 uint32_t bits = 0, bad = 0;
                 if (lane < S->world) {
@@ -103,11 +113,26 @@
     }
     const int wg = s_ticket - 1;
     const int a = wg / chunks, chunk = wg % chunks;
+    auto slot_left = [&](uint32_t word) {
+        if ((word >> 16) == 0 || (word & 0xffffu) + (word >> 16) != (uint32_t) chunks) return;
+        const uint64_t picks = (uint64_t) ld_agent(&abpicks[a]) + (uint64_t) (word & 0xffffu) * (uint64_t) n;
+        uint32_t why = AB ? ld_agent(&dead[a]) : 0u;
+        if (!why) why = CH_DEAD_BEST;
+        status[a].t = 0; status[a].pad = (int32_t) (((uint32_t) (picks / (uint64_t) chunks) << 2) | why);
+    };
+    auto leave_chunk = [&](int picks) {
+        if (chunk == 0) fwcnt[a] = 0;
+        if (picks > 0) {
+            __hip_atomic_fetch_add(&abpicks[a], (uint32_t) picks, __ATOMIC_RELAXED, __HIP_MEMORY_SCOPE_AGENT);
+            asm volatile("s_waitcnt vmcnt(0)" ::: "memory");
+        }
+        slot_left(__hip_atomic_fetch_add(&done[a], CH_LEFT, __ATOMIC_RELAXED, __HIP_MEMORY_SCOPE_AGENT) + CH_LEFT);
+    };
     {
         const uint32_t h = s_halt;
-        if ((h & 2u) && (uint32_t) a >= (h >> 8)) {
-            if (threadIdx.x == 0) { status[a].t = 0; if (chunk == 0) fwcnt[a] = 0; }
-            CH_NEXT;
+        if (((h & 2u) && (uint32_t) a >= (h >> 8)) || s_dead) {
+            if constexpr (SH) { if (threadIdx.x == 0) { status[a].t = 0; if (chunk == 0) fwcnt[a] = 0; } CH_NEXT; }
+            else { if (threadIdx.x == 0) leave_chunk(0); CH_LEAVE }
         }
     }
     const uint64_t block = first_block + (uint64_t) a;
@@ -157,6 +182,9 @@
     const double hneg = -(0.5 * n);
     const uint32_t lane_off = (uint32_t) (colc * sizeof(double));
     V v[U];
+    const bool ABM = AB && n <= NLA_ADV_RCAP;
+    uint32_t pollv = 0;
+    bool went = false, saw = false;
     for (int seg0 = 0; seg0 < n; seg0 += NLA_ADV_RCAP) {
         const int cnt = (n - seg0 < NLA_ADV_RCAP) ? n - seg0 : NLA_ADV_RCAP;
         nla_lds_barrier();
@@ -170,6 +198,7 @@
             const int base = b * U;
             const int mine = base + lane < cnt ? base + lane : cnt - 1;
             const int32_t myrow = srow[mine];
+            if (ABM) pollv = ld_agent(&dead[a]);
 #pragma unroll
             for (int u = 0; u < U; ++u) {
                 const int64_t r = (int64_t) __builtin_amdgcn_readlane(myrow, u);
@@ -201,8 +230,15 @@
         };
         if (wave < nb) issue(wave);
         for (int ph = wave; ph < nb; ph += WAVES) {
-            while (*turn != ph) __builtin_amdgcn_s_sleep(1);
+            int tn;
+            while ((tn = *turn) != ph && tn >= 0) __builtin_amdgcn_s_sleep(1);
             asm volatile("" ::: "memory");
+            if (tn < 0) { went = true; break; }
+            if (ABM && __builtin_amdgcn_readfirstlane((int) pollv) != 0) {
+                if (lane == 0) { s_leftpicks = seg0 + ph * U; *left = 1; asm volatile("s_waitcnt lgkmcnt(0)" ::: "memory"); *turn = -1; }
+                went = true;
+                break;
+            }
             V acc = sacc[lane];
             const int base = ph * U, tb = seg0 + base;
             if (base + U <= cnt && !(jn >= tb && jn < tb + U)) {
@@ -218,11 +254,16 @@
             if (lane == 0) *turn = ph + 1;
             if (ph + WAVES < nb) issue(ph + WAVES);
         }
+        if (went) break;
         if (wave == 0) {
-            while (*turn != nb) __builtin_amdgcn_s_sleep(1);
+            int tn;
+            while ((tn = *turn) != nb && tn >= 0) __builtin_amdgcn_s_sleep(1);
             asm volatile("" ::: "memory");
-        }
-    }
+            if (tn < 0) { went = true; break; }
+        }
+    }
+    if (went) nla_lds_barrier();
+    if (!(went || saw)) {
     if (wave == 0 && active) {
         V acc = sacc[lane];
         const double s = 2.0 / n;
@@ -250,16 +291,25 @@
         asm volatile("s_waitcnt vmcnt(0)" ::: "memory");
     }
     __syncthreads();
+    if (ABM && *left) saw = true;
+    }
+    if (went || saw) {
+        if (threadIdx.x == 0) leave_chunk(s_leftpicks);
+        CH_LEAVE
+    }
     if constexpr (SH) {
         if (threadIdx.x < (unsigned) S->world)
             st_sys(S->peerflags[threadIdx.x] + (size_t) a * (size_t) S->chunks_total + (size_t) (S->chunk0 + chunk), seq << 2);
     }
     if (threadIdx.x == 0) {
         if (chunk == 0) fwcnt[a] = s_nrec;
-        s_last = (atomicAdd(&done[a], 1u) == (uint32_t) (chunks - 1));
+        const uint32_t before = atomicAdd(&done[a], 1u);
+        s_last = (before == (uint32_t) (chunks - 1));
+        if constexpr (!SH) slot_left(before + 1u);
     }
     __syncthreads();
-    if (!s_last) CH_NEXT;
+    if constexpr (SH) { if (!s_last) CH_NEXT; }
+    else if (!s_last) CH_LEAVE
     if constexpr (SH) {
         if (wave == 0) {
             const uint32_t *fl = S->peerflags[S->rank] + (size_t) a * (size_t) S->chunks_total;
@@ -290,7 +340,11 @@
         __builtin_amdgcn_fence(__ATOMIC_ACQUIRE, "");
     } else
     {
+#ifdef NLA_CHAIN_EVAL_LIGHT
+        if (true) __builtin_amdgcn_fence(__ATOMIC_ACQUIRE, "workgroup");
+#else
         if (n < NLA_CHAIN_LIGHT_BELOW) __builtin_amdgcn_fence(__ATOMIC_ACQUIRE, "workgroup");
+#endif
         else __builtin_amdgcn_fence(__ATOMIC_ACQUIRE, "agent");
     }
     {
@@ -323,14 +377,15 @@
             __hip_atomic_store(rec + 1, ch_bits_of_f(fM), __ATOMIC_RELAXED, __HIP_MEMORY_SCOPE_AGENT);
         }
     }
-    if constexpr (!SH) return;
+    if constexpr (!LOOP) return;
     }
 #undef CH_NEXT
+#undef CH_LEAVE
 }
 
 extern "C" size_t nla_crs_chain_ctrl_bytes(int K, int nW)
 {
-    return sizeof(chain_ctrl) + sizeof(double) * 2 * (size_t) K + sizeof(uint32_t) * (2 * (size_t) K + (size_t) nW + 8);
+    return sizeof(chain_ctrl) + sizeof(double) * 2 * (size_t) K + sizeof(uint32_t) * (3 * (size_t) K + (size_t) nW + 8);
 }
 
 static bool chain_vec2(int n, int ld)
@@ -347,10 +402,26 @@
     return (n + cpw - 1) / cpw;
 }
 
-extern "C" uint32_t nla_crs_chain_tickets(int n, int ld, int K)
-{
-    return (uint32_t) nla_crs_chain_chunks(n, ld) * (uint32_t) K + 1u;
-}
+#ifndef NLA_CHAIN_WGS_DEFAULT
+#define NLA_CHAIN_WGS_DEFAULT 0
+#endif
+static int chain_cap(int n, int wgs)
+{
+    if (wgs == 0) wgs = (n >= 2048 && NLA_CHAIN_WGS_DEFAULT >= 2) ? NLA_CHAIN_WGS_DEFAULT : -1;
+    return wgs;
+}
+static unsigned chain_grid(int n, int ld, int K, int wgs)
+{
+    const long total = (long) nla_crs_chain_chunks(n, ld) * K + 1;
+    const int cap = chain_cap(n, wgs);
+    return (unsigned) ((cap >= 2 && cap < total) ? cap : total);
+}
+extern "C" uint32_t nla_crs_chain_tickets_wgs(int n, int ld, int K, int wgs)
+{
+    const uint32_t slots = (uint32_t) nla_crs_chain_chunks(n, ld) * (uint32_t) K;
+    return slots + (chain_cap(n, wgs) >= 2 ? chain_grid(n, ld, K, wgs) : 1u);
+}
+extern "C" uint32_t nla_crs_chain_tickets(int n, int ld, int K) { return nla_crs_chain_tickets_wgs(n, ld, K, 0); }
 
 extern "C" int nla_k_crs_chain_lean(int obj, int n, int ld, const double *X, int64_t i0, double f_best, const int32_t *jn_ring,
                                     const int32_t *pos_ring, const int32_t *last_ring, const uint32_t *words_ring, uint32_t ring_blocks,
@@ -372,7 +443,18 @@
                         uint64_t first_block, int K, const int64_t *W, const double *Wf, int nW, int w_on_host, int slot_mask,
                         const double *lb, const double *ub, double *TX, double *TM, void *ctrl, uint32_t ticket_base,
                         nla_crs_slot_status *status, uint32_t *fwcnt, uint32_t *fwrec, int fwcap, int ctrl_is_zero, void *stream,
-                        int ncols, const chain_shard *S, int ldf, uint32_t seq, uint32_t stopbits, int grid_cap);
+                        int ncols, const chain_shard *S, int ldf, uint32_t seq, uint32_t stopbits, int grid_cap, int abandon);
+extern "C" int nla_k_crs_chain_wgs(int obj, int n, int ld, const double *X, int64_t i0, double f_best, const int32_t *jn_ring,
+                                   const int32_t *pos_ring, const int32_t *last_ring, const uint32_t *words_ring, uint32_t ring_blocks,
+                                   uint64_t first_block, int K, const int64_t *W, const double *Wf, int nW, int w_on_host, int slot_mask,
+                                   const double *lb, const double *ub, double *TX, double *TM, void *ctrl, uint32_t ticket_base,
+                                   nla_crs_slot_status *status, uint32_t *fwcnt, uint32_t *fwrec, int fwcap, int ctrl_is_zero, int wgs, int abandon,
+                                   void *stream)
+{
+    if (wgs < -1 || wgs == 1) return (int) hipErrorInvalidValue;
+    return chain_launch(obj, n, ld, X, i0, f_best, jn_ring, pos_ring, last_ring, words_ring, ring_blocks, first_block, K, W, Wf, nW, w_on_host, slot_mask,
+                        lb, ub, TX, TM, ctrl, ticket_base, status, fwcnt, fwrec, fwcap, ctrl_is_zero, stream, n, nullptr, ld, 0u, 0u, wgs, abandon);
+}
 extern "C" int nla_k_crs_chain_lean(int obj, int n, int ld, const double *X, int64_t i0, double f_best, const int32_t *jn_ring,
                                     const int32_t *pos_ring, const int32_t *last_ring, const uint32_t *words_ring, uint32_t ring_blocks,
                                     uint64_t first_block, int K, const int64_t *W, const double *Wf, int nW, int w_on_host, int slot_mask,
@@ -380,7 +462,7 @@
                                     nla_crs_slot_status *status, uint32_t *fwcnt, uint32_t *fwrec, int fwcap, int ctrl_is_zero, void *stream)
 {
     return chain_launch(obj, n, ld, X, i0, f_best, jn_ring, pos_ring, last_ring, words_ring, ring_blocks, first_block, K, W, Wf, nW, w_on_host, slot_mask,
-                        lb, ub, TX, TM, ctrl, ticket_base, status, fwcnt, fwrec, fwcap, ctrl_is_zero, stream, n, nullptr, ld, 0u, 0u, 0);
+                        lb, ub, TX, TM, ctrl, ticket_base, status, fwcnt, fwrec, fwcap, ctrl_is_zero, stream, n, nullptr, ld, 0u, 0u, 0, 0);
 }
 
 extern "C" int nla_crs_chain_sh_chunks(int n, int ncols)
@@ -411,7 +493,7 @@
 {
     if (!table || ncols < 1 || ncols > ld || ldf < n || ldf % 16 != 0) return (int) hipErrorInvalidValue;
     return chain_launch(obj, n, ld, X, i0, f_best, jn_ring, pos_ring, last_ring, words_ring, ring_blocks, first_block, K, W, Wf, nW, w_on_host, slot_mask,
-                        lb, ub, TX, TM, ctrl, ticket_base, status, fwcnt, fwrec, fwcap, ctrl_is_zero, stream, ncols, (const chain_shard *) table, ldf, seq, stopbits, grid_cap);
+                        lb, ub, TX, TM, ctrl, ticket_base, status, fwcnt, fwrec, fwcap, ctrl_is_zero, stream, ncols, (const chain_shard *) table, ldf, seq, stopbits, grid_cap, 0);
 }
 static unsigned chain_sh_grid(int n, int ncols, int K, int grid_cap)
 {
@@ -428,7 +510,7 @@
                         uint64_t first_block, int K, const int64_t *W, const double *Wf, int nW, int w_on_host, int slot_mask,
                         const double *lb, const double *ub, double *TX, double *TM, void *ctrl, uint32_t ticket_base,
                         nla_crs_slot_status *status, uint32_t *fwcnt, uint32_t *fwrec, int fwcap, int ctrl_is_zero, void *stream,
-                        int ncols, const chain_shard *S, int ldf, uint32_t seq, uint32_t stopbits, int grid_cap)
+                        int ncols, const chain_shard *S, int ldf, uint32_t seq, uint32_t stopbits, int grid_cap, int abandon)
 {
     if (K <= 0) return 0;
     if (K > 256 || nW > 256 || nW < 0 || obj < 0) return (int) hipErrorInvalidValue;
@@ -448,19 +530,25 @@
     const bool vec2 = sh ? (n >= 128 && ncols % 2 == 0 && ld % 2 == 0) : chain_vec2(n, ld);
     const int chunks = sh ? nla_crs_chain_sh_chunks(n, ncols) : nla_crs_chain_chunks(n, ld);
     if (sh && (ldf % 16 != 0)) return (int) hipErrorInvalidValue;
-    const dim3 grid(sh ? chain_sh_grid(n, ncols, K, grid_cap) : (unsigned) ((long) chunks * K) + 1u);
+    if (chunks >= (int) CH_LEFT - 1) return (int) hipErrorInvalidValue;
+    const bool persist = !sh && chain_cap(n, grid_cap) >= 2;
+    const dim3 grid(sh ? chain_sh_grid(n, ncols, K, grid_cap) : chain_grid(n, ld, K, grid_cap));
     const uint64_t res_timeout = 200000000ull;
     chain_ctrl *c = (chain_ctrl *) ctrl;
     if (!ctrl_is_zero) {
         hipError_t e = hipMemsetAsync((char *) ctrl + sizeof(uint32_t), 0, nla_crs_chain_ctrl_bytes(K, nW) - sizeof(uint32_t), st);
         if (e != hipSuccess) return (int) e;
     }
-#define CHAIN(VEC, UU, WV, O) hipLaunchKernelGGL((crs_chain_kernel<VEC, UU, WV, O>), grid, dim3(WV * 64), 0, st, L, n, ld, X, i0, f_best, jn_ring, \
-        pos_ring, last_ring, words_ring, ring_blocks, first_block, K, W, Wf, nW, slot_mask, chunks, lb, ub, TX, TM, c, ticket_base, status,         \
-        fwcnt, fwrec, fwcap, sign, res_timeout, ncols, S, seq, stopbits)
-#define CHAIN_SH(VEC, UU, WV, O) hipLaunchKernelGGL((crs_chain_kernel<VEC, UU, WV, O, true>), grid, dim3(WV * 64), 0, st, L, n, ld, X, i0, f_best, jn_ring, \
-        pos_ring, last_ring, words_ring, ring_blocks, first_block, K, W, Wf, nW, slot_mask, chunks, lb, ub, TX, TM, c, ticket_base, status,         \
-        fwcnt, fwrec, fwcap, sign, res_timeout, ncols, S, seq, stopbits)
+#define CHAIN_ARGS L, n, ld, X, i0, f_best, jn_ring, pos_ring, last_ring, words_ring, ring_blocks, first_block, K, W, Wf, nW, slot_mask, chunks, lb, ub, TX, TM, c, \
+        ticket_base, status, fwcnt, fwrec, fwcap, sign, res_timeout, ncols, S, seq, stopbits, abandon
+#define CHAIN(VEC, UU, WV, O) do {                                                                                                                    \
+        if (persist) hipLaunchKernelGGL((crs_chain_kernel<VEC, UU, WV, O, false, true>), grid, dim3(WV * 64), 0, st, CHAIN_ARGS);                 \
+        else hipLaunchKernelGGL((crs_chain_kernel<VEC, UU, WV, O>), grid, dim3(WV * 64), 0, st, CHAIN_ARGS);                                       \
+    } while (0)
+#define CHAIN_SH(VEC, UU, WV, O) hipLaunchKernelGGL((crs_chain_kernel<VEC, UU, WV, O, true>), grid, dim3(WV * 64), 0, st, CHAIN_ARGS)
+#ifndef NLA_CHAIN_HIGH_U
+#define NLA_CHAIN_HIGH_U 32
+#endif
 #ifndef NLA_CHAIN_MID_W
 #define NLA_CHAIN_MID_W 8
 #endif
@@ -478,9 +566,9 @@
 #endif
 #define CHAIN_SHAPE(O)                                                                   \
     if (vec2) {                                                                          \
-        if (n >= 2048) CHAIN(2, 32, 8, O); else if (n >= 512) CHAIN(2, NLA_CHAIN_MID_U, NLA_CHAIN_MID_W, O); else CHAIN(2, NLA_CHAIN_LOW_U, NLA_CHAIN_LOW_W, O); \
+        if (n >= 2048) CHAIN(2, NLA_CHAIN_HIGH_U, 8, O); else if (n >= 512) CHAIN(2, NLA_CHAIN_MID_U, NLA_CHAIN_MID_W, O); else CHAIN(2, NLA_CHAIN_LOW_U, NLA_CHAIN_LOW_W, O); \
     } else {                                                                             \
-        if (n >= 2048) CHAIN(1, 32, 8, O); else if (n >= 512) CHAIN(1, NLA_CHAIN_MID_U, NLA_CHAIN_MID_W, O); else if (n >= 128) CHAIN(1, NLA_CHAIN_LOW_U, NLA_CHAIN_LOW_W, O); else CHAIN(1, 16, NLA_CHAIN_TINY_W, O); \
+        if (n >= 2048) CHAIN(1, NLA_CHAIN_HIGH_U, 8, O); else if (n >= 512) CHAIN(1, NLA_CHAIN_MID_U, NLA_CHAIN_MID_W, O); else if (n >= 128) CHAIN(1, NLA_CHAIN_LOW_U, NLA_CHAIN_LOW_W, O); else CHAIN(1, 16, NLA_CHAIN_TINY_W, O); \
     }
 #define CHAIN_SHAPE_SH(O)                                                                \
     if (vec2) { if (n >= 512) CHAIN_SH(2, 32, 8, O); else CHAIN_SH(2, 16, 4, O); } else CHAIN_SH(1, 16, 4, O);
@@ -490,6 +578,7 @@
 #undef CHAIN_SH
 #undef CHAIN_SHAPE
 #undef CHAIN
+#undef CHAIN_ARGS
     NLA_LAUNCH_CHECK();
     return 0;
 }
diff --git a/nlopt_amd/csrc/hip/crs_chain_resolver.h b/nlopt_amd/csrc/hip/crs_chain_resolver.h
--- a/nlopt_amd/csrc/hip/crs_chain_resolver.h
+++ b/nlopt_amd/csrc/hip/crs_chain_resolver.h
@@ -50,12 +50,16 @@
 #define CH_CTRL_WP 5
 #define CH_CTRL_NEXTRA 6
 #define CH_CTRL_PK 7
+#define CH_DEAD_ROLE 1u
+#define CH_DEAD_BEST 2u
 
 CH_DEV void chain_resolver_wave(uint32_t *ctrl_words, const uint64_t *recs, uint32_t *rowstate, int K, int nW,
-                                const int64_t *W, const double *Wf, double f_best, int64_t i0, uint64_t timeout, bool light = false)
+                                const int64_t *W, const double *Wf, double f_best, int64_t i0, uint64_t timeout, bool light = false,
+                                uint32_t *dead = nullptr)
 {
     const int lane = ch_lane();
     uint32_t next = 0, wp = 0, nextra = 0, naccept = 0, halt = 0, idle = 0;
+    uint32_t dead_upto = 0;
     uint64_t xfb = 0;
     int64_t xrow = 0;
     uint64_t wfb[4];
@@ -134,8 +138,14 @@
             int kind = 0;
             double fnew = 0;
             if (fT < fw) { kind = 1; fnew = fT; }
-            else if (rmi == 0) break;
-            else if (fM < fw) { kind = 2; fnew = fM; }
+            else {
+                if (dead && j + 1u < (uint32_t) K && j + 1u >= dead_upto) {
+                    if (lane == 0) ch_st32(&dead[j + 1u], CH_DEAD_ROLE);
+                    dead_upto = j + 2u;
+                }
+                if (rmi == 0) break;
+                if (fM < fw) { kind = 2; fnew = fM; }
+            }
             if (kind) {
                 if (xi >= 0) {
                     const uint64_t lf = ch_readlane_u64(xfb, nextra - 1);
@@ -159,6 +169,7 @@
                 if (fnew < f_best || (fnew == f_best && rw < i0)) {
                     halt = 2u | ((j + 1u) << 8);
                     if (lane == 0) ch_st32(&ctrl_words[CH_CTRL_HALT], halt);
+                    if (dead) for (uint32_t s2 = j + 1u + (uint32_t) lane; s2 < (uint32_t) K; s2 += 64u) ch_st32(&dead[s2], CH_DEAD_BEST);
                 }
             }
             i += (kind == 1) ? 1u : 2u;
```

After: 45220 evals/s. No clear change (-0.0%).
